# voxel-tracer/cuda-raytracing-optimized

Hardware: AMD Instinct MI355X
Metric: Msamples/s (pixels x spp / s), random-spheres 1200x800x100spp (higher is better)
Workload: dtype f32; 1 GPU; random-spheres (488 spheres, LCG seed 0) 1200x800 100spp maxDepth 50, gradient sky, reference RNG stream, fp parity; spp=100, max_depth=50, spheres=488, partition=single GPU, fp_mode=parity, rng=reference, kernel_variant=0

## Files before the change

cuda-raytracing-optimized_amd/__init__.py:

```python
import ctypes as C
import os

import numpy as np

_HERE = os.path.dirname(os.path.abspath(__file__))
RENDERER_LIB = os.path.join(_HERE, "librt_mi355x.so")
HOST_LIB = os.path.join(_HERE, "librt_host.so")

RT_DIFFUSE, RT_METAL, RT_GLASS = 0, 1, 2
(RT_FLOOR_COAT, RT_FLOOR_DIFFUSE, RT_FLOOR_CHECKER, RT_MODEL_COAT, RT_MODEL_DIFFUSE, RT_MODEL_GLOSSY, RT_MODEL_GLASS,
 RT_MODEL_TINTEDGLASS, RT_MODEL_SSS) = range(3, 12)
RT_SKY_CONST_GREY, RT_SKY_GRADIENT = 0, 1
RT_RNG_REFERENCE_STREAM, RT_RNG_COUNTER = 0, 1
RT_FP_PARITY, RT_FP_FAST = 0, 1
RT_MAX_DEVICES = 8



class vec3(C.Structure):
    _fields_ = [("e", C.c_float * 3)]


class camera(C.Structure):
    _fields_ = [("origin", vec3), ("lower_left_corner", vec3), ("horizontal", vec3), ("vertical", vec3),
                ("u", vec3), ("v", vec3), ("w", vec3), ("lens_radius", C.c_float)]


class sphere(C.Structure):
    _fields_ = [("center", vec3), ("radius", C.c_float)]


class plane(C.Structure):
    _fields_ = [("norm", vec3), ("point", vec3)]


class bbox(C.Structure):
    _fields_ = [("min", vec3), ("max", vec3)]


class triangle(C.Structure):
    _fields_ = [("v", vec3 * 3), ("texCoords", C.c_float * 6), ("meshID", C.c_ubyte), ("_pad", C.c_ubyte * 3)]


class bvh_node(C.Structure):
    _fields_ = [("a", vec3), ("b", vec3)]


class material(C.Structure):
    _fields_ = [("type", C.c_int32), ("color", vec3), ("param", C.c_float), ("texId", C.c_int32)]


class stexture(C.Structure):
    _fields_ = [("data", C.POINTER(C.c_float)), ("width", C.c_int32), ("height", C.c_int32)]


class mesh(C.Structure):
    _fields_ = [("tris", C.POINTER(triangle)), ("numTris", C.c_uint32), ("bvh", C.POINTER(bvh_node)),
                ("numBvhNodes", C.c_int32), ("bounds", bbox)]


class kernel_scene(C.Structure):
    _fields_ = [("m", C.POINTER(mesh)), ("floor", plane), ("materials", C.POINTER(material)),
                ("numMaterials", C.c_int32), ("textures", C.POINTER(stexture)), ("numTextures", C.c_int32),
                ("numPrimitivesPerLeaf", C.c_int32)]


class render_options(C.Structure):
    _fields_ = [("sky", C.c_int32), ("nee", C.c_int32), ("rr", C.c_int32), ("t_min", C.c_float),
                ("rng", C.c_int32), ("fp", C.c_int32), ("light", sphere), ("lightColor", vec3),
                ("stripe_rows", C.c_int32), ("num_devices", C.c_int32), ("devices", C.c_int32 * RT_MAX_DEVICES),
                ("part_rank", C.c_int32), ("part_world", C.c_int32), ("variant", C.c_int32), ("counters", C.c_int32),
                ("samples_per_item", C.c_int32), ("floor", C.c_int32)]


class render_stats(C.Structure):
    _fields_ = [("kernel_ms", C.c_double), ("total_ms", C.c_double), ("samples", C.c_int64),
                ("num_launches", C.c_int32), ("vgprs", C.c_int32), ("rays", C.c_uint64),
                ("prim_tests", C.c_uint64), ("node_visits", C.c_uint64), ("exec_tests", C.c_uint64),
                ("shadow_rays", C.c_uint64), ("box_tests", C.c_uint64), ("ref_stats", C.c_uint64 * 18)]


(RT_STAT_PRIMARY, RT_STAT_PRIMARY_HIT_MESH, RT_STAT_PRIMARY_NOHITS, RT_STAT_PRIMARY_BBOX_NOHITS, RT_STAT_SECONDARY,
 RT_STAT_SECONDARY_MESH, RT_STAT_SECONDARY_NOHIT, RT_STAT_SECONDARY_MESH_NOHIT, RT_STAT_SECONDARY_BBOX_NOHIT, RT_STAT_SHADOWS,
 RT_STAT_SHADOWS_BBOX_NOHITS, RT_STAT_SHADOWS_NOHITS, RT_STAT_LOW_POWER, RT_STAT_EXCEED_MAX_BOUNCE, RT_STAT_RUSSIAN_KILL,
 RT_STAT_NAN, RT_STAT_NODES_BOTH, RT_STAT_NODES_SINGLE) = range(18)
RT_STAT_NAMES = ["primary", "primary hit mesh", "primary nohit", "primary bb nohit", "secondary", "secondary mesh", "secondary no hit",
                 "secondary mesh nohit", "secondary bb nohit", "shadows", "shadows bb nohit", "shadows nohit", "power < 0.01",
                 "exceeded max bounce", "russian roulette", "NaNs", "both nodes hit", "single node hit"]


_SIZES = {vec3: 12, camera: 88, sphere: 16, plane: 24, bbox: 24, triangle: 64, bvh_node: 24, material: 24,
          stexture: 16, mesh: 56, kernel_scene: 64}
for _t, _s in _SIZES.items():
    assert C.sizeof(_t) == _s, (_t, C.sizeof(_t), _s)

sphere_dtype = np.dtype([("center", np.float32, 3), ("radius", np.float32)])
material_dtype = np.dtype([("type", np.int32), ("color", np.float32, 3), ("param", np.float32), ("texId", np.int32)])
triangle_dtype = np.dtype([("v", np.float32, (3, 3)), ("texCoords", np.float32, 6), ("meshID", np.uint8), ("_pad", np.uint8, 3)])
bvh_node_dtype = np.dtype([("a", np.float32, 3), ("b", np.float32, 3)])
assert sphere_dtype.itemsize == 16 and material_dtype.itemsize == 24
assert triangle_dtype.itemsize == 64 and bvh_node_dtype.itemsize == 24

RENDERER_SYMBOLS = ["initRenderer", "runRenderer", "cleanupRenderer", "initRendererSpheres",
                    "getDefaultRenderOptions", "setRenderOptions", "setExternalFramebuffer", "getRenderStats",
                    "rtDeviceCount", "rtApiVersion", "rtStructSizes", "rtLastLaunches",
                    "runRendererProgressive", "rtProgressiveSamples", "rtResetProgressive", "setCamera",
                    "renderGuides", "rtLastGuidesMs",
                    "rtDefaultDenoiseFlags", "denoiseFrame", "rtLastDenoiseMs",
                    "accumulateFrame", "rtResetHistory", "rtHistoryFrames", "rtLastAccumulateMs",
                    "previewFrame", "rtResetPreview", "rtPreviewFrames", "rtLastPreviewMs",
                    "displayFrame", "rtLastExposure", "rtDisplayHistogram", "rtResetDisplay", "rtLastDisplayMs",
                    "traceRays", "occludedRays", "rtLastRaysMs",
                    "updateTriangles", "updateMaterials", "updateSpheres", "getMeshBvh", "rtLastUpdateMs",
                    "rebuildBvh", "rtLastRebuildMs",
                    "rtLastSphereForm"]
RT_API_VERSION = 1002
ABI_STRUCTS = [render_options, render_stats, camera, sphere, material, triangle, bvh_node, mesh, kernel_scene, stexture, plane, bbox, vec3]
HOST_SYMBOLS = ["rtMakeCamera", "rtRandomFloat", "rtSceneThreeSpheres", "rtSceneRandomSpheres", "rtStaircaseCamera",
                "rtBuildBvh", "rtBuildBvhLevels", "rtLoadBvhFile", "rtSaveBvhFile", "rtFreeMesh", "rtMeshView",
                "rtSceneStaircaseProcedural", "rtLinearToSRGB", "rtWritePPM", "rtSaveReference", "rtLoadReference", "rtRmse",
                "rtDisplayFrameHost", "rtCentreRays", "rtRefitBvhArrays", "rtRefitBvh", "rtRebuildBvhArrays", "rtRebuildBvh"]

_renderer = None
_host = None


def load_host():
    global _host
    if _host is None:
        if not os.path.exists(HOST_LIB):
            raise ImportError(f"{HOST_LIB} is not built: run `make` (or __graft_entry__.build())")
        h = C.CDLL(HOST_LIB)
        fp = C.POINTER(C.c_float)
        h.rtMakeCamera.argtypes = [fp, fp, fp, C.c_float, C.c_float, C.c_float, C.c_float, C.POINTER(camera)]
        h.rtMakeCamera.restype = None
        h.rtRandomFloat.argtypes = [C.POINTER(C.c_uint32)]
        h.rtRandomFloat.restype = C.c_float
        h.rtSceneThreeSpheres.argtypes = [C.c_void_p, C.c_void_p, C.c_int, C.c_int, C.c_int, C.POINTER(camera)]
        h.rtSceneThreeSpheres.restype = C.c_int
        h.rtSceneRandomSpheres.argtypes = [C.c_uint32, C.c_void_p, C.c_void_p, C.c_int, C.c_int, C.c_int, C.POINTER(camera)]
        h.rtSceneRandomSpheres.restype = C.c_int
        h.rtStaircaseCamera.argtypes = [C.c_int, C.c_int, C.POINTER(camera)]
        h.rtStaircaseCamera.restype = None
        h.rtBuildBvh.argtypes = [C.c_void_p, C.c_int, C.c_int]
        h.rtBuildBvh.restype = C.c_void_p
        h.rtBuildBvhLevels.argtypes = [C.c_void_p, C.c_int, C.c_int, C.c_int]
        h.rtBuildBvhLevels.restype = C.c_void_p
        h.rtLoadBvhFile.argtypes = [C.c_char_p]
        h.rtLoadBvhFile.restype = C.c_void_p
        h.rtSaveBvhFile.argtypes = [C.c_void_p, C.c_char_p]
        h.rtSaveBvhFile.restype = C.c_int
        h.rtFreeMesh.argtypes = [C.c_void_p]
        h.rtFreeMesh.restype = None
        h.rtMeshView.argtypes = [C.c_void_p, C.POINTER(mesh)]
        h.rtMeshView.restype = C.c_int
        h.rtSceneStaircaseProcedural.argtypes = [C.c_int, C.c_void_p, C.c_int, C.c_void_p]
        h.rtSceneStaircaseProcedural.restype = C.c_int
        h.rtLinearToSRGB.argtypes = [C.c_float]
        h.rtLinearToSRGB.restype = C.c_uint32
        h.rtWritePPM.argtypes = [C.c_char_p, C.c_int, C.c_int, C.c_void_p]
        h.rtWritePPM.restype = C.c_int
        h.rtSaveReference.argtypes = [C.c_char_p, C.c_int, C.c_int, C.c_void_p]
        h.rtSaveReference.restype = C.c_int
        h.rtLoadReference.argtypes = [C.c_char_p, C.c_void_p, C.c_int, C.c_int]
        h.rtLoadReference.restype = C.c_int
        h.rtRmse.argtypes = [C.c_void_p, C.c_void_p, C.c_int, C.c_int]
        h.rtRmse.restype = C.c_double
        h.rtDisplayFrameHost.argtypes = [C.c_void_p, C.c_void_p, C.c_int, C.c_int, C.c_int, C.c_int, C.c_float, C.c_float, C.POINTER(C.c_float),
                                         C.POINTER(C.c_uint32)]
        h.rtDisplayFrameHost.restype = C.c_int
        h.rtCentreRays.argtypes = [C.POINTER(camera), C.c_int, C.c_int, C.POINTER(C.c_int32), C.c_int, fp, fp]
        h.rtCentreRays.restype = None
        h.rtRefitBvhArrays.argtypes = [C.c_void_p, C.c_uint32, C.c_void_p, C.c_int, C.c_int, C.POINTER(bbox)]
        h.rtRefitBvhArrays.restype = C.c_int
        h.rtRefitBvh.argtypes = [C.c_void_p]
        h.rtRefitBvh.restype = C.c_int
        h.rtRebuildBvhArrays.argtypes = [C.c_void_p, C.c_uint32, C.c_void_p, C.c_int, C.c_int, C.POINTER(bbox), C.c_void_p]
        h.rtRebuildBvhArrays.restype = C.c_int
        h.rtRebuildBvh.argtypes = [C.c_void_p, C.c_void_p]
        h.rtRebuildBvh.restype = C.c_int
        _host = h
    return _host


def check_abi(lib, path=RENDERER_LIB, structs=None):
    structs = ABI_STRUCTS if structs is None else structs
    if not hasattr(lib, "rtStructSizes"):
        raise ImportError(f"{path} predates the ABI handshake (no rtStructSizes): rebuild it with `make`")
    lib.rtApiVersion.argtypes = []
    lib.rtApiVersion.restype = C.c_int
    lib.rtStructSizes.argtypes = [C.POINTER(C.c_int32), C.c_int]
    lib.rtStructSizes.restype = C.c_int
    ver = lib.rtApiVersion()
    if ver != RT_API_VERSION:
        raise ImportError(f"{path} has API version {ver}, this binding was written against {RT_API_VERSION}: rebuild the library or update the mirror")
    out = (C.c_int32 * len(structs))()
    n = lib.rtStructSizes(out, len(structs))
    if n != len(structs):
        raise ImportError(f"{path} reports {n} ABI structs, the mirror has {len(structs)}")
    for t, sz in zip(structs, out):
        if C.sizeof(t) != sz:
            raise ImportError(f"{path}: sizeof({t.__name__}) is {sz} in the library and {C.sizeof(t)} in the Python mirror - "
                              "library and mirror are of different generations; refusing to call into it")


def load_renderer():
    global _renderer
    if _renderer is None:
        if not os.path.exists(RENDERER_LIB):
            raise ImportError(f"{RENDERER_LIB} is not built: run `make` (or __graft_entry__.build()); "
                              "there is no CPU fallback for the render path")
        r = C.CDLL(RENDERER_LIB)
        check_abi(r)
        r.initRenderer.argtypes = [kernel_scene, camera, C.POINTER(C.POINTER(vec3)), C.c_int, C.c_int, C.c_int]
        r.initRenderer.restype = None
        r.runRenderer.argtypes = [C.c_int, C.c_int, C.c_int]
        r.runRenderer.restype = None
        r.cleanupRenderer.argtypes = []
        r.cleanupRenderer.restype = None
        r.initRendererSpheres.argtypes = [C.c_void_p, C.c_void_p, C.c_int, camera, C.POINTER(C.POINTER(vec3)),
                                          C.c_int, C.c_int, C.c_int]
        r.initRendererSpheres.restype = None
        r.getDefaultRenderOptions.argtypes = [C.POINTER(render_options), C.c_int]
        r.getDefaultRenderOptions.restype = None
        r.setRenderOptions.argtypes = [C.POINTER(render_options)]
        r.setRenderOptions.restype = None
        r.setExternalFramebuffer.argtypes = [C.c_void_p]
        r.setExternalFramebuffer.restype = None
        r.getRenderStats.argtypes = [C.POINTER(render_stats)]
        r.getRenderStats.restype = None
        r.rtDeviceCount.argtypes = []
        r.rtDeviceCount.restype = C.c_int
        r.rtApiVersion.argtypes = []
        r.rtApiVersion.restype = C.c_int
        r.rtLastLaunches.argtypes = [C.POINTER(C.c_int32), C.c_int]
        r.rtLastLaunches.restype = C.c_int
        r.runRendererProgressive.argtypes = [C.c_int, C.c_int, C.c_int]
        r.runRendererProgressive.restype = None
        r.rtProgressiveSamples.argtypes = []
        r.rtProgressiveSamples.restype = C.c_int
        r.rtResetProgressive.argtypes = []
        r.rtResetProgressive.restype = None
        r.setCamera.argtypes = [C.POINTER(camera)]
        r.setCamera.restype = None
        r.renderGuides.argtypes = [C.c_int, C.POINTER(C.c_float), C.POINTER(C.c_float), C.POINTER(C.c_float),
                                   C.POINTER(C.c_int32), C.POINTER(C.c_int32)]
        r.renderGuides.restype = None
        r.rtLastGuidesMs.argtypes = []
        r.rtLastGuidesMs.restype = C.c_double
        r.rtDefaultDenoiseFlags.argtypes = []
        r.rtDefaultDenoiseFlags.restype = C.c_int
        r.denoiseFrame.argtypes = [C.c_void_p, C.c_void_p, C.c_int, C.c_int, C.c_int, C.c_float, C.c_float]
        r.denoiseFrame.restype = None
        r.rtLastDenoiseMs.argtypes = []
        r.rtLastDenoiseMs.restype = C.c_double
        r.accumulateFrame.argtypes = [C.c_void_p, C.c_void_p, C.c_void_p, C.c_int, C.c_int, C.c_float, C.c_float]
        r.accumulateFrame.restype = None
        r.rtResetHistory.argtypes = []
        r.rtResetHistory.restype = None
        r.rtHistoryFrames.argtypes = []
        r.rtHistoryFrames.restype = C.c_int
        r.rtLastAccumulateMs.argtypes = []
        r.rtLastAccumulateMs.restype = C.c_double
        r.previewFrame.argtypes = [C.c_void_p, C.c_void_p, C.c_void_p, C.c_void_p, C.c_int, C.c_int, C.c_int, C.c_int, C.c_float, C.c_float, C.c_float]
        r.previewFrame.restype = None
        r.rtResetPreview.argtypes = []
        r.rtResetPreview.restype = None
        r.rtPreviewFrames.argtypes = []
        r.rtPreviewFrames.restype = C.c_int
        r.rtLastPreviewMs.argtypes = []
        r.rtLastPreviewMs.restype = C.c_double
        r.displayFrame.argtypes = [C.c_void_p, C.c_void_p, C.c_int, C.c_int, C.c_float, C.c_float]
        r.displayFrame.restype = None
        r.rtLastExposure.argtypes = []
        r.rtLastExposure.restype = C.c_float
        r.rtDisplayHistogram.argtypes = [C.POINTER(C.c_uint32), C.c_int]
        r.rtDisplayHistogram.restype = C.c_int
        r.rtResetDisplay.argtypes = []
        r.rtResetDisplay.restype = None
        r.rtLastDisplayMs.argtypes = []
        r.rtLastDisplayMs.restype = C.c_double
        fp, ip = C.POINTER(C.c_float), C.POINTER(C.c_int32)
        r.traceRays.argtypes = [C.c_int, fp, fp, fp, fp, C.c_int, fp, ip, fp, fp, ip]
        r.traceRays.restype = None
        r.occludedRays.argtypes = [C.c_int, fp, fp, fp, fp, C.POINTER(C.c_uint8)]
        r.occludedRays.restype = None
        r.rtLastRaysMs.argtypes = []
        r.rtLastRaysMs.restype = C.c_double
        r.updateTriangles.argtypes = [C.c_int, C.c_int, C.c_void_p]
        r.updateTriangles.restype = None
        r.updateMaterials.argtypes = [C.c_void_p, C.c_int]
        r.updateMaterials.restype = None
        r.updateSpheres.argtypes = [C.c_void_p, C.c_void_p, C.c_int]
        r.updateSpheres.restype = None
        r.getMeshBvh.argtypes = [C.c_void_p, C.c_int, C.POINTER(bbox)]
        r.getMeshBvh.restype = C.c_int
        r.rtLastUpdateMs.argtypes = []
        r.rtLastUpdateMs.restype = C.c_double
        r.rebuildBvh.argtypes = [C.c_void_p]
        r.rebuildBvh.restype = None
        r.rtLastRebuildMs.argtypes = []
        r.rtLastRebuildMs.restype = C.c_double
        _renderer = r
    return _renderer



def _f3(v):
    return (C.c_float * 3)(*[float(x) for x in v])


def make_camera(lookfrom, lookat, vup, vfov, aspect, aperture, focus_dist):
    cam = camera()
    load_host().rtMakeCamera(_f3(lookfrom), _f3(lookat), _f3(vup), vfov, aspect, aperture, focus_dist, C.byref(cam))
    return cam


def scene_three_spheres(nx, ny):
    sp = np.zeros(3, sphere_dtype)
    mt = np.zeros(3, material_dtype)
    cam = camera()
    n = load_host().rtSceneThreeSpheres(sp.ctypes.data, mt.ctypes.data, 3, nx, ny, C.byref(cam))
    assert n == 3
    return sp, mt, cam


def scene_random_spheres(nx, ny, seed=0):
    cap = 488
    sp = np.zeros(cap, sphere_dtype)
    mt = np.zeros(cap, material_dtype)
    cam = camera()
    n = load_host().rtSceneRandomSpheres(seed, sp.ctypes.data, mt.ctypes.data, cap, nx, ny, C.byref(cam))
    assert n == cap, n
    return sp, mt, cam


def staircase_camera(nx, ny):
    cam = camera()
    load_host().rtStaircaseCamera(nx, ny, C.byref(cam))
    return cam


class HostMesh:

    def __init__(self, handle):
        if not handle:
            raise ValueError("mesh build/load failed")
        self._h = C.c_void_p(handle)
        self.view = mesh()
        self.nppl = load_host().rtMeshView(self._h, C.byref(self.view))

    @classmethod
    def build(cls, tris, nppl=5, extra_levels=None):
        tris = np.ascontiguousarray(tris, dtype=triangle_dtype)
        if extra_levels is None:
            return cls(load_host().rtBuildBvh(tris.ctypes.data, len(tris), nppl))
        return cls(load_host().rtBuildBvhLevels(tris.ctypes.data, len(tris), nppl, extra_levels))

    @classmethod
    def load(cls, path):
        return cls(load_host().rtLoadBvhFile(os.fsencode(path)))

    def save(self, path):
        return load_host().rtSaveBvhFile(self._h, os.fsencode(path))

    @property
    def tris(self):
        return np.ctypeslib.as_array(C.cast(self.view.tris, C.POINTER(C.c_ubyte)), (self.view.numTris * 64,)).view(triangle_dtype)

    @property
    def bvh(self):
        return np.ctypeslib.as_array(C.cast(self.view.bvh, C.POINTER(C.c_ubyte)), (self.view.numBvhNodes * 24,)).view(bvh_node_dtype)

    def refit(self):
        if load_host().rtRefitBvh(self._h) != 0:
            raise ValueError("rtRefitBvh refused the mesh")
        self.nppl = load_host().rtMeshView(self._h, C.byref(self.view))

    def rebuild(self):
        old_slot = np.zeros(self.view.numTris, np.int32)
        if load_host().rtRebuildBvh(self._h, old_slot.ctypes.data) != 0:
            raise ValueError("rtRebuildBvh refused the mesh")
        self.nppl = load_host().rtMeshView(self._h, C.byref(self.view))
        return old_slot

    def close(self):
        if self._h:
            load_host().rtFreeMesh(self._h)
            self._h = None

    def __del__(self):
        try:
            self.close()
        except Exception:
            pass


def scene_staircase_procedural(detail=1):
    h = load_host()
    mats = np.zeros(20, material_dtype)
    need = h.rtSceneStaircaseProcedural(detail, None, 0, mats.ctypes.data)
    n = -need if need < 0 else need
    tris = np.zeros(n, triangle_dtype)
    got = h.rtSceneStaircaseProcedural(detail, tris.ctypes.data, n, mats.ctypes.data)
    assert got == n, (got, n)
    return tris, mats


def make_kernel_scene(host_mesh, materials, textures=(), floor=None):
    materials = np.ascontiguousarray(materials, dtype=material_dtype)
    ks = kernel_scene()
    ks.m = C.pointer(host_mesh.view)
    ks.materials = C.cast(materials.ctypes.data, C.POINTER(material))
    ks.numMaterials = len(materials)
    tex_arr = (stexture * max(1, len(textures)))()
    keep = [materials, tex_arr, host_mesh]
    for k, t in enumerate(textures):
        t = np.ascontiguousarray(t, dtype=np.float32)
# ... 167 lines not shown
def update_materials(mats):
    mats = _records("update_materials", "material", mats, material_dtype)
    load_renderer().updateMaterials(mats.ctypes.data, len(mats))


def update_spheres(spheres, mats):
    spheres = _records("update_spheres", "sphere", spheres, sphere_dtype)
    mats = _records("update_spheres", "material", mats, material_dtype)
    if len(spheres) != len(mats):
        raise ValueError("update_spheres: one material per sphere")
    load_renderer().updateSpheres(spheres.ctypes.data, mats.ctypes.data, len(spheres))


def mesh_bvh():
    r = load_renderer()
    n = r.getMeshBvh(None, 0, None)
    nodes = np.zeros(n, bvh_node_dtype)
    b = bbox()
    r.getMeshBvh(nodes.ctypes.data, n, C.byref(b))
    return nodes, np.array([list(b.min.e), list(b.max.e)], np.float32)


def last_update_ms():
    return load_renderer().rtLastUpdateMs()


def _header_constant(name):
    import re
    text = open(os.path.join(os.path.dirname(_HERE), "include", "rt_api.h")).read()
    m = re.search(r"^#define\s+%s\s+\(?\s*(\d+)\s*(?:<<\s*(\d+))?\s*\)?\s*$" % name, text, re.M)
    if not m:
        raise ImportError(f"include/rt_api.h does not define {name}")
    return int(m.group(1)) << int(m.group(2) or 0)


RT_REBUILD_TILE = _header_constant("RT_REBUILD_TILE")
RT_REBUILD_MAX_TRIS = _header_constant("RT_REBUILD_MAX_TRIS")


def rebuild_bvh():
    r = load_renderer()
    old_slot = np.zeros(int(_state.get("num_tris") or 0) if not _state.get("spheres") else 0, np.int32)
    r.rebuildBvh(old_slot.ctypes.data if len(old_slot) else None)
    return old_slot


def last_rebuild_ms():
    return load_renderer().rtLastRebuildMs()


def rebuild_bvh_arrays(tris, bvh, nppl):
    for name, a, dt in (("tris", tris, triangle_dtype), ("bvh", bvh, bvh_node_dtype)):
        if not (isinstance(a, np.ndarray) and a.dtype == dt and a.ndim == 1 and a.flags["C_CONTIGUOUS"] and a.flags["WRITEABLE"]):
            raise ValueError(f"rebuild_bvh_arrays: {name} must be a writable C-contiguous one-dimensional array of its record dtype")
    if isinstance(nppl, bool) or not isinstance(nppl, (int, np.integer)):
        raise ValueError("rebuild_bvh_arrays: nppl must be an integer")
    b = bbox()
    old_slot = np.zeros(len(tris), np.int32)
    if load_host().rtRebuildBvhArrays(tris.ctypes.data, len(tris), bvh.ctypes.data, len(bvh), int(nppl), C.byref(b), old_slot.ctypes.data) != 0:
        return None
    return np.array([list(b.min.e), list(b.max.e)], np.float32), old_slot


def refit_bvh_arrays(tris, bvh, nppl):
    tris = _records("refit_bvh_arrays", "triangle", tris, triangle_dtype)
    if not (isinstance(bvh, np.ndarray) and bvh.dtype == bvh_node_dtype and bvh.ndim == 1 and bvh.flags["C_CONTIGUOUS"] and bvh.flags["WRITEABLE"]):
        raise ValueError("refit_bvh_arrays: bvh must be a writable C-contiguous one-dimensional array of bvh_node_dtype records")
    b = bbox()
    if load_host().rtRefitBvhArrays(tris.ctypes.data, len(tris), bvh.ctypes.data, len(bvh), int(nppl), C.byref(b)) != 0:
        return None
    return np.array([list(b.min.e), list(b.max.e)], np.float32)


def centre_rays(cam, nx, ny, ij):
    ij = np.ascontiguousarray(ij, dtype=np.int32)
    if ij.ndim != 2 or ij.shape[1] != 2:
        raise ValueError(f"centre_rays: ij must have shape (n, 2), got {ij.shape}")
    n = ij.shape[0]
    org, d = np.zeros((n, 3), np.float32), np.zeros((n, 3), np.float32)
    fp = C.POINTER(C.c_float)
    load_host().rtCentreRays(C.byref(cam), nx, ny, ij.ctypes.data_as(C.POINTER(C.c_int32)), n, org.ctypes.data_as(fp), d.ctypes.data_as(fp))
    return org, d


RT_DENOISE_DEMODULATE, RT_DENOISE_SAME_PRIM = 1, 2
RT_DENOISE_MAX_ITERATIONS, RT_DENOISE_MAX_SQUARINGS, RT_DENOISE_ALBEDO_FLOOR = 8, 7, 0.01


def default_denoise_flags():
    return load_renderer().rtDefaultDenoiseFlags()


def _frame_in_out(who, fb, out):
    shape = (_state["ny"], _state["nx"], 3)
    ok = lambda a: isinstance(a, np.ndarray) and a.dtype == np.float32 and a.flags["C_CONTIGUOUS"] and a.shape == shape
    if fb is not None and not ok(fb):
        raise ValueError(f"{who}: fb must be a C-contiguous float32 array of shape {shape}")
    if out is None:
        out = np.empty(shape, np.float32)
    elif not (ok(out) and out.flags["WRITEABLE"]):
        raise ValueError(f"{who}: out must be a writable C-contiguous float32 array of shape {shape}")
    return None if fb is None else fb.ctypes.data, out


def denoiseFrame(fb=None, iterations=5, flags=None, normal_squarings=5, sigma_z=0.01, sigma_c=1.0, out=None):
    r = load_renderer()
    if flags is None:
        flags = r.rtDefaultDenoiseFlags()
    src, out = _frame_in_out("denoiseFrame", fb, out)
    r.denoiseFrame(src, out.ctypes.data, iterations, flags, normal_squarings, sigma_z, sigma_c)
    return out


def last_denoise_ms():
    return load_renderer().rtLastDenoiseMs()


RT_ACCUM_MAX_HISTORY = 1024


def accumulateFrame(fb=None, out=None, history=False, flags=None, max_history=32, sigma_z=0.01, normal_min=0.9):
    nx, ny = _state["nx"], _state["ny"]
    r = load_renderer()
    if flags is None:
        flags = r.rtDefaultDenoiseFlags()
    src, out = _frame_in_out("accumulateFrame", fb, out)
    hist = None
    if history is True:
        hist = np.empty((ny, nx), np.float32)
    elif history is not False and history is not None:
        hist = history
        if not (isinstance(hist, np.ndarray) and hist.dtype == np.float32 and hist.flags["C_CONTIGUOUS"] and hist.flags["WRITEABLE"] and hist.shape == (ny, nx)):
            raise ValueError(f"accumulateFrame: history must be True, False or a writable C-contiguous float32 array of shape {(ny, nx)}")
    r.accumulateFrame(src, out.ctypes.data, None if hist is None else hist.ctypes.data, flags, max_history, sigma_z, normal_min)
    return out if hist is None else (out, hist)


def reset_history():
    load_renderer().rtResetHistory()


def history_frames():
    return load_renderer().rtHistoryFrames()


def last_accumulate_ms():
    return load_renderer().rtLastAccumulateMs()


RT_PREVIEW_MIN_HISTORY, RT_PREVIEW_LUM_EPS = 4.0, 1e-4


def _pixel_plane(who, what, plane):
    shape = (_state["ny"], _state["nx"])
    if plane is True:
        return np.empty(shape, np.float32)
    if plane is False or plane is None:
        return None
    if not (isinstance(plane, np.ndarray) and plane.dtype == np.float32 and plane.flags["C_CONTIGUOUS"] and plane.flags["WRITEABLE"] and plane.shape == shape):
        raise ValueError(f"{who}: {what} must be True, False or a writable C-contiguous float32 array of shape {shape}")
    return plane


def previewFrame(fb=None, out=None, history=False, variance=False, flags=None, max_history=32, iterations=5, normal_squarings=5, sigma_z=0.01, normal_min=0.9,
                 sigma_l=4.0):
    r = load_renderer()
    if flags is None:
        flags = r.rtDefaultDenoiseFlags()
    src, out = _frame_in_out("previewFrame", fb, out)
    hist = _pixel_plane("previewFrame", "history", history)
    var = _pixel_plane("previewFrame", "variance", variance)
    r.previewFrame(src, out.ctypes.data, None if hist is None else hist.ctypes.data, None if var is None else var.ctypes.data, flags, max_history, iterations,
                   normal_squarings, sigma_z, normal_min, sigma_l)
    planes = tuple(a for a in (hist, var) if a is not None)
    return (out,) + planes if planes else out


def reset_preview():
    load_renderer().rtResetPreview()


def preview_frames():
    return load_renderer().rtPreviewFrames()


def last_preview_ms():
    return load_renderer().rtLastPreviewMs()


RT_DISPLAY_TOP_DOWN, RT_DISPLAY_DITHER, RT_DISPLAY_AUTO_EXPOSURE, RT_DISPLAY_FROM_PREVIEW = 1, 2, 4, 8
RT_TONEMAP_NONE, RT_TONEMAP_REINHARD, RT_TONEMAP_ACES = 0, 1, 2
RT_DISPLAY_BINS, RT_DISPLAY_KEY = 256, 0.18
RT_DISPLAY_BAYER8 = ((0, 32, 8, 40, 2, 34, 10, 42), (48, 16, 56, 24, 50, 18, 58, 26), (12, 44, 4, 36, 14, 46, 6, 38), (60, 28, 52, 20, 62, 30, 54, 22),
                     (3, 35, 11, 43, 1, 33, 9, 41), (51, 19, 59, 27, 49, 17, 57, 25), (15, 47, 7, 39, 13, 45, 5, 37), (63, 31, 55, 23, 61, 29, 53, 21))


def _display_in_out(who, src, out, shape):
    if src is not None and not (isinstance(src, np.ndarray) and src.dtype == np.float32 and src.flags["C_CONTIGUOUS"] and src.shape == shape + (3,)):
        raise ValueError(f"{who}: src must be a C-contiguous float32 array of shape {shape + (3,)}")
    if out is None:
        out = np.empty(shape + (4,), np.uint8)
    elif not (isinstance(out, np.ndarray) and out.dtype == np.uint8 and out.flags["C_CONTIGUOUS"] and out.flags["WRITEABLE"] and out.shape == shape + (4,)):
        raise ValueError(f"{who}: out must be a writable C-contiguous uint8 array of shape {shape + (4,)}")
    return None if src is None else src.ctypes.data, out


def display_frame(src=None, out=None, flags=0, tonemap=0, exposure=1.0, adapt=1.0):
    src, out = _display_in_out("display_frame", src, out, (_state["ny"], _state["nx"]))
    load_renderer().displayFrame(src, out.ctypes.data, flags, tonemap, exposure, adapt)
    return out


def last_exposure():
    return load_renderer().rtLastExposure()


def display_histogram():
    out = np.zeros(RT_DISPLAY_BINS, np.uint32)
    n = load_renderer().rtDisplayHistogram(out.ctypes.data_as(C.POINTER(C.c_uint32)), RT_DISPLAY_BINS)
    assert n == RT_DISPLAY_BINS
    return out


def reset_display():
    load_renderer().rtResetDisplay()


def last_display_ms():
    return load_renderer().rtLastDisplayMs()


def display_frame_host(src, out=None, flags=0, tonemap=0, exposure=1.0, adapt=1.0, state=None, histogram=False):
    if not (isinstance(src, np.ndarray) and src.ndim == 3):
        raise ValueError("display_frame_host: src must be a (ny, nx, 3) float32 array")
    addr, out = _display_in_out("display_frame_host", src, out, src.shape[:2])
    if state is not None and not (isinstance(state, np.ndarray) and state.dtype == np.float32 and state.size == 1 and state.flags["WRITEABLE"]):
        raise ValueError("display_frame_host: state must be None or a writable float32 array of one element")
    hist = np.zeros(RT_DISPLAY_BINS, np.uint32) if histogram else None
    rc = load_host().rtDisplayFrameHost(addr, out.ctypes.data, src.shape[1], src.shape[0], flags, tonemap, exposure, adapt,
                                        None if state is None else state.ctypes.data_as(C.POINTER(C.c_float)),
                                        None if hist is None else hist.ctypes.data_as(C.POINTER(C.c_uint32)))
    if rc != 0:
        raise ValueError("display_frame_host: arguments displayFrame would refuse (flags, tonemap, exposure or adapt)")
    return (out, hist) if histogram else out


def cleanupRenderer():
    load_renderer().cleanupRenderer()
    _state.update(fb=None, keep=None)


def getDefaultRenderOptions(is_sphere_scene):
    o = render_options()
    load_renderer().getDefaultRenderOptions(C.byref(o), 1 if is_sphere_scene else 0)
    return o


def setRenderOptions(opt=None, **kw):
    if opt is None:
        raise ValueError("pass the options struct from getDefaultRenderOptions()")
    for k, v in kw.items():
        if k == "devices":
            opt.num_devices = len(v)
            for idx, d in enumerate(v):
                opt.devices[idx] = d
        else:
            setattr(opt, k, v)
    load_renderer().setRenderOptions(C.byref(opt))
    return opt


def setExternalFramebuffer(array):
    if array is None:
        load_renderer().setExternalFramebuffer(None)
        _state["ext"] = None
        return
    assert array.dtype == np.float32 and array.flags["C_CONTIGUOUS"] and array.shape == (_state["ny"], _state["nx"], 3)
    load_renderer().setExternalFramebuffer(array.ctypes.data)
    _state["ext"] = array


def getRenderStats():
    s = render_stats()
    load_renderer().getRenderStats(C.byref(s))
    return s


def device_count():
    return load_renderer().rtDeviceCount()


RT_KERNEL_SPHERE_QUEUE, RT_KERNEL_SPHERE_TILES, RT_KERNEL_MESH_QUEUE, RT_KERNEL_MESH_TILES = 1, 2, 3, 4
LAUNCH_FIELDS = ("family", "phase", "cls", "chunked", "dbg", "scene", "lean", "threads", "blocks", "device", "fp")


def last_launches():
    lib = load_renderer()
    n = lib.rtLastLaunches(None, 0)
    buf = (C.c_int32 * (n * len(LAUNCH_FIELDS)))()
    n = min(n, lib.rtLastLaunches(buf, n))
    return [dict(zip(LAUNCH_FIELDS, buf[k * len(LAUNCH_FIELDS):(k + 1) * len(LAUNCH_FIELDS)])) for k in range(n)]


RT_SPHERE_FORM_NONE, RT_SPHERE_FORM_GENERAL, RT_SPHERE_FORM_DEFAULT = -1, 0, 1


def last_sphere_form():
    lib = load_renderer()
    lib.rtLastSphereForm.argtypes = []
    lib.rtLastSphereForm.restype = C.c_int
    return lib.rtLastSphereForm()



def write_ppm(path, fb):
    fb = np.ascontiguousarray(fb, dtype=np.float32)
    return load_host().rtWritePPM(os.fsencode(path), fb.shape[1], fb.shape[0], fb.ctypes.data)


def save_reference(path, fb):
    fb = np.ascontiguousarray(fb, dtype=np.float32)
    return load_host().rtSaveReference(os.fsencode(path), fb.shape[1], fb.shape[0], fb.ctypes.data)


def load_reference(path, nx, ny):
    out = np.zeros((ny, nx, 3), np.float32)
    rc = load_host().rtLoadReference(os.fsencode(path), out.ctypes.data, nx, ny)
    return rc, out


def rmse(f, g):
    f = np.ascontiguousarray(f, dtype=np.float32)
    g = np.ascontiguousarray(g, dtype=np.float32)
    assert f.shape == g.shape
    return load_host().rtRmse(f.ctypes.data, g.ctypes.data, f.shape[1], f.shape[0])



PROBE_SYMBOLS = [f"rtProbe{n}_{m}" for n in ("Rng", "DiskSphere", "GetRay", "SphereHit", "TriangleHit", "Bbox", "Scatter", "Math", "ShadowRay", "PlaneHit", "SinCos", "Schlick")
                 for m in ("parity", "fast")]


def _f32(a):
    return np.ascontiguousarray(a, dtype=np.float32)


def _u32(a):
    return np.ascontiguousarray(a, dtype=np.uint32)


def _p(a):
    return a.ctypes.data_as(C.c_void_p)


class Probe:

    def __init__(self, mode="parity"):
        assert mode in ("parity", "fast")
        self.lib = load_renderer()
        self.sfx = "_" + mode

    def _fn(self, name):
        f = getattr(self.lib, "rtProbe" + name + self.sfx)
        f.restype = None
        return f

    def rng(self, pixel_ids):
        ids = _u32(pixel_ids); n = len(ids)
        seed = np.zeros(n, np.uint32); draws = np.zeros((n, 4), np.float32); state = np.zeros(n, np.uint32)
        self._fn("Rng")(_p(ids), C.c_int(n), _p(seed), _p(draws), _p(state))
        return seed, draws, state

    def disk_sphere(self, states):
        st = _u32(states); n = len(st)
        disk = np.zeros((n, 3), np.float32); sd = np.zeros(n, np.uint32)
        sph = np.zeros((n, 3), np.float32); ss = np.zeros(n, np.uint32)
        self._fn("DiskSphere")(_p(st), C.c_int(n), _p(disk), _p(sd), _p(sph), _p(ss))
        return disk, sd, sph, ss

    def get_ray(self, cam, s, t, states):
        s = _f32(s); t = _f32(t); st = _u32(states); n = len(s)
        org = np.zeros((n, 3), np.float32); d = np.zeros((n, 3), np.float32); sa = np.zeros(n, np.uint32)
        self._fn("GetRay")(C.byref(cam), _p(s), _p(t), _p(st), C.c_int(n), _p(org), _p(d), _p(sa))
        return org, d, sa

    def sphere_hit(self, spheres, org, dirs, tmin, tmax):
        sp = np.ascontiguousarray(spheres, dtype=sphere_dtype); n = len(sp)
        org = _f32(org); dirs = _f32(dirs); tmin = _f32(tmin); tmax = _f32(tmax)
        out = np.zeros(n, np.float32)
        self._fn("SphereHit")(_p(sp), _p(org), _p(dirs), _p(tmin), _p(tmax), C.c_int(n), _p(out))
        return out

    def triangle_hit(self, tris, org, dirs, tmin, tmax):
        tr = np.ascontiguousarray(tris, dtype=triangle_dtype); n = len(tr)
        org = _f32(org); dirs = _f32(dirs); tmin = _f32(tmin); tmax = _f32(tmax)
        t = np.zeros(n, np.float32); u = np.zeros(n, np.float32); v = np.zeros(n, np.float32)
        self._fn("TriangleHit")(_p(tr), _p(org), _p(dirs), _p(tmin), _p(tmax), C.c_int(n), _p(t), _p(u), _p(v))
        return t, u, v

    def bbox(self, bmin, bmax, org, dirs, tmax):
        bmin = _f32(bmin); bmax = _f32(bmax); org = _f32(org); dirs = _f32(dirs); tmax = _f32(tmax); n = len(tmax)
        dist = np.zeros(n, np.float32); hit = np.zeros(n, np.int32)
        self._fn("Bbox")(_p(bmin), _p(bmax), _p(org), _p(dirs), _p(tmax), C.c_int(n), _p(dist), _p(hit))
        return dist, hit

    def scatter(self, t, normal, inside, wo, mats, color, states, hit_point=None):
        t = _f32(t); normal = _f32(normal); inside = np.ascontiguousarray(inside, dtype=np.int32); wo = _f32(wo)
        hp = _f32(hit_point if hit_point is not None else np.zeros((len(t), 3), np.float32))
        mats = np.ascontiguousarray(mats, dtype=material_dtype); color = _f32(color); st = _u32(states); n = len(t)
        wi = np.zeros((n, 3), np.float32); thr = np.zeros((n, 3), np.float32); flags = np.zeros(n, np.int32)
        tout = np.zeros(n, np.float32); sa = np.zeros(n, np.uint32)
        self._fn("Scatter")(_p(t), _p(hp), _p(normal), _p(inside), _p(wo), _p(mats), _p(color), _p(st), C.c_int(n),
                            _p(wi), _p(thr), _p(flags), _p(tout), _p(sa))
        return wi, thr, flags, tout, sa

    def shadow_ray(self, light, light_color, org, atten, normal, states):
        org = _f32(org); atten = _f32(atten); normal = _f32(normal); st = _u32(states); n = len(st)
        out = np.zeros((n, 9), np.float32); ok = np.zeros(n, np.int32); sa = np.zeros(n, np.uint32)
        self._fn("ShadowRay")(C.byref(light), C.byref(light_color), _p(org), _p(atten), _p(normal), _p(st), C.c_int(n), _p(out), _p(ok), _p(sa))
        return ok, out[:, 0:3], out[:, 3:6], out[:, 6], out[:, 7], out[:, 8].astype(np.int32), sa

    def plane_hit(self, planes, org, dirs, tmin, tmax):
        pl = np.ascontiguousarray(planes, dtype=np.float32).reshape(-1, 6); n = len(pl)
        org = _f32(org); dirs = _f32(dirs); tmin = _f32(tmin); tmax = _f32(tmax)
        out = np.zeros(n, np.float32)
        self._fn("PlaneHit")(_p(pl), _p(org), _p(dirs), _p(tmin), _p(tmax), C.c_int(n), _p(out))
        return out

    def sincos(self, y):
        y = _f32(y); n = len(y)
        s = np.zeros(n, np.float32); c = np.zeros(n, np.float32)
        self._fn("SinCos")(_p(y), C.c_int(n), _p(s), _p(c))
        return s, c

    def schlick(self, cosine, ref_idx, u):
        c = _f32(cosine); r = _f32(ref_idx); u = _f32(u); n = len(c)
        out = np.zeros(n, np.float32); above = np.zeros(n, np.int32)
        self._fn("Schlick")(_p(c), _p(r), _p(u), C.c_int(n), _p(out), _p(above))
        return out, above

    def math(self, a, b):
        a = _f32(a); b = _f32(b); n = len(a)
        q = np.zeros(n, np.float32); r = np.zeros(n, np.float32); p5 = np.zeros(n, np.float32); u3 = np.zeros((n, 3), np.float32)
        self._fn("Math")(_p(a), _p(b), C.c_int(n), _p(q), _p(r), _p(p5), _p(u3))
        return q, r, p5, u3
```

cuda-raytracing-optimized_amd/csrc/rt_kernels_spheres.hip:

```cpp
#include "rt_device.h"
#include "rt_params.h"
#include "rt_sphere_form.h"

#include <float.h>
#include <cstdio>
#include <cstdlib>
#include <algorithm>
#include <utility>

using namespace rtd;

#if defined(RT_MODE_PARITY)
#define RT_LAUNCH_NAME rt_launch_spheres_parity
#elif defined(RT_MODE_FAST)
#define RT_LAUNCH_NAME rt_launch_spheres_fast
#else
#error "define RT_MODE_PARITY or RT_MODE_FAST"
#endif

namespace {

#ifndef RT_BOX_CUT
#define RT_BOX_CUT 12
#endif
// ... 873 lines not shown
        if (px < P.nx && r < P.part.local_rows)
            fbf[((size_t)r * P.nx + i0) * 3 + off] = wfb[q];
    }

    if (P.counters) {
        atomicAdd(&P.counters->rays, (unsigned long long)nrays);
        atomicAdd(&P.counters->prim_tests, (unsigned long long)nrays * (unsigned long long)P.n);
        atomicAdd(&P.counters->exec_tests, (unsigned long long)groups_done * 4ull);
        atomicAdd(&P.counters->box_tests, (unsigned long long)boxes_done);
    }
}

template <int SCENE>
__global__ void __launch_bounds__(kThreads) k_classify_spheres(const RtSphereParams P) {
    extern __shared__ __align__(16) unsigned char smem[];
    float* unused;
    const SceneLds S = stage_scene<false, SCENE>(P, smem, &unused);
    const int tiles_x = (P.nx + 7) >> 3;
    const int tiles_y = (P.part.local_rows + 7) >> 3;
    const uint32_t total = (uint32_t)tiles_x * (uint32_t)tiles_y * 64u;
    const uint32_t p = blockIdx.x * kThreads + threadIdx.x;
    const uint32_t tile = p >> 6, within = p & 63u;
    const int ty = (int)(tile / (uint32_t)tiles_x), tx = (int)(tile - (uint32_t)ty * (uint32_t)tiles_x);
    const int i = tx * 8 + (int)(within & 7u);
    const int lr = ty * 8 + (int)(within >> 3);
    const bool valid = p < total && i < P.nx && lr < P.part.local_rows;
    bool hits = false, glass = false;
    if (valid) {
        const int j = global_row(P.part, lr);
        const float u = ((float)i + 0.5f) / (float)P.nx, v = ((float)j + 0.5f) / (float)P.ny;
        const f3 org = ld3(P.cam.origin);
        const f3 dn = unit(ld3(P.cam.lower_left_corner) + u * ld3(P.cam.horizontal) + v * ld3(P.cam.vertical) - org);
        for (int k = 0; k < P.n_padded; k++) {
            const float4 sph = S.sph[sidx(k)];
            const f3 oc = org - F3(sph.x, sph.y, sph.z);
            const float b = dot(oc, dn);
            const float c = dot(oc, oc) - sph.w;
            const bool h = (S.orig[k] != 0x7fffffff) && (b * b - c > 0.0f) && (b < 0.0f || c < 0.0f);
            hits = hits || h;
            glass = glass || (h && S.typ[k] == RT_GLASS);
        }
    }
    const int cls = glass ? 0 : (hits ? 1 : 2);
    const unsigned long long m0 = __ballot(valid && cls == 0), m1 = __ballot(valid && cls == 1), m2 = __ballot(valid && cls == 2);
    uint32_t b0 = 0, b1 = 0, b2 = 0;
    if ((threadIdx.x & 63) == 0) {
        if (m0) b0 = atomicAdd(P.queue + 4, (uint32_t)__popcll(m0));
        if (m1) b1 = atomicAdd(P.queue + 5, (uint32_t)__popcll(m1));
        if (m2) b2 = atomicAdd(P.queue + 6, (uint32_t)__popcll(m2));
    }
    b0 = __builtin_amdgcn_readfirstlane(b0);
    b1 = __builtin_amdgcn_readfirstlane(b1);
    b2 = __builtin_amdgcn_readfirstlane(b2);
    if (valid) {
        const unsigned long long m = cls == 0 ? m0 : (cls == 1 ? m1 : m2);
        const uint32_t base = cls == 0 ? b0 : (cls == 1 ? b1 : b2);
        const uint32_t rank = __builtin_amdgcn_mbcnt_hi((uint32_t)(m >> 32), __builtin_amdgcn_mbcnt_lo((uint32_t)m, 0u));
        P.order[(uint32_t)cls * total + base + rank] = p;
    }
}

#if defined(RT_MODE_PARITY)
__device__ __forceinline__ Hit first_hit_spheres(const RtSphereParams& P, const SceneLds& S, f3 org, f3 dn, float t_min, float t_max, f3& normal) {
    const float a = dot(dn, dn);
    Hit h = { t_max, -1, 0x7fffffff };
    for (int k = 0; k < P.n_padded; k++) {
        const int orig = S.orig[k];
        if (orig == 0x7fffffff) continue;
        const float t = sphere_hit_exact(S.sph[sidx(k)], org, dn, a, t_min, h.closest);
        if (t < t_max) accept(h, t, k, orig);
    }
    normal = F3(0, 0, 0);
    if (h.sid >= 0) {
        const float4 sc4 = S.sph[sidx(h.sid)];
        const f3 hp = org + h.closest * dn;
        normal = (hp - F3(sc4.x, sc4.y, sc4.z)) / S.rad[h.sid];
        if (dot(dn, normal) > 0.0f) normal = -normal;
    } else {
        h.closest = FLT_MAX;
    }
    return h;
}

template <int SCENE>
__global__ void __launch_bounds__(kThreads) k_guides_spheres(const RtSphereParams P, const RtGuidePlanes G) {
    extern __shared__ __align__(16) unsigned char smem[];
    float* unused;
    const SceneLds S = stage_scene<false, SCENE>(P, smem, &unused);
    const int tiles_x = (P.nx + 7) >> 3;
    const int tiles_y = (P.part.local_rows + 7) >> 3;
    const uint32_t total = (uint32_t)tiles_x * (uint32_t)tiles_y * 64u;
    const uint32_t p = blockIdx.x * kThreads + threadIdx.x;
    const uint32_t tile = p >> 6, within = p & 63u;
    const int ty = (int)(tile / (uint32_t)tiles_x), tx = (int)(tile - (uint32_t)ty * (uint32_t)tiles_x);
    const int i = tx * 8 + (int)(within & 7u);
    const int lr = ty * 8 + (int)(within >> 3);
    if (!(p < total && i < P.nx && lr < P.part.local_rows)) return;
    const int j = global_row(P.part, lr);
    const float u = ((float)i + 0.5f) / (float)P.nx, v = ((float)j + 0.5f) / (float)P.ny;
    const f3 org = ld3(P.cam.origin);
    const f3 dir = unit(ld3(P.cam.lower_left_corner) + u * ld3(P.cam.horizontal) + v * ld3(P.cam.vertical) - org);
    const f3 dn = unit(dir);
    f3 normal;
    const Hit h = first_hit_spheres(P, S, org, dn, P.t_min, FLT_MAX, normal);
    const size_t px = (size_t)lr * P.nx + i;
    f3 albedo;
    if (h.sid >= 0) {
        const float4 m = S.mat[h.sid];
        albedo = F3(m.x, m.y, m.z);
    } else {
        albedo = sky_color(P.sky, dir);
    }
    if (G.albedo) { float* o = G.albedo + px * 3; o[0] = albedo.x; o[1] = albedo.y; o[2] = albedo.z; }
    if (G.normal) { float* o = G.normal + px * 3; o[0] = normal.x; o[1] = normal.y; o[2] = normal.z; }
    if (G.depth) G.depth[px] = h.closest;
    if (G.prim) G.prim[px] = h.sid >= 0 ? h.orig : RT_GUIDE_PRIM_NONE;
}

template <int SCENE, bool ANY>
__global__ void __launch_bounds__(kThreads) k_rays_spheres(const RtSphereParams P, const RtRayBatch B) {
    extern __shared__ __align__(16) unsigned char smem[];
    float* unused;
    const SceneLds S = stage_scene<false, SCENE>(P, smem, &unused);
    const uint32_t n = (uint32_t)B.n;
    const uint32_t tiles = (n + kThreads - 1) / kThreads;
    for (uint32_t tile = blockIdx.x; tile < tiles; tile += gridDim.x) {
        const uint32_t r = tile * kThreads + threadIdx.x;
        const bool live = r < n;
        f3 org = F3(0, 0, 0), dn = F3(0, 0, 1);
        float t_min = B.t_min_default, t_max = FLT_MAX;
        if (live) {
            const float* o = B.org + (size_t)r * 3;
            const float* d = B.dir + (size_t)r * 3;
            org = F3(o[0], o[1], o[2]);
            dn = unit(F3(d[0], d[1], d[2]));
            if (B.t_min) t_min = B.t_min[r];
            if (B.t_max) t_max = fminf(B.t_max[r], FLT_MAX);
        }
        if (ANY) {
            const float a = dot(dn, dn);
            bool occ = false;
            for (int base = 0; base < P.n_padded; base += kSphereGroup) {
#pragma unroll
                for (int kk = 0; kk < kSphereGroup; kk++) {
                    const int k = base + kk;
                    const int orig = S.orig[k];
                    if (live && !occ && orig != 0x7fffffff)
                        occ = sphere_hit_exact(S.sph[sidx(k)], org, dn, a, t_min, t_max) < t_max;
                }
                if (__ballot(live && !occ) == 0ull) break;
            }
            if (live) B.occluded[r] = occ ? 1 : 0;
        } else if (live) {
            f3 normal;
            const Hit h = first_hit_spheres(P, S, org, dn, t_min, t_max, normal);
            if (B.t) B.t[r] = h.closest;
            if (B.prim) B.prim[r] = h.sid >= 0 ? h.orig : RT_GUIDE_PRIM_NONE;
            if (B.normal) { float* o = B.normal + (size_t)r * 3; o[0] = normal.x; o[1] = normal.y; o[2] = normal.z; }
            if (B.uv) { float* o = B.uv + (size_t)r * 2; o[0] = 0.0f; o[1] = 0.0f; }
        }
    }
}
#endif

constexpr int kCostClasses = 18;
constexpr int kChainClasses = 4;
constexpr int kExactCostSamples = 8;
constexpr int kHeavyClasses = 3;

static_assert(9ull * 16ull * 255ull * RT_PROGRESSIVE_MAX_SAMPLES <= 0xFFFFFFFFull, "cost_class: window sum of a progressive total overflows 32 bits");
__device__ __forceinline__ int cost_class(const RtSphereParams& P, const uint32_t* __restrict__ rays, uint32_t samples, bool exact, int i, int lr) {
    uint32_t sum = 0, cnt = 0;
    for (int dy = -1; dy <= 1; dy++) {
        const int y = lr + dy;
        if (y < 0 || y >= P.part.local_rows) continue;
        for (int dx = -1; dx <= 1; dx++) {
            const int x = i + dx;
            if (x < 0 || x >= P.nx) continue;
            sum += rays[(size_t)y * P.nx + x];
            cnt++;
        }
    }
    const uint32_t own = (rays[(size_t)lr * P.nx + i] * (exact ? 16u : 12u)) / samples;
    const uint32_t e = max((sum * 16u) / (cnt * samples), own);
    const uint32_t lim[kCostClasses - 1] = { (uint32_t)P.chain_top_thr, 320u, 240u, 192u, 160u, 128u, 96u, 72u, 56u, 44u, 36u, 30u, 26u, 22u, 19u, 18u, 17u };
    int cls = kCostClasses - 1;
#pragma unroll
    for (int c = kCostClasses - 2; c >= 0; c--) if (e >= lim[c]) cls = c;
    return cls;
}

__device__ __forceinline__ uint32_t coprime_stride_of(uint32_t n) {
    if (n <= 64u) return 1u;
    uint32_t c = ((uint32_t)((unsigned long long)n * 2654435769ull >> 32)) | 1u;
    for (;;) {
        uint32_t a = c, b = n;
        while (b) { const uint32_t t = a % b; a = b; b = t; }
        if (a == 1u) break;
        c += 2u;
    }
    return c % n;
}

constexpr int kOrderBlocks = 1024;

template <int PASS>
__global__ void __launch_bounds__(kThreads) k_order_by_cost(const RtSphereParams P) {
    constexpr int kLists = kCostClasses * kXcdQueues;
    __shared__ uint32_t s_cnt[kLists], s_base[kLists], s_start[kLists], s_n[kLists], s_stride[kLists];
    const int xq = P.xcd_queues == kXcdQueues ? kXcdQueues : 1;
    const int tiles_x = (P.nx + 7) >> 3;
    const int tiles_y = (P.part.local_rows + 7) >> 3;
    const uint32_t total = (uint32_t)tiles_x * (uint32_t)tiles_y * 64u;
    const uint32_t per = ((total + gridDim.x - 1u) / gridDim.x + (uint32_t)kThreads - 1u) / (uint32_t)kThreads * (uint32_t)kThreads;
    const uint32_t first = blockIdx.x * per, last = min(first + per, total);
    const bool fresh = P.s_split == 0;
    const bool exact = fresh && P.cost_samples >= kExactCostSamples;
    const uint32_t* const rays = fresh ? P.cost_rays : P.px_rays;
    const uint32_t samples = (uint32_t)(fresh ? P.cost_samples : P.s_split);
    uint32_t packed = 0;
    auto class_of = [&](uint32_t p) {
        const uint32_t tile = p >> 6, within = p & 63u;
        const int ty = (int)(tile / (uint32_t)tiles_x), tx = (int)(tile - (uint32_t)ty * (uint32_t)tiles_x);
        const int i = tx * 8 + (int)(within & 7u);
        const int lr = ty * 8 + (int)(within >> 3);
        packed = ((uint32_t)lr << 16) | (uint32_t)i;
        if (!(p < last && i < P.nx && lr < P.part.local_rows)) return -1;
        const int x = xq > 1 ? (int)rt_xcd_of_pixel((uint32_t)lr, (uint32_t)P.nx, (uint32_t)i) : 0;
        return x * kCostClasses + cost_class(P, rays, samples, exact, i, lr);
    };
    if (threadIdx.x < kLists) s_cnt[threadIdx.x] = 0u;
    __syncthreads();
    for (uint32_t p = first + threadIdx.x; p < last; p += kThreads) {
        const int cls = class_of(p);
        if (cls >= 0) atomicAdd(&s_cnt[cls], 1u);
    }
    __syncthreads();
    const int lx = (int)threadIdx.x / kCostClasses, lc = (int)threadIdx.x - lx * kCostClasses;
    uint32_t* const Q = P.queue + (size_t)lx * kXcdQueueWords;
    if (PASS == 0) {
        if ((int)threadIdx.x < xq * kCostClasses && s_cnt[threadIdx.x]) atomicAdd(Q + 4 + lc, s_cnt[threadIdx.x]);
        return;
    }
    if ((int)threadIdx.x < xq * kCostClasses) {
        uint32_t start = 0;
        for (int x = 0; x < lx; x++)
            for (int c = 0; c < kCostClasses; c++) start += P.queue[(size_t)x * kXcdQueueWords + 4 + c];
        if (lc == 0) Q[3] = start;
        for (int c = 0; c < lc; c++) start += Q[4 + c];
        const uint32_t n = Q[4 + lc];
        s_start[threadIdx.x] = start;
        s_n[threadIdx.x] = n;
        s_stride[threadIdx.x] = (lc == kCostClasses - 1) ? 1u : coprime_stride_of(n);
        s_base[threadIdx.x] = s_cnt[threadIdx.x] ? atomicAdd(Q + 4 + kCostClasses + lc, s_cnt[threadIdx.x]) : 0u;
        s_cnt[threadIdx.x] = 0u;
    }
    __syncthreads();
    for (uint32_t p = first + threadIdx.x; p < last; p += kThreads) {
        const int cls = class_of(p);
        if (cls >= 0) {
            const uint32_t rank = s_base[cls] + atomicAdd(&s_cnt[cls], 1u);
            const uint32_t at = s_start[cls] + (uint32_t)(((unsigned long long)rank * s_stride[cls]) % s_n[cls]);
            const size_t px = (size_t)(packed >> 16) * P.nx + (packed & 0xFFFFu);
            const float4 state = fresh ? make_float4(0.0f, 0.0f, 0.0f, __uint_as_float(pixel_seed((uint32_t)(global_row(P.part, (int)(packed >> 16)) * P.nx + (int)(packed & 0xFFFFu)))))
                                       : P.px_state[px];
            const uint32_t parked_rays = fresh ? 0u : P.px_rays[px];
            if (P.ord_rec) {
                P.ord_rec[2 * (size_t)at] = state;
                P.ord_rec[2 * (size_t)at + 1] = make_float4(__uint_as_float(packed), __uint_as_float(parked_rays), 0.0f, 0.0f);
            } else {
                P.order[at] = packed;
                P.ord_state[at] = state;
                P.ord_rays[at] = parked_rays;
            }
        }
    }
}


constexpr int kCfgCull = 1 << 0;
constexpr int kCfgChainSingle = 1 << 1;
constexpr int kCfgSingleRay = 1 << 2;
constexpr BitField kCfgPool = { 3, 0x1F };
constexpr BitField kCfgBoost = { 8, 0xFF };
constexpr BitField kCfgSparseMax = { 16, 0xFF };
constexpr int kCfgDbgLight = 1 << 29;
constexpr int kCfgP1Segments = 1 << 30;
constexpr BitField kChainEvery = { 0, 0xFF };
constexpr BitField kChainWaves = { 8, 0xF };
constexpr BitField kChainPixels = { 12, 0xF };
constexpr BitField kChainHeavyThr = { 16, 0xFF };
constexpr BitField kChainLists = { 24, 0xF };
constexpr BitField caps_list(int c) { return { 4 * c, 0xF }; }
constexpr BitField kCapsMidWaves = { 16, 0xF };
constexpr BitField kCapsMidCap = { 20, 0xFF };

template <int FORM> struct FormTag {};
constexpr int kDefaultCfg = kCfgCull | kCfgChainSingle | kCfgSingleRay | kCfgPool.put(1) | kCfgBoost.put(1) | kCfgSparseMax.put(4);
constexpr int default_chain_cfg(bool six_waves) { return kChainEvery.put(1) | kChainWaves.put(six_waves ? 2 : 3) | kChainPixels.put(4) | kChainHeavyThr.put(8) | kChainLists.put(4); }
constexpr int kDefaultCaps = caps_list(0).put(1) | caps_list(1).put(4) | caps_list(2).put(4) | caps_list(3).put(4) | kCapsMidWaves.put(0) | kCapsMidCap.put(16);
template <int PHASE, int CLS, bool CHUNKED, bool DBG, int SCENE = 0, int LEAN = 0, int FORM = 0>
__global__ void __launch_bounds__(kThreads, (LEAN & 4) ? 6 : 4) k_render_spheres_queue(const RtSphereParams P, uint32_t stride, int cfg, int chain_cfg, int caps, FormTag<FORM>) {
    static_assert(FORM == kSphereFormGeneral || (PHASE == 2 && CLS == 2 && !CHUNKED && !DBG && SCENE == 0), "the folded form is the cost-ordered dispatch of whole pixels, LDS scene, no diagnostics");
    constexpr bool FOLDED = FORM == kSphereFormDefault;
    constexpr bool MID = CLS == 2 && !FOLDED;
    if (FOLDED) { cfg = kDefaultCfg; chain_cfg = default_chain_cfg((LEAN & 4) != 0); caps = kDefaultCaps; }
    extern __shared__ __align__(16) unsigned char smem[];
    float* unused;
    const SceneLds S = stage_scene<false, SCENE>(P, smem, &unused);

    const bool cull = (cfg & kCfgCull) != 0;
    const int boost = (cfg >> kCfgBoost.shift) & kCfgBoost.mask;
    const int sparse_max = (cfg >> kCfgSparseMax.shift) & kCfgSparseMax.mask;
    const int tiles_x = (P.nx + 7) >> 3;
    const int tiles_y = (P.part.local_rows + 7) >> 3;
    const uint32_t padded = (uint32_t)tiles_x * (uint32_t)tiles_y * 64u;
    constexpr int n_cls = CLS == 2 ? kCostClasses : (CLS == 1 ? 3 : 0);
    __shared__ uint32_t s_cls_base[kCostClasses], s_cls_pos[kCostClasses + 1], s_cls_stride[kCostClasses];
    __shared__ uint32_t s_q[8 * kXcdQueues];
    const uint32_t xq = (FOLDED || (CLS == 2 && P.xcd_queues == kXcdQueues)) ? (uint32_t)kXcdQueues : 1u;
    const uint32_t myx = xq > 1u ? ((uint32_t)__builtin_amdgcn_s_getreg((31 << 11) | 20) & (uint32_t)(kXcdQueues - 1)) : 0u;
    if (threadIdx.x < xq) {
        const uint32_t x = threadIdx.x;
        const uint32_t* const Q = P.queue + (size_t)x * kXcdQueueWords;
        const uint32_t seg = CLS == 2 ? Q[3] : 0u;
        const int n_chain = CLS == 2 ? ((chain_cfg >> kChainLists.shift) & kChainLists.mask) : 0;
        const int n_heavy_end = CLS == 2 ? kChainClasses + kHeavyClasses : 1;
        uint32_t pos = 0, nA = 0, n0 = 0;
        for (int c = 0; c < n_cls; c++) {
            const uint32_t n = Q[4 + c];
            if (x == myx) {
                s_cls_base[c] = CLS == 2 ? seg + pos : (uint32_t)c * padded;
                s_cls_pos[c] = pos;
                s_cls_stride[c] = (CLS != 1 || c == n_cls - 1) ? 1u : coprime_stride_of(n);
            }
            if (c < n_chain) nA += n; else if (c < n_heavy_end) n0 += n;
            pos += n;
        }
        if (x == myx) for (int c = n_cls; c <= kCostClasses; c++) s_cls_pos[c] = pos;
        const uint32_t total_px = n_cls ? pos - nA : padded;
        const uint32_t n_rest = total_px - n0;
        const uint32_t wgs = xq > 1u ? max(gridDim.x / xq, 1u) : gridDim.x;
        uint32_t spread = wgs * blockDim.x;
        if (nA > 0u) spread -= min(spread - 64u, ((wgs + (uint32_t)(chain_cfg & kChainEvery.mask) - 1u) / (uint32_t)(chain_cfg & kChainEvery.mask)) * (uint32_t)((chain_cfg >> kChainWaves.shift) & kChainWaves.mask) * 64u);
        uint32_t* const sq = s_q + 8 * x;
        sq[0] = nA; sq[1] = n0; sq[2] = total_px * (CHUNKED ? (uint32_t)P.chunks : 1u); sq[3] = spread;
        sq[4] = (n0 > 0u && n0 <= spread && (spread - n0) <= n_rest) ? 1u : 0u;
        sq[5] = 0u;
        if (MID && ((caps >> kCapsMidWaves.shift) & kCapsMidWaves.mask) != 0 && n0 > 0u) { sq[5] = 1u; sq[2] = n_rest; sq[4] = 0u; }
        sq[6] = seg;
    }
    __syncthreads();
    int role = 2;
    if (CLS == 2 && s_q[8 * myx] > 0u && (int)(threadIdx.x >> 6) < ((chain_cfg >> kChainWaves.shift) & kChainWaves.mask) && (blockIdx.x % (uint32_t)(chain_cfg & kChainEvery.mask)) == 0u) role = 0;
    else if (MID && s_q[8 * myx + 5] != 0u && (int)(threadIdx.x >> 6) < ((chain_cfg >> kChainWaves.shift) & kChainWaves.mask) + ((caps >> kCapsMidWaves.shift) & kCapsMidWaves.mask)) role = 1;
    const int mid_cap = (caps >> kCapsMidCap.shift) & kCapsMidCap.mask;
    uint32_t stolen = 0;
    int ccls = 7;

    Lane L;
    L.col = F3(0, 0, 0);
    L.org = F3(0, 0, 0); L.dir = F3(0, 0, 1);
    int lr = 0;
    int chunk = 0, s_end_lane = 0;
    auto s_end_of = [&]() -> int { return CHUNKED ? s_end_lane : (PHASE == 1 ? P.s_split : (PHASE == 2 ? P.ns : min(P.ns, P.spw))); };
    uint32_t nrays = 0, groups_done = 0, boxes_done = 0;
    bool have_pixel = false;
    uint32_t pix_rays = 0;
    bool exhausted = false;
    uint32_t pool_next = 0, pool_end = 0;
    float* fbf = reinterpret_cast<float*>(P.fb);
    auto sample_params = [&]() {
        typedef const __attribute__((address_space(4))) float* ColdF;
        typedef const __attribute__((address_space(4))) int32_t* ColdI;
        unsigned long long base = (unsigned long long)P.self;
        asm volatile("" : "+s"(base));
        SampleParams sp;
        ColdF cf = (ColdF)(base + offsetof(RtSphereParams, cam));
        float* dst = reinterpret_cast<float*>(&sp.cam);
#pragma unroll
        for (int k = 0; k < (int)(sizeof(rt_camera) / 4); k++) dst[k] = cf[k];
        sp.nx = *(ColdI)(base + offsetof(RtSphereParams, nx)); sp.ny = *(ColdI)(base + offsetof(RtSphereParams, ny));
        sp.rng_mode = *(ColdI)(base + offsetof(RtSphereParams, rng_mode));
        return sp;
    };
    unsigned long long* const wdbg = DBG ? P.wave_dbg : nullptr;
    const unsigned long long dbg_t0 = wdbg ? __builtin_amdgcn_s_memrealtime() : 0ull;
    const unsigned long long dbg_t0c = wdbg ? __builtin_amdgcn_s_memtime() : 0ull;
    unsigned long long dbg_tex = 0ull;
    uint32_t dbg_iters = 0, dbg_coop_iters = 0, dbg_coop_rays = 0, dbg_maxpix = 0;
    unsigned long long dbg_tm[16] = { 0, 0, 0, 0, 0, 0, 0, 0, 0, 0, 0, 0, 0, 0, 0, 0 };
    float dbg_grab = 0.0f, dbg_p1 = 0.0f;

    bool need_sample = false;
    auto finish = [&](bool fin, bool now, f3 sample) {
        if (fin) {
            if (DBG && P.counters && (isnan(sample.x) || isnan(sample.y) || isnan(sample.z))) ray_stat<DBG>(P, RT_STAT_NAN);
            L.col = L.col + sample;
            L.s++;
            if (L.s < s_end_of()) {
                if (now) start_sample<PHASE == 0>(sample_params(), L); else need_sample = true;
            } else {
                if (PHASE == 1) {
                    const size_t px = (size_t)lr * P.nx + L.i;
                    P.px_state[px] = make_float4(L.col.x, L.col.y, L.col.z, __uint_as_float(L.rng));
                    P.px_rays[px] = pix_rays;
                } else if (!CHUNKED) {
                    const f3 out = L.col / (float)P.ns;
                    *reinterpret_cast<float3*>(fbf + ((size_t)((!FOLDED && P.fb_global_rows) ? L.j : lr) * P.nx + L.i) * 3) = make_float3(out.x, out.y, out.z);
                    uint32_t* const rays_out = rt_cold_arg<uint32_t*>(offsetof(RtSphereParams, acc_rays));
                    if (rays_out) {
                        const size_t px = (size_t)lr * P.nx + L.i;
                        rays_out[px] = pix_rays;
                        float4* const acc = rt_cold_arg<float4*>(offsetof(RtSphereParams, acc_state));
                        if (acc) acc[px] = make_float4(L.col.x, L.col.y, L.col.z, __uint_as_float(L.rng));
                    }
                } else {
                    float* dst = reinterpret_cast<float*>(P.partial) + (((size_t)lr * P.nx + L.i) * (uint32_t)P.chunks + (uint32_t)chunk) * 3;
                    dst[0] = L.col.x; dst[1] = L.col.y; dst[2] = L.col.z;
                }
                if (wdbg) {
                    dbg_maxpix = max(dbg_maxpix, pix_rays);
                    if (PHASE == 2)
                        P.px_state[(size_t)lr * P.nx + L.i] = make_float4(dbg_grab, (float)(__builtin_amdgcn_s_memrealtime() - dbg_t0) * 1e-5f, (float)pix_rays, dbg_p1);
                }
                have_pixel = false;
            }
        }
    };

    uint32_t poison_at = (PHASE == 1 && P.poison_fb) ? 2u + 2u * ((blockIdx.x * (blockDim.x >> 6) + (threadIdx.x >> 6)) % 24u) : ~0u;
    uint32_t iter_no = 0;
    while (true) {
        if (PHASE == 1 && iter_no++ == poison_at) poison_rows(P, (size_t)blockIdx.x * blockDim.x + threadIdx.x, (size_t)gridDim.x * blockDim.x);
        const bool dbg_timers = DBG && wdbg && (cfg & kCfgDbgLight) == 0;
        const unsigned long long t_refill = dbg_timers ? __builtin_amdgcn_s_memtime() : 0ull;
        while (!exhausted) {
            const unsigned long long live_m = __ballot(have_pixel);
            int cap = 64;
            if (MID && (role == 1 || __ballot(have_pixel && ccls == 6) != 0ull)) cap = mid_cap;
            if (CLS == 2 && (role == 0 || __ballot(have_pixel && ccls < 6) != 0ull)) {
                cap = (chain_cfg >> kChainPixels.shift) & kChainPixels.mask;
                if (__ballot(have_pixel && ccls == 2) != 0ull) cap = min(cap, (caps >> caps_list(2).shift) & caps_list(2).mask);
                if (__ballot(have_pixel && ccls == 1) != 0ull) cap = min(cap, (caps >> caps_list(1).shift) & caps_list(1).mask);
                if (__ballot(have_pixel && ccls == 0) != 0ull) cap = min(cap, caps & caps_list(0).mask);
            }
            const int allowed = cap - (int)__popcll(live_m);
            if (allowed <= 0) break;
            const unsigned long long idle_m = ~live_m;
            const uint32_t idle_rank = __builtin_amdgcn_mbcnt_hi((uint32_t)(idle_m >> 32), __builtin_amdgcn_mbcnt_lo((uint32_t)idle_m, 0u));
            const unsigned long long need = __ballot(!have_pixel && idle_rank < (uint32_t)allowed);
            if (need == 0ull) break;
            const uint32_t cnt = (role == 0 && (cfg & kCfgChainSingle)) ? 1u : (uint32_t)__popcll(need);
            const uint32_t qx = xq > 1u ? ((myx + (stolen >> 1)) & (uint32_t)(kXcdQueues - 1)) : 0u;
            const uint32_t* const sq = s_q + 8 * qx;
            const uint32_t total = sq[2];
            if (pool_next >= pool_end) {
                const bool leftovers = (stolen & 1u) != 0u;
                const uint32_t grab = leftovers ? 1u : ((CHUNKED || PHASE == 1) ? max(cnt, 128u) : ((PHASE == 2 && role == 2) ? max(cnt, (uint32_t)((cfg >> kCfgPool.shift) & kCfgPool.mask) * 4u) : cnt));
                const uint32_t limit = (role == 0 || leftovers) ? sq[0] : ((MID && role == 1) ? sq[1] : total);
                uint32_t b = 0;
                if ((threadIdx.x & 63) == 0) b = atomicAdd(P.queue + (size_t)qx * kXcdQueueWords + ((role == 0 || leftovers) ? 1 : ((MID && role == 1) ? 2 : 0)), grab);
                b = __builtin_amdgcn_readfirstlane(b);
                if (b >= limit) {
                    if (role < 2) { role = 2; continue; }
                    if (xq > 1u && stolen + 1u < 2u * xq) { stolen++; continue; }
                    exhausted = true;
                    break;
                }
                pool_next = b;
                pool_end = min(b + grab, limit);
            }
            const uint32_t base = pool_next;
            const uint32_t take = min(cnt, pool_end - pool_next);
            pool_next += take;
            const uint32_t rank = __builtin_amdgcn_mbcnt_hi((uint32_t)(need >> 32), __builtin_amdgcn_mbcnt_lo((uint32_t)need, 0u));
            if (role == 2 && pool_next >= total && xq == 1u) exhausted = true;
            if (!have_pixel && rank < take) {
                const uint32_t item = base + rank;
                uint32_t pos = item;
                if (CHUNKED) { pos = item / (uint32_t)P.chunks; chunk = (int)(item - pos * (uint32_t)P.chunks); }
                uint32_t p, opos = 0;
                float4 rec0 = make_float4(0.0f, 0.0f, 0.0f, 0.0f);
                uint32_t rec_rays = 0;
                if (CLS == 0) {
                    if (PHASE == 1 && (cfg & kCfgP1Segments) != 0) p = ((uint32_t)(((unsigned long long)(pos >> 3) * stride) % (padded >> 3)) << 3) | (pos & 7u);
                    else p = (uint32_t)(((unsigned long long)pos * stride) % padded);
                } else {
                    uint32_t q;
                    if (role == 0 || (stolen & 1u) != 0u) q = pos;
                    else if (MID && role == 1) q = sq[0] + pos;
                    else if (MID && sq[5] != 0u) q = sq[0] + sq[1] + pos;
                    else {
                        const uint32_t nA = sq[0], n0 = sq[1], spread = sq[3];
                        const bool spread_ok = sq[4] != 0u;
                        uint32_t i0, i1;
                        bool is0;
                        if (spread_ok && pos < spread) {
                            const uint32_t before = (uint32_t)(((unsigned long long)pos * n0) / spread);
                            const uint32_t after = (uint32_t)(((unsigned long long)(pos + 1u) * n0) / spread);
                            is0 = after > before; i0 = before; i1 = pos - before;
                        } else if (spread_ok) {
                            is0 = false; i0 = 0; i1 = pos - n0;
                        } else {
                            is0 = pos < n0; i0 = pos; i1 = pos - n0;
                        }
                        q = nA + (is0 ? i0 : n0 + i1);
                    }
                    if (CLS == 2) {
                        opos = sq[6] + q;
                        if (FOLDED || P.ord_rec) {
                            rec0 = P.ord_rec[2 * (size_t)opos];
                            const float4 rec1 = P.ord_rec[2 * (size_t)opos + 1];
                            p = __float_as_uint(rec1.x);
                            rec_rays = __float_as_uint(rec1.y);
                        } else {
                            p = P.order[opos];
                        }
                    } else {
                        int c = 0;
                        for (int k = 1; k < n_cls; k++) if (q >= s_cls_pos[k]) c = k;
                        const uint32_t j = q - s_cls_pos[c];
                        const uint32_t nc = s_cls_pos[c + 1] - s_cls_pos[c];
                        p = P.order[s_cls_base[c] + (uint32_t)(((unsigned long long)j * s_cls_stride[c]) % nc)];
                    }
                }
                int i;
                if (CLS == 2) {
                    i = (int)(p & 0xFFFFu);
                    lr = (int)(p >> 16);
                } else {
                    const uint32_t tile = p >> 6, within = p & 63u;
                    const int ty = (int)(tile / (uint32_t)tiles_x), tx = (int)(tile - (uint32_t)ty * (uint32_t)tiles_x);
                    i = tx * 8 + (int)(within & 7u);
                    lr = ty * 8 + (int)(within >> 3);
                }
                if (i < P.nx && lr < P.part.local_rows) {
                    const int acc_first = (PHASE == 0 && !CHUNKED) ? rt_cold_arg<int32_t>(offsetof(RtSphereParams, acc_first)) : 0;
                    if (acc_first > 0) {
                        const size_t px = (size_t)lr * P.nx + i;
                        const float4 st4 = rt_cold_arg<const float4*>(offsetof(RtSphereParams, acc_state))[px];
                        L.i = i; L.j = global_row(P.part, lr);
                        L.pixelId = (uint32_t)(L.j * P.nx + i);
                        L.rng = __float_as_uint(st4.w);
                        L.col = F3(st4.x, st4.y, st4.z);
                        L.s = acc_first;
                        pix_rays = rt_cold_arg<const uint32_t*>(offsetof(RtSphereParams, acc_rays))[px];
                    } else if (PHASE == 0) {
                        s_end_lane = min(P.ns, (chunk + 1) * P.spw);
                        init_pixel(P, L, i, global_row(P.part, lr), chunk * P.spw);
                        pix_rays = 0;
                    } else if (PHASE == 1) {
                        init_pixel(P, L, i, global_row(P.part, lr), 0);
                        pix_rays = 0;
                    } else {
                        const float4 st4 = (CLS == 2 && (FOLDED || P.ord_rec)) ? rec0 : P.ord_state[opos];
                        L.i = i; L.j = global_row(P.part, lr);
                        L.pixelId = (uint32_t)(L.j * P.nx + i);
                        L.rng = __float_as_uint(st4.w);
                        L.col = F3(st4.x, st4.y, st4.z);
                        L.s = P.s_split;
                        pix_rays = (CLS == 2 && (FOLDED || P.ord_rec)) ? rec_rays : P.ord_rays[opos];
                        if (wdbg) { dbg_grab = (float)(__builtin_amdgcn_s_memrealtime() - dbg_t0) * 1e-5f; dbg_p1 = (float)pix_rays; }
                    }
                    need_sample = true;
                    have_pixel = true;
                    ccls = 7;
                    if (CLS == 2 && role == 0) { ccls = 0; for (int k = 1; k < kChainClasses; k++) if (pos >= s_cls_pos[k]) ccls = k; }
                    if (MID && role == 1) ccls = 6;
                    if (CLS == 2 && role == 2 && (stolen & 1u) != 0u) ccls = kChainClasses - 1;
                }
            }
        }
        if (need_sample) { start_sample<PHASE == 0>(sample_params(), L); need_sample = false; }
        const unsigned long long live_now = __ballot(have_pixel);
        if (dbg_timers) dbg_tm[7] += __builtin_amdgcn_s_memtime() - t_refill;
        if (live_now == 0ull) break;
        if (wdbg) {
            if (exhausted && dbg_tex == 0ull) dbg_tex = __builtin_amdgcn_s_memrealtime();
            dbg_iters++;
            if (__popcll(live_now) <= sparse_max) { dbg_coop_iters++; dbg_coop_rays += (uint32_t)__popcll(live_now); }
        }

        const int steps = (boost > 0 && __popcll(live_now) > sparse_max && !(MID && s_q[8 * myx + 5] != 0u && __ballot(have_pixel && ccls == 6) != 0ull)) ? 1 + boost : 1;
        for (int x = 0; x < steps; x++) {
            bool sel = have_pixel;
            if (x > 0) {
                const uint32_t heavy_thr = (uint32_t)((chain_cfg >> kChainHeavyThr.shift) & kChainHeavyThr.mask);
                const bool heavy = have_pixel && pix_rays > heavy_thr * (uint32_t)(L.s - chunk * P.spw + 2);
                const unsigned long long hm = __ballot(heavy);
                if (hm == 0ull) break;
                const int h = (int)__popcll(hm);
                const int hr = (int)__builtin_amdgcn_mbcnt_hi((uint32_t)(hm >> 32), __builtin_amdgcn_mbcnt_lo((uint32_t)hm, 0u));
                const int start = h > kSparseRays ? ((x - 1) * kSparseRays) % h : 0;
                int d = hr - start;
                if (d < 0) d += h;
                sel = heavy && d < kSparseRays;
            }
            if (sel) { nrays++; pix_rays++; }
            if (x > 0 || steps == 1) __builtin_amdgcn_s_setprio(3); else __builtin_amdgcn_s_setprio(0);
            f3 sample;
            const bool done = trace_rays<false, DBG, (LEAN & 1) != 0, (LEAN & 2) ? ((LEAN & 32) ? 4 : ((LEAN & 16) ? 2 : 1)) : 0, (LEAN & 8) != 0>(P, S, L, sel, -1, cull, groups_done, boxes_done, sample, sparse_max, dbg_timers ? dbg_tm : nullptr, (cfg & kCfgSingleRay) != 0);
            if (dbg_timers) { dbg_tm[x > 0 ? 9 : 8] += 1ull; }
            finish(done && sel, steps > 1, sample);
        }
    }

    if (PHASE == 1 && poison_at != ~0u && iter_no <= poison_at) poison_rows(P, (size_t)blockIdx.x * blockDim.x + threadIdx.x, (size_t)gridDim.x * blockDim.x);
    if (DBG && P.counters) {
        atomicAdd(&P.counters->rays, (unsigned long long)nrays);
        atomicAdd(&P.counters->prim_tests, (unsigned long long)nrays * (unsigned long long)P.n);
        atomicAdd(&P.counters->exec_tests, (unsigned long long)groups_done * 4ull);
        atomicAdd(&P.counters->box_tests, (unsigned long long)boxes_done);
    }
    if (wdbg) atomicMax(wdbg + 65536ull * 8 - 1, (unsigned long long)dbg_maxpix);
    if (wdbg && (threadIdx.x & 63) == 0) {
        unsigned long long* w = wdbg + ((size_t)blockIdx.x * (blockDim.x >> 6) + (threadIdx.x >> 6)) * 8;
        w[0] = dbg_t0; w[1] = dbg_tex; w[2] = __builtin_amdgcn_s_memrealtime();
        w[3] = dbg_iters; w[4] = dbg_coop_iters; w[5] = dbg_coop_rays;
        w[6] = ((unsigned long long)__builtin_amdgcn_s_getreg((31 << 11) | 20) << 32) | (unsigned)__builtin_amdgcn_s_getreg((31 << 11) | 4);
        w[7] = 1;
        for (int k = 0; k < 8; k++) atomicAdd(wdbg + 65534ull * 8 + k, dbg_tm[k]);
        if (dbg_coop_iters >= 2000ull) {
            for (int k = 0; k < 8; k++) atomicAdd(wdbg + 65532ull * 8 + k, dbg_tm[k]);
            for (int k = 0; k < 4; k++) atomicAdd(wdbg + 65531ull * 8 + k, dbg_tm[10 + k]);
            atomicAdd(wdbg + 65531ull * 8 + 4, dbg_coop_iters); atomicAdd(wdbg + 65531ull * 8 + 5, 1ull);
            atomicAdd(wdbg + 65531ull * 8 + 6, __builtin_amdgcn_s_memtime() - dbg_t0c);
        }
        atomicAdd(wdbg + 65533ull * 8 + 0, dbg_tm[8]); atomicAdd(wdbg + 65533ull * 8 + 1, dbg_tm[9]);
    }
}

}

namespace {
__global__ void __launch_bounds__(256) k_sum_chunks(const RtSphereParams P) {
    const size_t px = (size_t)blockIdx.x * 256 + threadIdx.x;
    if (px >= (size_t)P.part.local_rows * P.nx) return;
    const float* src = reinterpret_cast<const float*>(P.partial) + px * P.chunks * 3;
    f3 col = F3(src[0], src[1], src[2]);
    for (int c = 1; c < P.chunks; c++) col = col + F3(src[3 * c], src[3 * c + 1], src[3 * c + 2]);
    const f3 out = col / (float)P.ns;
    float* dst = reinterpret_cast<float*>(P.fb) + px * 3;
    dst[0] = out.x; dst[1] = out.y; dst[2] = out.z;
}
}

constexpr size_t kStaticLds = 1024;
constexpr size_t kLdsPerCu = 160 * 1024 - kStaticLds;
static size_t lds_bytes(int n_padded, int n, bool with_fb, int scene = 0, int waves = kWavesPerWg, bool onepass = false) {
    const size_t test_data = (size_t)(n_padded + n_padded / kSphereGroup) * 16 + (size_t)(n_padded / kSphereGroup) * 48 + (size_t)rt_cell_f4(n_padded / kSphereGroup) * 16;
    const size_t scratch = (size_t)waves * ws_total(onepass);
    if (scene == 1) return scratch;
    if (scene == 2) return test_data + (size_t)n_padded * 4 + scratch;
    return test_data + (size_t)n_padded * 16 + (size_t)n_padded * 12 +
           (size_t)((n + 3) & ~3) * 4 + (with_fb ? (size_t)kThreads * 3 * 4 : 0) + scratch;
}

static int scene_form(const RtSphereParams& p, bool onepass) {
    if (p.global_scene) return 1;
    return lds_bytes(p.n_padded, p.n, false, 0, kWavesPerWg, onepass) <= kLdsPerCu ? 0 : 2;
}

template <typename... Params, typename... Args>
static hipError_t launch_with_lds(void (*kern)(Params...), dim3 grid, dim3 block, size_t lds, hipStream_t stream, const Args&... args) {
    if (lds > 64 * 1024) {
        const hipError_t e = hipFuncSetAttribute(reinterpret_cast<const void*>(kern), hipFuncAttributeMaxDynamicSharedMemorySize, (int)lds);
        if (e != hipSuccess) return e;
    }
    hipLaunchKernelGGL(kern, grid, block, lds, stream, args...);
    return hipGetLastError();
}

static hipError_t order_pixels_by_cost(const RtSphereParams& q, hipStream_t stream) {
    hipLaunchKernelGGL(k_order_by_cost<0>, dim3(kOrderBlocks), dim3(kThreads), 0, stream, q);
    hipLaunchKernelGGL(k_order_by_cost<1>, dim3(kOrderBlocks), dim3(kThreads), 0, stream, q);
    return hipGetLastError();
}

#if defined(RT_MODE_PARITY)
hipError_t rt_order_pixels_by_cost(const RtSphereParams& q, hipStream_t stream) { return order_pixels_by_cost(q, stream); }
size_t rt_sphere_kernel_lds_bytes(int n_padded, int n) {
    return lds_bytes(n_padded, n, false, 2, 8) + kStaticLds;
}
hipError_t rt_launch_guides_spheres(const RtSphereParams& p, const RtGuidePlanes& g, hipStream_t stream) {
    const int scene = scene_form(p, false);
    const auto kern = scene == 0 ? k_guides_spheres<0> : (scene == 1 ? k_guides_spheres<1> : k_guides_spheres<2>);
    const unsigned long long total = (unsigned long long)((p.nx + 7) / 8) * ((p.part.local_rows + 7) / 8) * 64ull;
    const dim3 grid((unsigned)((total + kThreads - 1) / kThreads));
    return launch_with_lds(kern, grid, dim3(kThreads), lds_bytes(p.n_padded, p.n, false, scene, 0), stream, p, g);
}
hipError_t rt_launch_rays_spheres(const RtSphereParams& p, const RtRayBatch& b, bool any, hipStream_t stream) {
    if (b.n <= 0) return hipSuccess;
    const int scene = scene_form(p, false);
    using Kern = void (*)(const RtSphereParams, const RtRayBatch);
    const Kern kerns[2][3] = { { k_rays_spheres<0, false>, k_rays_spheres<1, false>, k_rays_spheres<2, false> },
                               { k_rays_spheres<0, true>, k_rays_spheres<1, true>, k_rays_spheres<2, true> } };
    const size_t lds = lds_bytes(p.n_padded, p.n, false, scene, 0);
    int dev = 0, cus = 256;
    if (hipGetDevice(&dev) == hipSuccess) (void)hipDeviceGetAttribute(&cus, hipDeviceAttributeMultiprocessorCount, dev);
    const unsigned per_cu = lds * 2 <= kLdsPerCu ? 2u : 1u;
    const unsigned tiles = ((unsigned)b.n + kThreads - 1) / kThreads;
    const dim3 grid(std::min(tiles, (unsigned)cus * per_cu));
    return launch_with_lds(kerns[any ? 1 : 0][scene], grid, dim3(kThreads), lds, stream, p, b);
}
#endif

constexpr int kLeanBasic = 1 << 0, kLeanOneList = 1 << 1, kLeanSixWaves = 1 << 2, kLeanAxes3 = 1 << 3, kLeanWords2 = 1 << 4, kLeanWords4 = 1 << 5;
using KindsFull = std::integer_sequence<int, 1, 3, 7, 11, 15, 19, 27, 35, 43>;
using KindsChunked = std::integer_sequence<int, 1, 3, 7>;
using KindsHybrid = std::integer_sequence<int, 1, 35, 43>;
using KindsStamped = std::integer_sequence<int, 3>;

template <int... LEANS>
constexpr bool in_kinds(std::integer_sequence<int, LEANS...>, int lean) { return ((lean == LEANS) || ...); }
constexpr bool built(int scene, bool chunked, int lean) {
    if (lean == 0) return true;
    if (scene == 0) return chunked ? in_kinds(KindsChunked{}, lean) : in_kinds(KindsFull{}, lean);
    return scene == 2 && !chunked && in_kinds(KindsHybrid{}, lean);
}
constexpr bool folded_built(int phase, int cls, bool chunked, bool dbg, int scene, int lean) {
    return phase == 2 && cls == 2 && !chunked && !dbg && scene == 0 && in_kinds(KindsFull{}, lean);
}
constexpr int clip_lean(int scene, bool chunked, int lean) {
    return built(scene, chunked, lean) ? lean : (built(scene, chunked, lean & kLeanBasic) ? (lean & kLeanBasic) : 0);
}

enum class SpherePlanError { None, Mid, Tune };
constexpr int kFirstSamples = 2;

struct SpherePlan {
    SpherePlanError error = SpherePlanError::None;
    SphereFrame frame = SphereFrame::PlainSingle;
    bool legacy = false;
    int coop_below = -1;
    int cull = 1;
    int scene = 0;
    bool chunked = false;
    int lean = 0;
    int lean_dbg = 0;
    int form = kSphereFormGeneral;
    int threads = kThreads;
    size_t lds = 0;
    unsigned blocks = 1, blocks_y = 1;
    unsigned cls_blocks = 1;
    uint32_t stride = 1;
    uint32_t stride1 = 1;
    int cfg = 0, cfg1 = 0, chain_cfg = 0, caps = 0;
    bool sum_chunks = false;
};

enum { kTuneChainEvery, kTuneChainWaves, kTuneHeavyThr, kTuneChainLists, kTuneBoost, kTuneChainPixels, kTuneList0, kTuneList1, kTuneList2, kTuneFields };
constexpr int kCapsNoTiers = caps_list(0).put(4) | caps_list(1).put(4) | caps_list(2).put(4) | caps_list(3).put(4);

static SpherePlan plan_spheres(const RtSphereParams& p, int variant, const RtSwitches& sw, int cus) {
    SpherePlan pl;
    const int cb_bits = (variant >> 16) & 0xFF;
    pl.legacy = cb_bits != 0 && cb_bits != 255;
    pl.cull = ((variant >> 26) & 1) ? 0 : 1;
    const size_t tile_lds = lds_bytes(p.n_padded, p.n, true, 0, kWavesPerWg);
    if (((variant & 0xFF) == 1 || pl.legacy) && !p.global_scene && tile_lds <= kLdsPerCu) {
        pl.frame = SphereFrame::Tiles;
        pl.coop_below = cb_bits == 0 ? -1 : (cb_bits == 255 ? -2 : cb_bits);
        pl.lds = tile_lds;
        pl.blocks = (p.nx + 8 * kWavesPerWg - 1) / (8 * kWavesPerWg);
        pl.blocks_y = (p.part.local_rows + 7) / 8;
        return pl;
    }
    pl.chunked = p.chunks > 1;
    int lean = 0;
    if (!p.global_scene && p.basic_materials && sw.basic) {
        const int n_small_groups = p.n_groups - p.n_big_groups;
        lean = kLeanBasic;
        if (pl.cull && p.cell_on != 0 && n_small_groups >= 1 && n_small_groups <= 128 && sw.onepass) {
            lean |= kLeanOneList;
            if (n_small_groups > 64) lean |= kLeanWords4;
            else if (n_small_groups > 32) lean |= kLeanWords2;
            if (p.box_shared_axis != 2) lean |= kLeanAxes3;
        }
    }
    lean = clip_lean(0, pl.chunked, lean);
    auto two_dispatch = [&](int order, bool enough_samples) {
        return order == 0 && p.order && p.px_state && p.px_rays && p.chunks == 1 && p.rng_mode == RT_RNG_REFERENCE_STREAM && enough_samples &&
               p.nx <= 65535 && p.part.local_rows <= 65535;
    };
    int order_mode = (variant >> 24) & 3;
    if (p.wave_dbg != nullptr || p.counters != nullptr) {
        pl.lean_dbg = (in_kinds(KindsStamped{}, lean) && p.counters == nullptr && sw.wave_debug_light && two_dispatch(order_mode, p.ns >= 8)) ? lean : 0;
        lean = pl.lean_dbg;
    }
    int waves = kWavesPerWg;
    pl.scene = scene_form(p, (lean & kLeanOneList) != 0);
    if (pl.scene == 2) {
        lean = clip_lean(2, pl.chunked, lean);
        if (lds_bytes(p.n_padded, p.n, false, 2, 16, (lean & kLeanOneList) != 0) > kLdsPerCu) waves = 8;
    }
    int default_wgs = 1;
    if ((lean & (kLeanOneList | kLeanWords2 | kLeanWords4)) == kLeanOneList && sw.lean6_pixels > 0 && (long long)p.nx * p.part.local_rows >= sw.lean6_pixels &&
        2 * (lds_bytes(p.n_padded, p.n, false, 0, 12, true) + kStaticLds) <= (size_t)160 * 1024) { lean |= kLeanSixWaves; waves = 12; default_wgs = 2; }
    pl.lean = lean;
    pl.threads = 64 * waves;
    pl.lds = lds_bytes(p.n_padded, p.n, false, pl.scene, waves, (lean & kLeanOneList) != 0);
    int wg_per_cu = (variant >> 8) & 0xFF;
    if (wg_per_cu == 0) wg_per_cu = default_wgs;
    const long long total_px = (long long)((p.nx + 7) / 8) * ((p.part.local_rows + 7) / 8) * 64;
    const long long useful = (total_px + pl.threads - 1) / pl.threads;
    pl.blocks = (unsigned)std::max(1ll, std::min((long long)cus * wg_per_cu, useful));
    pl.cls_blocks = (unsigned)((total_px + kThreads - 1) / kThreads);
    if (order_mode == 0 && ((pl.scene == 2 && !sw.hybrid_two) || pl.scene == 1)) order_mode = 2;
    if (order_mode != 1 && total_px > 64) pl.stride = rt_coprime_stride((unsigned long long)total_px);
    const bool resume = p.acc_first > 0 && p.acc_state && p.acc_rays;
    const bool reuse = !resume && p.cost_rays != nullptr && p.cost_samples >= kFirstSamples && p.wave_dbg == nullptr;
    if (pl.scene == 1) pl.frame = SphereFrame::GlobalSingle;
    else if (two_dispatch(order_mode, p.ns >= 8 || resume)) pl.frame = resume ? SphereFrame::TwoDispatchResume : (reuse ? SphereFrame::OrderedSingle : SphereFrame::TwoDispatch);
    else if ((order_mode == 0 || order_mode == 3) && p.order != nullptr) pl.frame = SphereFrame::ClassifiedSingle;
    else pl.frame = SphereFrame::PlainSingle;
    pl.sum_chunks = pl.chunked;

    if (sw.mid_waves < 0 || sw.mid_waves > 12 || sw.mid_cap < 1 || sw.mid_cap > 64) { pl.error = SpherePlanError::Mid; return pl; }
    const int pb = (variant >> 27) & 7;
    int sparse_max = 4 + 4 * ((variant >> 30) & 3);
    if (cb_bits == 255) sparse_max = 0;
    const int boost = (pb == 7 || cb_bits == 255) ? 0 : (pb == 0 ? 1 : pb);
    int t[kTuneFields] = { 1, waves == 16 ? 3 : (waves >= 10 ? 2 : 1), 8, kChainClasses, boost, kSparseRays, 1, 4, 4 };
    if (sw.tune) {
        t[kTuneChainWaves] = waves == 16 ? 3 : 1;
        for (int i = 0; i < sw.tune->n; i++) t[i] = sw.tune->v[i];
        const int lo[kTuneFields] = { 1, 0, 1, 0, 0, 1, 1, 1, 1 }, hi[kTuneFields] = { 255, waves, 255, 15, 255, 15, 15, 15, 15 };
        for (int i = 0; i < kTuneFields; i++)
            if (t[i] < lo[i] || t[i] > hi[i]) { pl.error = SpherePlanError::Tune; return pl; }
    }
    pl.chain_cfg = kChainEvery.put(t[kTuneChainEvery]) | kChainWaves.put(t[kTuneChainWaves]) | kChainPixels.put(t[kTuneChainPixels]) | kChainHeavyThr.put(t[kTuneHeavyThr]) |
                   kChainLists.put(t[kTuneChainLists]);
    const int mid_waves = (p.xcd_queues == kXcdQueues && pl.blocks < (unsigned)kXcdQueues) ? 0 : sw.mid_waves;
    pl.caps = caps_list(0).put(t[kTuneList0]) | caps_list(1).put(t[kTuneList1]) | caps_list(2).put(t[kTuneList2]) | caps_list(3).put(t[kTuneChainPixels]) |
              kCapsMidWaves.put(mid_waves) | kCapsMidCap.put(sw.mid_cap);
    pl.cfg = (pl.cull ? kCfgCull : 0) | (sw.chain_single ? kCfgChainSingle : 0) | (sw.single_ray ? kCfgSingleRay : 0) | kCfgPool.put((sw.pool / 4) & kCfgPool.mask) |
             kCfgBoost.put(t[kTuneBoost]) | kCfgSparseMax.put(sparse_max) | (sw.wave_debug_light ? kCfgDbgLight : 0);
    pl.stride1 = p.p1_tile_major == 1 ? 1u : pl.stride;
    pl.cfg1 = pl.cfg;
    const bool default_constants = pl.cfg == kDefaultCfg && pl.chain_cfg == default_chain_cfg((pl.lean & kLeanSixWaves) != 0) && pl.caps == kDefaultCaps;
    pl.form = sphere_frame_form(pl.frame, p, sw, folded_built(2, 2, pl.chunked, false, pl.scene, pl.lean), default_constants);
    if (p.p1_tile_major == 2 && total_px > 512) {
        pl.stride1 = rt_coprime_stride((unsigned long long)total_px >> 3);
        pl.cfg1 |= kCfgP1Segments;
    }
    return pl;
}

template <int PHASE, int CLS, bool CHUNKED, bool DBG, int SCENE, int LEAN = 0> struct SphereQueueForm {};

template <int PHASE, int CLS, bool CHUNKED, bool DBG, int SCENE, int LEAN>
static hipError_t launch_sphere_queue(SphereQueueForm<PHASE, CLS, CHUNKED, DBG, SCENE, LEAN>, const RtSphereParams& q, const SpherePlan& pl, hipStream_t stream,
                                      uint32_t stride, int cfg, int caps) {
    const int form = (PHASE == 2 && CLS == 2) ? pl.form : kSphereFormGeneral;
    auto launch_form = [&](auto tag) -> hipError_t {
        void (*kern)(const RtSphereParams, uint32_t, int, int, int, decltype(tag)) = k_render_spheres_queue<PHASE, CLS, CHUNKED, DBG, SCENE, LEAN>;
        return launch_with_lds(kern, dim3(pl.blocks), dim3(pl.threads), pl.lds, stream, q, stride, cfg, pl.chain_cfg, caps, tag);
    };
    hipError_t e;
    if constexpr (folded_built(PHASE, CLS, CHUNKED, DBG, SCENE, LEAN)) {
        e = form == kSphereFormDefault ? launch_form(FormTag<kSphereFormDefault>{}) : launch_form(FormTag<kSphereFormGeneral>{});
    } else {
        if (form != kSphereFormGeneral) return hipErrorInvalidValue;
        e = launch_form(FormTag<kSphereFormGeneral>{});
    }
    rt_note_launch(RT_KERNEL_SPHERE_QUEUE, PHASE, CLS, CHUNKED, DBG, SCENE, LEAN, pl.threads, pl.blocks);
    if (PHASE == 2 && CLS == 2) rt_note_sphere_form(form);
    return e;
}

template <int PHASE, int CLS, bool CHUNKED, bool DBG, int SCENE, int... LEANS, typename Go>
static bool launch_kind_of(std::integer_sequence<int, LEANS...>, int lean, Go&& go, hipError_t& e) {
    return ((lean == LEANS && ((e = go(SphereQueueForm<PHASE, CLS, CHUNKED, DBG, SCENE, LEANS>{})), true)) || ...);
}

template <int PHASE, int CLS, bool CHUNKED>
static hipError_t launch_queue_form(const SpherePlan& pl, const RtSphereParams& q, hipStream_t stream, uint32_t stride, int cfg, int caps = kCapsNoTiers) {
    const bool counting = q.wave_dbg != nullptr || q.counters != nullptr;
    auto go = [&](auto form) -> hipError_t { return launch_sphere_queue(form, q, pl, stream, stride, cfg, caps); };
    hipError_t e = hipErrorInvalidValue;
    if (pl.scene == 1) {
        if constexpr (PHASE == 0 && CLS == 0) e = counting ? go(SphereQueueForm<0, 0, CHUNKED, true, 1>{}) : go(SphereQueueForm<0, 0, CHUNKED, false, 1>{});
        return e;
    }
    if (counting && q.counters == nullptr && pl.scene == 0 && !CHUNKED && PHASE != 0 && launch_kind_of<PHASE, CLS, false, true, 0>(KindsStamped{}, pl.lean_dbg, go, e)) return e;
    if (counting) return pl.scene == 2 ? go(SphereQueueForm<PHASE, CLS, CHUNKED, true, 2>{}) : go(SphereQueueForm<PHASE, CLS, CHUNKED, true, 0>{});
    if (pl.lean == 0) return pl.scene == 2 ? go(SphereQueueForm<PHASE, CLS, CHUNKED, false, 2>{}) : go(SphereQueueForm<PHASE, CLS, CHUNKED, false, 0>{});
    if (pl.scene == 0 && !CHUNKED) launch_kind_of<PHASE, CLS, false, false, 0>(KindsFull{}, pl.lean, go, e);
    if (pl.scene == 0 && CHUNKED) launch_kind_of<PHASE, CLS, true, false, 0>(KindsChunked{}, pl.lean, go, e);
    if (pl.scene == 2 && !CHUNKED) launch_kind_of<PHASE, CLS, false, false, 2>(KindsHybrid{}, pl.lean, go, e);
    return e;
}

hipError_t RT_LAUNCH_NAME(const RtSphereParams& p, int variant, const RtSwitches& sw, hipStream_t stream) {
    if (!p.self) return hipErrorInvalidValue;
    int dev = 0, cus = 256;
    if (hipGetDevice(&dev) == hipSuccess) (void)hipDeviceGetAttribute(&cus, hipDeviceAttributeMultiprocessorCount, dev);
    const SpherePlan pl = plan_spheres(p, variant, sw, cus);
    auto wait_fb = [&]() -> hipError_t {
        if (!p.poison_fb) return hipSuccess;
        hipLaunchKernelGGL(k_poison_fb, dim3(512), dim3(256), 0, stream, p);
        return hipGetLastError();
    };
    hipError_t e;
    if (pl.frame == SphereFrame::Tiles) {
        if ((e = wait_fb()) != hipSuccess) return e;
        e = launch_with_lds(pl.legacy ? k_render_spheres_tiles<true> : k_render_spheres_tiles<false>, dim3(pl.blocks, pl.blocks_y), dim3(kThreads), pl.lds, stream, p, pl.coop_below, pl.cull);
        rt_note_launch(RT_KERNEL_SPHERE_TILES, 0, pl.legacy ? 1 : 0, 0, 0, 0, 0, kThreads, pl.blocks * pl.blocks_y);
        return e;
    }
    if (!p.queue) return hipErrorInvalidValue;
    if ((e = hipMemsetAsync(p.queue, 0, 256, stream)) != hipSuccess) return e;
    if (pl.error == SpherePlanError::Tune)
        fprintf(stderr, "rt error: RT_TUNE=%s out of range (chain_every 1..255, chain_waves 0..%d, heavy_thr 1..255, n_chain 0..15, boost 0..255, "
                        "chain_pixels 1..15, chain_pixels of list 0 / 1 / 2 1..15)\n", sw.tune->text.c_str(), kWavesPerWg);
    if (pl.error != SpherePlanError::None) return hipErrorInvalidValue;
    if (pl.frame == SphereFrame::TwoDispatch || pl.frame == SphereFrame::TwoDispatchResume || pl.frame == SphereFrame::OrderedSingle) {
        RtSphereParams q = p;
        if (pl.frame == SphereFrame::TwoDispatchResume) {
            q.px_state = p.acc_state; q.px_rays = p.acc_rays; q.s_split = p.acc_first;
            e = wait_fb();
        } else if (pl.frame == SphereFrame::OrderedSingle) {
            q.s_split = 0;
            e = wait_fb();
        } else {
            q.phase = 1; q.s_split = kFirstSamples;
            e = launch_queue_form<1, 0, false>(pl, q, stream, pl.stride1, pl.cfg1);
        }
        if (e != hipSuccess) return e;
        if ((e = hipMemsetAsync(p.queue, 0, sizeof(uint32_t) * kXcdQueues * kXcdQueueWords, stream)) != hipSuccess) return e;
        if ((e = order_pixels_by_cost(q, stream)) != hipSuccess) return e;
        q.phase = 2;
        if (sw.wave_debug_phase) q.wave_dbg = nullptr;
        return launch_queue_form<2, 2, false>(pl, q, stream, pl.stride, pl.cfg, pl.caps);
    }
    const bool classified = pl.frame == SphereFrame::ClassifiedSingle;
    if (classified) {
        e = launch_with_lds(pl.scene == 2 ? k_classify_spheres<2> : k_classify_spheres<0>, dim3(pl.cls_blocks), dim3(kThreads), pl.lds, stream, p);
        if (e != hipSuccess) return e;
    }
    if ((e = wait_fb()) != hipSuccess) return e;
    if (classified) e = pl.chunked ? launch_queue_form<0, 1, true>(pl, p, stream, pl.stride, pl.cfg) : launch_queue_form<0, 1, false>(pl, p, stream, pl.stride, pl.cfg);
    else e = pl.chunked ? launch_queue_form<0, 0, true>(pl, p, stream, pl.stride, pl.cfg) : launch_queue_form<0, 0, false>(pl, p, stream, pl.stride, pl.cfg);
    if (e != hipSuccess) return e;
    if (pl.sum_chunks) {
        const size_t npx = (size_t)p.part.local_rows * p.nx;
        hipLaunchKernelGGL(k_sum_chunks, dim3((unsigned)((npx + 255) / 256)), dim3(256), 0, stream, p);
    }
    return hipGetLastError();
}
```

cuda-raytracing-optimized_amd/csrc/rt_params.h:

```cpp
#pragma once

#include <hip/hip_runtime.h>
#include <stdint.h>

#include <optional>
#include <string>

#include "../../include/rt_types.h"
#include "../../include/rt_api.h"

constexpr int kSphereGroupShift = 4;
constexpr int kSphereGroup = 1 << kSphereGroupShift;
constexpr int kCellCount = 64;
constexpr int kCellWordsMax = 8;
__host__ __device__ inline int rt_cell_words(int n_groups) { const int w = (n_groups + 31) / 32; return w <= kCellWordsMax ? w : 0; }
__host__ __device__ inline int rt_cell_f4(int n_groups) { return (6 * kCellCount * rt_cell_words(n_groups)) / 4; }

struct RtPartition {
    int32_t stripe_rows;
    int32_t rank;
    int32_t world;
    int32_t local_rows;
};

struct RtCounters {
    unsigned long long rays;
    unsigned long long prim_tests;
    unsigned long long node_visits;
    unsigned long long shadow_rays;
    unsigned long long exec_tests;
    unsigned long long box_tests;
    unsigned long long ref_stats[RT_STAT_COUNT];
};

struct RtSphereParams {
    rt_camera cam;
    int32_t nx, ny, ns, max_depth;
    int32_t n;
    int32_t n_padded;
    int32_t n_groups;
    int32_t n_big_groups;
    int32_t n_big;
    const float4* spheres;
    const float*  rad;
    int32_t fb_global_rows;
    const struct RtSphereParams* self;
    int32_t basic_materials;
    int32_t global_scene;
    const float4* groups;
    float cull_cx, cull_cy, cull_cz, cull_radius, cull_k1, cull_k2, cull_k3, cull_coord_max;
    float box_shared_lo, box_shared_hi;
    int32_t box_shared_axis;
    float pair_k0;
    int32_t cell_on;
    int32_t cell_axes;
    float cell_scale[3], cell_off[3];
    float ubox[6];
    const float4* mat_color;
    const int32_t* mat_type;
    const int32_t* orig;
    const int32_t* slot_of;
    rt_vec3* fb;
    RtPartition part;
    int32_t sky;
    int32_t rr;
    int32_t rng_mode;
    float   t_min;
    RtCounters* counters;
    uint32_t* queue;
    unsigned long long* wave_dbg;
    uint32_t* order;
    int32_t spw;
    int32_t chunks;
    rt_vec3* partial;
    int32_t phase;
    int32_t s_split;
    int32_t chain_top_thr;
    int32_t poison_fb;
    float4* px_state;
    uint32_t* px_rays;
    float4* ord_state;
    uint32_t* ord_rays;
    float4* ord_rec;
    int32_t xcd_queues;
    int32_t p1_tile_major;
    float4* acc_state;
    uint32_t* acc_rays;
    int32_t acc_first;
    uint32_t* cost_rays;
    int32_t cost_samples;
};
constexpr int kXcdQueueWords = 64;
constexpr int kXcdQueues = 8;
__host__ __device__ inline uint32_t rt_xcd_of_pixel(uint32_t local_row, uint32_t nx, uint32_t column) {
#ifdef RT_XCD_PLAIN
    return ((local_row * nx + column) >> 5) & 7u;
#else
    return ((((local_row * nx + column) >> 5) * 2654435761u) >> 29) & 7u;
#endif
}

struct RtMeshParams {
    rt_camera cam;
    int32_t nx, ny, ns, max_depth;
    const rt_triangle* tris;
    const float4* bvh4;
    const float* bvh_axis;
    const float4* leaf_tri;
    const uint32_t* leaf_ofs;
    uint32_t first_leaf;
    uint32_t nppl;
    int32_t leaf_sentinels_trailing;
    int32_t lean_ok;
    rt_bbox bounds;
    const rt_material* materials;
    const float* const* tex_data;
    const int32_t* tex_width;
    const int32_t* tex_height;
    rt_vec3* fb;
    RtPartition part;
    int32_t sky;
    int32_t nee;
    int32_t rr;
    int32_t rng_mode;
    float   t_min;
    rt_sphere light;
    rt_vec3 lightColor;
    int32_t floor_on;
    rt_plane floor;
    RtCounters* counters;
    uint32_t* queue;
    unsigned long long* dbg;
    int32_t s_split;
    float4* px_state;
    uint32_t* px_rays;
    uint32_t* order;
    float4* ord_state;
    uint32_t* ord_rays;
    float4* ord_rec;
    int32_t xcd_queues;
    int32_t p1_segments;
    float4* acc_state;
    int32_t acc_first;
};

struct BitField {
    int shift, mask;
    constexpr int put(int value) const { return value << shift; }
    constexpr int get(int word) const { return (word >> shift) & mask; }
};

template <typename T>
__device__ __forceinline__ T rt_cold_arg(size_t offset) {
    unsigned long long base = (unsigned long long)__builtin_amdgcn_kernarg_segment_ptr();
    asm volatile("" : "+s"(base));
    return *reinterpret_cast<const __attribute__((address_space(4))) T*>(base + offset);
}

size_t rt_sphere_kernel_lds_bytes(int n_padded, int n);
hipError_t rt_order_pixels_by_cost(const RtSphereParams& q, hipStream_t stream);

struct RtTune {
    std::string text;
    int n = 0;
    int v[9] = {};
};

struct RtSwitches {
    bool xcd_queues = true;
    bool ord_packed = true;
    int p1_tile = 2;
    std::optional<std::string> wave_debug;
    bool fb_direct = false;
    bool fb_poison = true;
    bool box_cells = true;
    bool compact_leaves = true;
    bool ext_fb_no_register = false;
    bool cleanup_device_reset = false;
    int cost_reuse = 1;
    int top_thr = 384;
    bool basic = true;
    bool onepass = true;
    long long lean6_pixels = 2600000;
    bool hybrid_two = false;
    int mid_waves = 0, mid_cap = 16;
    bool chain_single = true;
    bool single_ray = true;
    int pool = 4;
    bool wave_debug_light = false;
    bool wave_debug_phase = false;
    std::optional<RtTune> tune;
    bool mesh_lean = true;
    bool mesh_tile_order = false;
    bool mesh_two = true;
    int mesh_split = 2;
    int mesh_heavy = 5;
    int mesh_rounds = 2;
    bool mesh_rev = false;
    int mesh_chain_thr = 448;
    int mesh_chain_lanes = 6;
    int mesh_chain_frac = 8;
    std::optional<std::string> mesh_diag_file;
};
RtSwitches rt_read_switches();

inline uint32_t rt_coprime_stride(unsigned long long n) {
    auto gcd = [](unsigned long long a, unsigned long long b) { while (b) { const unsigned long long t = a % b; a = b; b = t; } return a; };
    unsigned long long cand = (unsigned long long)((double)n * 0.6180339887) | 1ull;
    while (gcd(cand, n) != 1ull) cand += 2;
    return (uint32_t)(cand % n);
}

hipError_t rt_launch_spheres_parity(const RtSphereParams& p, int variant, const RtSwitches& sw, hipStream_t stream);
hipError_t rt_launch_spheres_fast(const RtSphereParams& p, int variant, const RtSwitches& sw, hipStream_t stream);
hipError_t rt_launch_mesh_parity(const RtMeshParams& p, int variant, const RtSwitches& sw, hipStream_t stream);
hipError_t rt_launch_mesh_fast(const RtMeshParams& p, int variant, const RtSwitches& sw, hipStream_t stream);
void rt_note_launch(int family, int phase, int cls, int chunked, int dbg, int scene, int lean, int threads, unsigned blocks);
void rt_note_sphere_form(int form);

struct RtGuidePlanes {
    float* albedo;
    float* normal;
    float* depth;
    int32_t* prim;
    int32_t* nodes;
};
hipError_t rt_launch_guides_spheres(const RtSphereParams& p, const RtGuidePlanes& g, hipStream_t stream);
hipError_t rt_launch_guides_mesh(const RtMeshParams& p, const RtGuidePlanes& g, hipStream_t stream);

struct RtRayBatch {
    const float* org;
    const float* dir;
    const float* t_min;
    const float* t_max;
    float* t;
    int32_t* prim;
    float* normal;
    float* uv;
    int32_t* nodes;
    uint8_t* occluded;
    int32_t n;
    float t_min_default;
};
hipError_t rt_launch_rays_spheres(const RtSphereParams& p, const RtRayBatch& b, bool any, hipStream_t stream);
hipError_t rt_launch_rays_mesh(const RtMeshParams& p, const RtRayBatch& b, bool any, hipStream_t stream);
```

cuda-raytracing-optimized_amd/csrc/rt_renderer.hip:

```cpp
#include <hip/hip_runtime.h>

#include <algorithm>
#include <array>
#include <chrono>
#include <climits>
#include <cmath>
#include <cstdio>
#include <cstdlib>
#include <cstring>
#include <functional>
#include <string>
#include <vector>

#include "../../include/rt_api.h"
#include "rt_params.h"
#include "rt_scene_layout.h"
#include "rt_denoise.h"
#include "rt_accumulate.h"
#include "rt_preview.h"
#include "rt_display.h"
#include "rt_update.h"
#include "rt_build.h"

namespace {

#define HIP_CHECK(expr) hip_check((expr), #expr, __FILE__, __LINE__)

void hip_check(hipError_t result, const char* func, const char* file, int line) {
    if (result != hipSuccess) {
        fprintf(stderr, "HIP error = %s at %s:%d '%s' \n", hipGetErrorString(result), file, line, func);
        (void)hipDeviceReset();
        exit(99);
    }
}

[[noreturn]] void rt_fail(const char* msg, const char* who = "") {
    fprintf(stderr, "rt error: %s%s\n", who, msg);
    exit(99);
}

template <typename T>
T* dev_alloc(std::vector<void*>& owned, size_t count) {
    void* p = nullptr;
    HIP_CHECK(hipMalloc(&p, count * sizeof(T)));
    owned.push_back(p);
    return static_cast<T*>(p);
}

template <typename T>
void dev_release(std::vector<void*>& owned, T*& p) {
    if (!p) return;
    owned.erase(std::find(owned.begin(), owned.end(), static_cast<void*>(p)));
    HIP_CHECK(hipFree(p));
    p = nullptr;
}

void dev_release_all(std::vector<void*>& owned) {
    for (void* p : owned) HIP_CHECK(hipFree(p));
    owned.clear();
}

template <typename T>
T* upload(std::vector<void*>& owned, const std::vector<T>& v) {
    if (v.empty()) return nullptr;
    T* p = dev_alloc<T>(owned, v.size());
    HIP_CHECK(hipMemcpy(p, v.data(), v.size() * sizeof(T), hipMemcpyHostToDevice));
    return p;
}

struct DeviceState {
    int device = 0;
    std::vector<void*> owned;
    hipStream_t stream = nullptr;
    hipEvent_t ev_start = nullptr, ev_stop = nullptr;
    hipEvent_t ev_upd_start = nullptr, ev_upd_stop = nullptr;
    hipEvent_t ev_reb_start = nullptr, ev_reb_stop = nullptr;
    RtSphereParams* d_params = nullptr;
    RtSphereParams* h_params = nullptr;
    float4* d_spheres = nullptr;
    float* d_rad = nullptr;
    float4* d_mat_color = nullptr;
    int32_t* d_mat_type = nullptr;
    float4* d_groups = nullptr;
    int32_t* d_orig = nullptr;
    int32_t* d_slot_of = nullptr;
    rt_triangle* d_tris = nullptr;
    float4* d_bvh = nullptr;
    float* d_bvh_axis = nullptr;
    float4* d_leaf_tri = nullptr;
    uint32_t* d_leaf_ofs = nullptr;
    rt_material* d_materials = nullptr;
    rt_triangle* d_tris_alt = nullptr;
    int32_t* d_old_slot = nullptr;
    uint32_t* d_build_work = nullptr;
    size_t build_words = 0;
    float** d_tex_data = nullptr;
    int32_t* d_tex_width = nullptr;
    int32_t* d_tex_height = nullptr;
    rt_vec3* d_fb = nullptr;
    size_t fb_rows = 0;
    RtCounters* d_counters = nullptr;
    uint32_t* d_queue = nullptr;
    unsigned long long* d_wave_dbg = nullptr;
    uint32_t* d_order = nullptr;
    rt_vec3* d_partial = nullptr;
    size_t partial_bytes = 0;
    float4* d_px_state = nullptr;
    uint32_t* d_px_rays = nullptr;
    float4* d_ord_state = nullptr;
    uint32_t* d_ord_rays = nullptr;
    float4* d_ord_rec = nullptr;
    uint32_t* d_cost_rays = nullptr;
    int cost_samples = 0;
    std::array<int, 11> cost_key = {};
    float4* d_acc_state = nullptr;
    uint32_t* d_acc_rays = nullptr;
    void* d_guide[5] = { nullptr, nullptr, nullptr, nullptr, nullptr };
};

constexpr size_t kGuideBytes[5] = { 12, 12, 4, 4, 4 };

struct RenderContext {
    bool initialised = false;
    bool is_spheres = false;
    int nx = 0, ny = 0, max_depth = 0;
    rt_camera cam;
    rt_render_options opt;
    rt_vec3* h_fb = nullptr;
    rt_vec3* h_ext = nullptr;
    bool ext_registered = false;
    SphereLayout sphere;
    MeshLayout mesh;
    std::vector<DeviceState> devs;
    rt_render_stats stats;
    int prog_samples = 0;
    int camera_moves = 0;
    int scene_edits = 0;
    bool refit_stale = false;
    double update_ms = 0.0;
    double rebuild_ms = 0.0;
    double guides_ms = 0.0;
    double denoise_ms = 0.0;
    double accumulate_ms = 0.0;
    double preview_ms = 0.0;
    double display_ms = 0.0;
    double rays_ms = 0.0;
};

struct PassState {
    int device = -1;
    size_t npix = 0;
    std::vector<void*> owned;
    float* d_guide[4] = { nullptr, nullptr, nullptr, nullptr };
    rt_vec3* d_in = nullptr;
    rt_vec3* d_out = nullptr;
    hipEvent_t ev_start = nullptr, ev_stop = nullptr;
};

struct DenoiseState : PassState {
    float4* d_rec = nullptr;
    float4* d_col[2] = { nullptr, nullptr };
};

struct AccumulateState : PassState {
    float* d_history = nullptr;
    float4* d_rec[2] = { nullptr, nullptr };
    int newest = 0;
    int frames = 0;
    rt_camera prev_cam;
};

RenderContext g_ctx;
struct PreviewState : PassState {
    float* d_history = nullptr;
    float* d_variance = nullptr;
    float4* d_rec[2] = { nullptr, nullptr };
    float2* d_mom[2] = { nullptr, nullptr };
    float4* d_col[2] = { nullptr, nullptr };
    int newest = 0;
    int frames = 0;
    rt_camera prev_cam;
};

struct DisplayState : PassState {
    uint32_t* d_rgba = nullptr;
    uint32_t* d_words = nullptr;
    uint32_t h_words[RT_DISPLAY_BINS + 2] = {};
    bool adapted = false;
    float last_exposure = 1.0f;
};

enum { kRayOrg = 0, kRayDir, kRayTMin, kRayTMax, kRayT, kRayPrim, kRayNormal, kRayUv, kRayNodes, kRayOccluded, kRayBuffers };
constexpr size_t kRayBytes[kRayBuffers] = { 12, 12, 4, 4, 4, 4, 12, 8, 4, 1 };
constexpr int kRayChunk = RT_RAY_CHUNK;
struct RayState {
    int device = -1;
    std::vector<void*> owned;
    char* d_buf[kRayBuffers] = {};
    size_t cap[kRayBuffers] = {};
    hipEvent_t ev_start = nullptr, ev_stop = nullptr;
};

DenoiseState g_denoise;
AccumulateState g_accumulate;
PreviewState g_preview;
DisplayState g_display;
RayState g_rays;

void reset_display() {
    g_display.adapted = false;
    memset(g_display.h_words, 0, RT_DISPLAY_BINS * sizeof(uint32_t));
}

std::vector<int32_t> g_launches;
int g_launch_device = 0, g_launch_fp = 0;
int g_sphere_form = RT_SPHERE_FORM_NONE;

void default_options(rt_render_options* o, int spheres) {
    memset(o, 0, sizeof *o);
    o->sky = spheres ? RT_SKY_GRADIENT : RT_SKY_CONST_GREY;
    o->nee = spheres ? 0 : 1;
    o->rr = spheres ? 0 : 1;
    o->t_min = spheres ? 0.001f : 0.01f;
    o->rng = RT_RNG_REFERENCE_STREAM;
    o->fp = RT_FP_PARITY;
    o->light.center.e[0] = (float)52.514355;
    o->light.center.e[1] = (float)715.686951;
    o->light.center.e[2] = (float)-272.620972;
    o->light.radius = 50.0f;
    o->lightColor.e[0] = o->lightColor.e[1] = o->lightColor.e[2] = 20.0f;
    o->stripe_rows = 8;
    o->num_devices = 0;
    o->part_rank = 0;
    o->part_world = 1;
}

void free_device(DeviceState& d) {
    HIP_CHECK(hipSetDevice(d.device));
    if (d.stream) HIP_CHECK(hipStreamSynchronize(d.stream));
    dev_release_all(d.owned);
    if (d.h_params) HIP_CHECK(hipHostFree(d.h_params));
    if (d.ev_start) HIP_CHECK(hipEventDestroy(d.ev_start));
    if (d.ev_stop) HIP_CHECK(hipEventDestroy(d.ev_stop));
    if (d.ev_upd_start) HIP_CHECK(hipEventDestroy(d.ev_upd_start));
    if (d.ev_upd_stop) HIP_CHECK(hipEventDestroy(d.ev_upd_stop));
    if (d.ev_reb_start) HIP_CHECK(hipEventDestroy(d.ev_reb_start));
    if (d.ev_reb_stop) HIP_CHECK(hipEventDestroy(d.ev_reb_stop));
    if (d.stream) HIP_CHECK(hipStreamDestroy(d.stream));
    d = DeviceState();
}

template <typename State>
void free_pass(State& n) {
    if (n.device >= 0) {
        int current = 0;
        HIP_CHECK(hipGetDevice(&current));
        HIP_CHECK(hipSetDevice(n.device));
        HIP_CHECK(hipDeviceSynchronize());
        dev_release_all(n.owned);
        if (n.ev_start) HIP_CHECK(hipEventDestroy(n.ev_start));
        if (n.ev_stop) HIP_CHECK(hipEventDestroy(n.ev_stop));
        HIP_CHECK(hipSetDevice(current));
    }
    n = State();
}

int local_rows_of(int ny, int sr, int rank, int world) {
    int rows = 0;
    const int nstripes = (ny + sr - 1) / sr;
    for (int k = rank; k < nstripes; k += world) rows += std::min(sr, ny - k * sr);
    return rows;
}

void fetch_refit() {
    RenderContext& c = g_ctx;
    if (!c.refit_stale) return;
    const DeviceState& d = c.devs[0];
    int current = 0;
    HIP_CHECK(hipGetDevice(&current));
    HIP_CHECK(hipSetDevice(d.device));
    HIP_CHECK(hipMemcpy(c.mesh.bvh.data(), d.d_bvh, c.mesh.bvh.size() * sizeof(float4), hipMemcpyDeviceToHost));
    HIP_CHECK(hipMemcpy(c.mesh.bvh_axis.data(), d.d_bvh_axis, c.mesh.bvh_axis.size() * sizeof(float), hipMemcpyDeviceToHost));
    if (!c.mesh.leaf_tri.empty()) HIP_CHECK(hipMemcpy(c.mesh.leaf_tri.data(), d.d_leaf_tri, c.mesh.leaf_tri.size() * sizeof(float4), hipMemcpyDeviceToHost));
    HIP_CHECK(hipSetDevice(current));
    c.refit_stale = false;
}

void upload_sphere_arrays(DeviceState& d) {
    const RenderContext& c = g_ctx;
    dev_release(d.owned, d.d_spheres); dev_release(d.owned, d.d_rad); dev_release(d.owned, d.d_mat_color); dev_release(d.owned, d.d_mat_type);
    dev_release(d.owned, d.d_groups); dev_release(d.owned, d.d_orig); dev_release(d.owned, d.d_slot_of);
    d.d_spheres = upload(d.owned, c.sphere.spheres);
    d.d_rad = upload(d.owned, c.sphere.rad);
    d.d_mat_color = upload(d.owned, c.sphere.mat_color);
    d.d_mat_type = upload(d.owned, c.sphere.mat_type);
    d.d_groups = upload(d.owned, c.sphere.groups);
    d.d_orig = upload(d.owned, c.sphere.orig);
    d.d_slot_of = upload(d.owned, c.sphere.slot_of);
}

void setup_devices() {
    RenderContext& c = g_ctx;
    fetch_refit();
    free_pass(g_denoise);
    free_pass(g_accumulate);
    free_pass(g_preview);
    free_pass(g_display);
    free_pass(g_rays);
    for (DeviceState& d : c.devs) free_device(d);
    c.devs.clear();
    int count = 0;
    HIP_CHECK(hipGetDeviceCount(&count));
    int nd = c.opt.num_devices <= 0 ? 1 : c.opt.num_devices;
    if (nd > RT_MAX_DEVICES) rt_fail("too many devices");
    int current = 0;
    HIP_CHECK(hipGetDevice(&current));
    for (int k = 0; k < nd; k++) {
        DeviceState d;
        d.device = (c.opt.num_devices <= 0) ? current : c.opt.devices[k];
        if (d.device < 0 || d.device >= count) rt_fail("device index out of range");
        HIP_CHECK(hipSetDevice(d.device));
        HIP_CHECK(hipStreamCreateWithFlags(&d.stream, hipStreamNonBlocking));
        HIP_CHECK(hipEventCreate(&d.ev_start));
        HIP_CHECK(hipEventCreate(&d.ev_stop));
        HIP_CHECK(hipEventCreate(&d.ev_upd_start));
        HIP_CHECK(hipEventCreate(&d.ev_upd_stop));
        HIP_CHECK(hipEventCreate(&d.ev_reb_start));
        HIP_CHECK(hipEventCreate(&d.ev_reb_stop));
        if (c.is_spheres) {
            d.d_params = dev_alloc<RtSphereParams>(d.owned, 1);
            HIP_CHECK(hipHostMalloc((void**)&d.h_params, sizeof(RtSphereParams), hipHostMallocDefault));
            upload_sphere_arrays(d);
        } else {
            d.d_tris = upload(d.owned, c.mesh.tris);
            d.d_bvh = upload(d.owned, c.mesh.bvh);
            d.d_bvh_axis = upload(d.owned, c.mesh.bvh_axis);
            d.d_leaf_tri = upload(d.owned, c.mesh.leaf_tri);
            d.d_leaf_ofs = upload(d.owned, c.mesh.leaf_ofs);
            d.d_materials = upload(d.owned, c.mesh.materials);
            if (!c.mesh.tex.empty()) {
                std::vector<float*> ptrs;
                for (const std::vector<float>& t : c.mesh.tex) ptrs.push_back(upload(d.owned, t));
                d.d_tex_data = upload(d.owned, ptrs);
                d.d_tex_width = upload(d.owned, c.mesh.tex_w);
                d.d_tex_height = upload(d.owned, c.mesh.tex_h);
            }
        }
        const int world = c.opt.part_world * nd, rank = c.opt.part_rank * nd + k;
        d.fb_rows = (size_t)local_rows_of(c.ny, c.opt.stripe_rows, rank, world);
        if (d.fb_rows > 0) {
            const size_t pixels = d.fb_rows * c.nx;
            const size_t padded = (size_t)((c.nx + 7) / 8) * ((d.fb_rows + 7) / 8) * 64;
            d.d_fb = dev_alloc<rt_vec3>(d.owned, pixels);
            d.d_order = dev_alloc<uint32_t>(d.owned, 3 * padded);
        }
        d.d_counters = dev_alloc<RtCounters>(d.owned, 1);
        HIP_CHECK(hipMemset(d.d_counters, 0, sizeof(RtCounters)));
        d.d_queue = dev_alloc<uint32_t>(d.owned, (size_t)kXcdQueues * kXcdQueueWords);
        HIP_CHECK(hipMemset(d.d_queue, 0, sizeof(uint32_t) * kXcdQueues * kXcdQueueWords));
        c.devs.push_back(d);
    }
    HIP_CHECK(hipSetDevice(c.devs[0].device));
    g_rays.device = c.devs[0].device;
    HIP_CHECK(hipEventCreate(&g_rays.ev_start));
    HIP_CHECK(hipEventCreate(&g_rays.ev_stop));
    HIP_CHECK(hipSetDevice(current));
}

void validate_options(const rt_render_options& o) {
    if (o.stripe_rows <= 0 || (o.stripe_rows % 8) != 0) rt_fail("stripe_rows must be a positive multiple of 8");
    if (o.part_world < 1 || o.part_rank < 0 || o.part_rank >= o.part_world) rt_fail("bad part_rank/part_world");
    if (o.num_devices < 0 || o.num_devices > RT_MAX_DEVICES) rt_fail("bad num_devices");
    if (!(o.t_min >= 0.0f)) rt_fail("t_min must be >= 0");
    if (o.sky != RT_SKY_CONST_GREY && o.sky != RT_SKY_GRADIENT) rt_fail("bad sky mode");
    if (o.rng != RT_RNG_REFERENCE_STREAM && o.rng != RT_RNG_COUNTER) rt_fail("bad rng mode");
    if (o.fp != RT_FP_PARITY && o.fp != RT_FP_FAST) rt_fail("bad fp mode");
}

void common_init(const rt_camera& cam, rt_vec3** fb, int nx, int ny, int maxDepth) {
    RenderContext& c = g_ctx;
    if (nx <= 0 || ny <= 0 || (long long)nx * ny > (1ll << 30)) rt_fail("bad image size");
    if (!fb) rt_fail("fb out-parameter is null");
    c.nx = nx; c.ny = ny;
    c.max_depth = maxDepth > 255 ? 255 : maxDepth;
    c.cam = cam;
    HIP_CHECK(hipHostMalloc((void**)&c.h_fb, (size_t)nx * ny * sizeof(rt_vec3), hipHostMallocDefault));
    memset(c.h_fb, 0, (size_t)nx * ny * sizeof(rt_vec3));
    *fb = c.h_fb;
    memset(&c.stats, 0, sizeof c.stats);
    c.prog_samples = 0;
    setup_devices();
    c.initialised = true;
}

void build_sphere_scene(const char* fn, const rt_sphere* spheres, const rt_material* materials, int n) {
    RenderContext& c = g_ctx;
    for (int k = 0; k < n; k++)
        if (materials[k].type < RT_DIFFUSE || materials[k].type >= RT_MATERIAL_TYPE_COUNT) rt_fail(": bad material type", fn);
    c.sphere = layout_spheres(spheres, materials, n, rt_read_switches().box_cells);
    c.sphere.scene.global_scene = rt_sphere_kernel_lds_bytes(c.sphere.scene.n_padded, n) > 160 * 1024 ? 1 : 0;
    if (c.sphere.scene.n_padded > (1 << 24)) rt_fail(": more than 16 M sphere slots", fn);
}

void cleanup_impl() {
    RenderContext& c = g_ctx;
    free_pass(g_denoise);
    free_pass(g_accumulate);
    free_pass(g_preview);
    free_pass(g_display);
    free_pass(g_rays);
    for (DeviceState& d : c.devs) free_device(d);
    c.devs.clear();
    if (c.h_ext) { if (c.ext_registered) HIP_CHECK(hipHostUnregister(c.h_ext)); c.h_ext = nullptr; c.ext_registered = false; }
    if (c.h_fb) HIP_CHECK(hipHostFree(c.h_fb));
    c = RenderContext();
}

}

void rt_note_launch(int family, int phase, int cls, int chunked, int dbg, int scene, int lean, int threads, unsigned blocks) {
    const int32_t rec[RT_LAUNCH_WORDS] = { family, phase, cls, chunked, dbg, scene, lean, threads, (int32_t)blocks, g_launch_device, g_launch_fp };
    g_launches.insert(g_launches.end(), rec, rec + RT_LAUNCH_WORDS);
}
void rt_note_sphere_form(int form) { g_sphere_form = g_sphere_form == RT_SPHERE_FORM_NONE ? form : std::min(g_sphere_form, form); }

extern "C" {

int rtApiVersion(void) { return RT_API_VERSION; }

int rtStructSizes(int32_t* out, int n) {
    const int32_t sizes[RT_SIZEOF_COUNT] = {
        (int32_t)sizeof(rt_render_options), (int32_t)sizeof(rt_render_stats), (int32_t)sizeof(rt_camera), (int32_t)sizeof(rt_sphere),
        (int32_t)sizeof(rt_material), (int32_t)sizeof(rt_triangle), (int32_t)sizeof(rt_bvh_node), (int32_t)sizeof(rt_mesh),
        (int32_t)sizeof(rt_kernel_scene), (int32_t)sizeof(rt_stexture), (int32_t)sizeof(rt_plane), (int32_t)sizeof(rt_bbox), (int32_t)sizeof(rt_vec3) };
    for (int k = 0; k < n && k < RT_SIZEOF_COUNT; k++) out[k] = sizes[k];
    return RT_SIZEOF_COUNT;
}

int rtLastSphereForm(void) { return g_sphere_form; }

int rtLastLaunches(int32_t* out, int cap) {
    const int count = (int)(g_launches.size() / RT_LAUNCH_WORDS);
    const int n = std::min(count, std::max(cap, 0));
    if (out && n > 0) memcpy(out, g_launches.data(), (size_t)n * RT_LAUNCH_WORDS * sizeof(int32_t));
    return count;
}

int rtDeviceCount(void) {
    int count = 0;
    if (hipGetDeviceCount(&count) != hipSuccess) return 0;
    return count;
}

void getDefaultRenderOptions(rt_render_options* opt, int is_sphere_scene) {
    if (!opt) return;
    default_options(opt, is_sphere_scene);
}

void initRenderer(const rt_kernel_scene sc, const rt_camera cam, rt_vec3** fb, int nx, int ny, int maxDepth) {
    if (g_ctx.initialised) cleanup_impl();
    RenderContext& c = g_ctx;
    if (!sc.m || !sc.m->tris || !sc.m->bvh || !sc.materials) rt_fail("initRenderer: null scene pointers");
    if (sc.m->numBvhNodes < 4 || (sc.m->numBvhNodes & 1)) rt_fail("initRenderer: numBvhNodes must be even and >= 4");
    if (sc.numPrimitivesPerLeaf <= 0) rt_fail("initRenderer: numPrimitivesPerLeaf must be positive");
    const uint32_t first_leaf = (uint32_t)sc.m->numBvhNodes / 2;
    if ((unsigned long long)first_leaf * (unsigned)sc.numPrimitivesPerLeaf > sc.m->numTris)
        rt_fail("initRenderer: leaves * numPrimitivesPerLeaf exceeds numTris (traversal would read out of bounds)");
    if (first_leaf > (1u << 30)) rt_fail("initRenderer: BVH deeper than the 32-bit traversal bit-stack");
    c.is_spheres = false;
    default_options(&c.opt, 0);
    for (size_t k = 0; k < sc.m->numTris; k++)
        if (sc.m->tris[k].meshID >= sc.numMaterials && !std::isinf(sc.m->tris[k].v[0].e[0])) rt_fail("initRenderer: triangle meshID out of range");
    for (int t = 0; t < sc.numTextures; t++)
        if (!sc.textures[t].data || sc.textures[t].width <= 0 || sc.textures[t].height <= 0) rt_fail("initRenderer: bad texture");
    for (int k = 0; k < sc.numMaterials; k++)
        if (sc.materials[k].texId != -1 && (sc.materials[k].texId < 0 || sc.materials[k].texId >= sc.numTextures)) rt_fail("initRenderer: material texId out of range");
    c.mesh = layout_mesh(sc);
    common_init(cam, fb, nx, ny, maxDepth);
}

void initRendererSpheres(const rt_sphere* spheres, const rt_material* materials, int n,
                         const rt_camera cam, rt_vec3** fb, int nx, int ny, int maxDepth) {
    if (g_ctx.initialised) cleanup_impl();
    RenderContext& c = g_ctx;
    if (!spheres || !materials || n <= 0) rt_fail("initRendererSpheres: empty scene");
    c.is_spheres = true;
    default_options(&c.opt, 1);
    build_sphere_scene("initRendererSpheres", spheres, materials, n);
    common_init(cam, fb, nx, ny, maxDepth);
}

void setRenderOptions(const rt_render_options* opt) {
    RenderContext& c = g_ctx;
    if (!c.initialised) rt_fail("setRenderOptions before init");
    if (!opt) rt_fail("setRenderOptions: null");
    validate_options(*opt);
    const rt_render_options old = c.opt;
    c.opt = *opt;
    bool relayout = old.stripe_rows != opt->stripe_rows || old.part_rank != opt->part_rank ||
                    old.part_world != opt->part_world || old.num_devices != opt->num_devices;
    for (int k = 0; k < RT_MAX_DEVICES && !relayout; k++) relayout = old.devices[k] != opt->devices[k];
    if (relayout) setup_devices();
    c.prog_samples = 0;
    g_accumulate.frames = 0;
    g_preview.frames = 0;
    reset_display();
}

}

namespace {

RtPartition partition_of(int k) {
    const RenderContext& c = g_ctx;
    const int nd = (int)c.devs.size();
    RtPartition part;
    part.stripe_rows = c.opt.stripe_rows;
    part.rank = c.opt.part_rank * nd + k;
    part.world = c.opt.part_world * nd;
    part.local_rows = (int)c.devs[k].fb_rows;
    return part;
}

RtPartition whole_image_partition() {
    RtPartition part;
    part.stripe_rows = g_ctx.opt.stripe_rows;
    part.rank = 0;
    part.world = 1;
    part.local_rows = g_ctx.ny;
    return part;
}

RtSphereParams sphere_params(const DeviceState& d, const RtPartition& part) {
    const RenderContext& c = g_ctx;
    RtSphereParams p = c.sphere.scene;
    p.cam = c.cam; p.nx = c.nx; p.ny = c.ny;
    p.spheres = d.d_spheres; p.rad = d.d_rad; p.mat_color = d.d_mat_color; p.mat_type = d.d_mat_type;
    p.groups = d.d_groups; p.orig = d.d_orig; p.slot_of = d.d_slot_of;
    p.part = part; p.sky = c.opt.sky; p.t_min = c.opt.t_min;
    return p;
}

RtMeshParams mesh_params(const DeviceState& d, const RtPartition& part) {
    const RenderContext& c = g_ctx;
    RtMeshParams p = c.mesh.scene;
    p.cam = c.cam; p.nx = c.nx; p.ny = c.ny;
    p.tris = d.d_tris; p.bvh4 = d.d_bvh; p.bvh_axis = d.d_bvh_axis;
    p.materials = d.d_materials;
    p.tex_data = d.d_tex_data; p.tex_width = d.d_tex_width; p.tex_height = d.d_tex_height;
    p.part = part; p.sky = c.opt.sky; p.t_min = c.opt.t_min;
    p.floor_on = c.opt.floor ? 1 : 0;
    return p;
}

void launch_guides(const DeviceState& d, const RtPartition& part, const RtGuidePlanes& g) {
    HIP_CHECK(g_ctx.is_spheres ? rt_launch_guides_spheres(sphere_params(d, part), g, d.stream) : rt_launch_guides_mesh(mesh_params(d, part), g, d.stream));
}

constexpr size_t kWaveDbgWords = (size_t)65536 * 8;
unsigned long long* wave_debug_buffer(DeviceState& d) {
    if (!d.d_wave_dbg) d.d_wave_dbg = dev_alloc<unsigned long long>(d.owned, kWaveDbgWords);
    HIP_CHECK(hipMemsetAsync(d.d_wave_dbg, 0, kWaveDbgWords * sizeof(unsigned long long), d.stream));
    return d.d_wave_dbg;
}

void deliver_stripes(const DeviceState& d, const RtPartition& part, char* host, const char* dev, size_t px_bytes) {
    const RenderContext& c = g_ctx;
    const size_t row_bytes = (size_t)c.nx * px_bytes;
    const size_t stripe_bytes = (size_t)part.stripe_rows * row_bytes;
    const size_t full = d.fb_rows / part.stripe_rows, rem = d.fb_rows % part.stripe_rows;
    char* dst0 = host + (size_t)part.rank * stripe_bytes;
    if (part.world == 1) {
        HIP_CHECK(hipMemcpyAsync(dst0, dev, d.fb_rows * row_bytes, hipMemcpyDeviceToHost, d.stream));
        return;
    }
    if (full > 0)
        HIP_CHECK(hipMemcpy2DAsync(dst0, (size_t)part.world * stripe_bytes, dev, stripe_bytes, stripe_bytes, full, hipMemcpyDeviceToHost, d.stream));
    if (rem > 0)
        HIP_CHECK(hipMemcpyAsync(dst0 + full * (size_t)part.world * stripe_bytes, dev + full * stripe_bytes, rem * row_bytes, hipMemcpyDeviceToHost, d.stream));
}


enum { kCheckInit = 1, kCheckOut = 2, kCheckFlags = 4, kCheckSigmaZ = 8, kCheckFloor = 16 };
void check_pass_args(const char* fn, int which, const rt_vec3* out, int flags, float sigma_z) {
    const RenderContext& c = g_ctx;
    if ((which & kCheckInit) && !c.initialised) rt_fail(" before init", fn);
    if ((which & kCheckOut) && !out) rt_fail(": out is null", fn);
    if ((which & kCheckFlags) && (flags & ~(RT_DENOISE_DEMODULATE | RT_DENOISE_SAME_PRIM)) != 0) rt_fail(": unknown flag bits", fn);
    if ((which & kCheckSigmaZ) && (!std::isfinite(sigma_z) || !(sigma_z > 0.0f))) rt_fail(": sigma_z must be finite and positive", fn);
    if ((which & kCheckFloor) && c.is_spheres && c.opt.floor) rt_fail(": the floor plane is only defined for mesh scenes (kernel_scene.floor)", fn);
}

enum { kPassNoGuides = 1, kPassOwnOutput = 2, kPassNoUpload = 4 };
template <typename State, typename AllocOwn>
int begin_pass(State& n, const rt_vec3* in, AllocOwn alloc_own, int without = 0) {
    const RenderContext& c = g_ctx;
    if (!in) in = c.h_ext ? c.h_ext : c.h_fb;
    int current = 0;
    HIP_CHECK(hipGetDevice(&current));
    const DeviceState& d = c.devs[0];
    HIP_CHECK(hipSetDevice(d.device));
    const size_t npix = (size_t)c.nx * c.ny;
    if (n.device != d.device || n.npix != npix) {
        free_pass(n);
        HIP_CHECK(hipSetDevice(d.device));
        n.device = d.device; n.npix = npix;
        if (!(without & kPassNoGuides))
            for (int q = 0; q < 4; q++) n.d_guide[q] = dev_alloc<float>(n.owned, npix * kGuideBytes[q] / sizeof(float));
        n.d_in = dev_alloc<rt_vec3>(n.owned, npix);
        if (!(without & kPassOwnOutput)) n.d_out = dev_alloc<rt_vec3>(n.owned, npix);
        alloc_own();
        HIP_CHECK(hipEventCreate(&n.ev_start));
        HIP_CHECK(hipEventCreate(&n.ev_stop));
    }
    if (!(without & kPassNoUpload)) HIP_CHECK(hipMemcpyAsync(n.d_in, in, npix * sizeof(rt_vec3), hipMemcpyHostToDevice, d.stream));
    if (!(without & kPassNoGuides))
        launch_guides(d, whole_image_partition(), { n.d_guide[0], n.d_guide[1], n.d_guide[2], reinterpret_cast<int32_t*>(n.d_guide[3]), nullptr });
    return current;
}

template <typename Params>
Params pass_params(const PassState& n) {
    Params q;
    memset(&q, 0, sizeof q);
    q.cam = g_ctx.cam; q.nx = g_ctx.nx; q.ny = g_ctx.ny;
    q.albedo = n.d_guide[0]; q.normal = n.d_guide[1]; q.depth = n.d_guide[2]; q.prim = reinterpret_cast<const int32_t*>(n.d_guide[3]);
    q.in = n.d_in; q.out = n.d_out;
    return q;
}

struct PassCopy {
    void* host;
    const void* dev;
    size_t bytes;
};
double end_pass(const PassState& n, int current, rt_vec3* out, float* history = nullptr, const float* d_history = nullptr, float* variance = nullptr,
                const float* d_variance = nullptr, const PassCopy* own = nullptr, int n_own = 0) {
    const DeviceState& d = g_ctx.devs[0];
    HIP_CHECK(hipEventRecord(n.ev_stop, d.stream));
    if (out) HIP_CHECK(hipMemcpyAsync(out, n.d_out, n.npix * sizeof(rt_vec3), hipMemcpyDeviceToHost, d.stream));
    for (int k = 0; k < n_own; k++) HIP_CHECK(hipMemcpyAsync(own[k].host, own[k].dev, own[k].bytes, hipMemcpyDeviceToHost, d.stream));
    if (history) HIP_CHECK(hipMemcpyAsync(history, d_history, n.npix * sizeof(float), hipMemcpyDeviceToHost, d.stream));
    if (variance) HIP_CHECK(hipMemcpyAsync(variance, d_variance, n.npix * sizeof(float), hipMemcpyDeviceToHost, d.stream));
    HIP_CHECK(hipStreamSynchronize(d.stream));
    float ms = 0.0f;
    HIP_CHECK(hipEventElapsedTime(&ms, n.ev_start, n.ev_stop));
    HIP_CHECK(hipSetDevice(current));
    return (double)ms;
}

void parked_buffers(DeviceState& d, bool packed) {
    const size_t nx = (size_t)g_ctx.nx;
    const size_t pixels = d.fb_rows * nx;
    const size_t padded = ((nx + 7) / 8) * ((d.fb_rows + 7) / 8) * 64;
    if (!d.d_px_state) d.d_px_state = dev_alloc<float4>(d.owned, pixels);
    if (!d.d_px_rays) d.d_px_rays = dev_alloc<uint32_t>(d.owned, pixels);
    if (packed) {
        dev_release(d.owned, d.d_ord_state);
        dev_release(d.owned, d.d_ord_rays);
        if (!d.d_ord_rec) d.d_ord_rec = dev_alloc<float4>(d.owned, padded * 2);
    } else {
        dev_release(d.owned, d.d_ord_rec);
        if (!d.d_ord_state) d.d_ord_state = dev_alloc<float4>(d.owned, padded);
        if (!d.d_ord_rays) d.d_ord_rays = dev_alloc<uint32_t>(d.owned, padded);
    }
}

std::array<int, 11> cost_key_of(const RtPartition& part, bool with_camera) {
    const RenderContext& c = g_ctx;
    return { c.nx, c.ny, part.stripe_rows, part.rank, part.world, part.local_rows, c.max_depth, (int)c.opt.rr, (int)c.opt.rng, with_camera ? c.camera_moves : 0,
             c.scene_edits };
}

double finish_devices(hipEvent_t DeviceState::*start, hipEvent_t DeviceState::*stop, bool with_rows) {
    double ms_max = 0.0;
    for (DeviceState& d : g_ctx.devs) {
        if (with_rows && d.fb_rows == 0) continue;
        HIP_CHECK(hipSetDevice(d.device));
        HIP_CHECK(hipStreamSynchronize(d.stream));
        float ms = 0.0f;
        HIP_CHECK(hipEventElapsedTime(&ms, d.*start, d.*stop));
        ms_max = std::max(ms_max, (double)ms);
    }
    return ms_max;
}

void render_frame(int ns, int first, bool progressive) {
    RenderContext& c = g_ctx;
    const auto t0 = std::chrono::steady_clock::now();
    int current = 0;
    HIP_CHECK(hipGetDevice(&current));
    const int nd = (int)c.devs.size();
    const size_t row_bytes = (size_t)c.nx * sizeof(rt_vec3);
    int64_t samples = 0;
    int launches = 0;
    g_launches.clear();
    g_sphere_form = RT_SPHERE_FORM_NONE;
    g_launch_fp = c.opt.fp;
    const RtSwitches sw = rt_read_switches();

    for (int k = 0; k < nd; k++) {
        DeviceState& d = c.devs[k];
        if (d.fb_rows == 0) continue;
        HIP_CHECK(hipSetDevice(d.device));
        g_launch_device = d.device;
        const RtPartition part = partition_of(k);
        if (c.opt.counters) HIP_CHECK(hipMemsetAsync(d.d_counters, 0, sizeof(RtCounters), d.stream));
        int spw = ns, chunks = 1;
        if (c.is_spheres && c.opt.rng == RT_RNG_COUNTER && (c.opt.variant & 0xFF) == 0) {
            int want = c.opt.samples_per_item;
            if (want <= 0) {
                const long long pixels = std::max<long long>(1, (long long)d.fb_rows * c.nx);
                const long long max_chunks = std::max<long long>(1, (32ll << 20) / pixels);
                want = (int)std::max<long long>(4, (ns + max_chunks - 1) / max_chunks);
            }
            if (want < ns) { spw = want; chunks = (ns + want - 1) / want; }
        }
        const int vk = c.opt.variant & 0xFF, vcb = (c.opt.variant >> 16) & 0xFF;
        const bool fb_direct = c.is_spheres && c.max_depth > 0 && sw.fb_direct && vk == 0 && (vcb == 0 || vcb == 255) && chunks == 1 &&
                               (!c.h_ext || c.ext_registered);
        rt_vec3* const h_target = c.h_ext ? c.h_ext : c.h_fb;
        if (!fb_direct && d.fb_rows > 0) HIP_CHECK(hipMemsetAsync(d.d_fb, 0xFF, d.fb_rows * row_bytes, d.stream));
        HIP_CHECK(hipEventRecord(d.ev_start, d.stream));
        if (c.max_depth <= 0) {
            HIP_CHECK(hipMemsetAsync(d.d_fb, 0, d.fb_rows * row_bytes, d.stream));
        } else if (c.is_spheres) {
            RtSphereParams p = sphere_params(d, part);
            p.ns = ns; p.max_depth = c.max_depth;
            p.fb = d.d_fb;
            p.rr = c.opt.rr; p.rng_mode = c.opt.rng;
            p.counters = c.opt.counters ? d.d_counters : nullptr;
            p.queue = d.d_queue;
            p.order = d.d_order;
            p.spw = spw; p.chunks = chunks; p.partial = nullptr;
            const bool whole_pixels = c.opt.rng == RT_RNG_REFERENCE_STREAM && chunks == 1 && vk == 0 && (vcb == 0 || vcb == 255) && !p.global_scene;
            if (whole_pixels && (ns >= 8 || progressive)) parked_buffers(d, sw.ord_packed);
            p.phase = 0; p.s_split = 0; p.px_state = d.d_px_state; p.px_rays = d.d_px_rays; p.ord_state = d.d_ord_state; p.ord_rays = d.d_ord_rays;
            if (progressive) { p.acc_state = d.d_acc_state; p.acc_rays = d.d_acc_rays; p.acc_first = first; }
            if (whole_pixels && !progressive && sw.cost_reuse != 0 && ns <= RT_PROGRESSIVE_MAX_SAMPLES) {
                if (!d.d_cost_rays) {
                    d.d_cost_rays = dev_alloc<uint32_t>(d.owned, d.fb_rows * c.nx);
                    d.cost_samples = 0;
                }
                const std::array<int, 11> key = cost_key_of(part, sw.cost_reuse != 2);
                p.cost_rays = d.d_cost_rays;
                p.acc_rays = d.d_cost_rays;
                p.cost_samples = key == d.cost_key ? d.cost_samples : 0;
                d.cost_key = key;
                d.cost_samples = ns;
            }
            p.chain_top_thr = sw.top_thr;
            p.ord_rec = sw.ord_packed ? d.d_ord_rec : nullptr;
            p.xcd_queues = sw.xcd_queues ? kXcdQueues : 0;
            p.p1_tile_major = sw.p1_tile;
            if (chunks > 1) {
                const size_t sums = d.fb_rows * c.nx * (size_t)p.chunks;
                if (sums * sizeof(rt_vec3) > d.partial_bytes) {
                    dev_release(d.owned, d.d_partial);
                    d.d_partial = dev_alloc<rt_vec3>(d.owned, sums);
                    d.partial_bytes = sums * sizeof(rt_vec3);
                }
                p.partial = d.d_partial;
            }
            if (sw.wave_debug && !progressive) p.wave_dbg = wave_debug_buffer(d);
            if (c.opt.nee) rt_fail("runRenderer: next-event estimation is only defined for mesh scenes");
            if (c.opt.floor) rt_fail("runRenderer: the floor plane is only defined for mesh scenes (kernel_scene.floor)");
            if (fb_direct) {
                void* dp = nullptr;
                HIP_CHECK(hipHostGetDevicePointer(&dp, (void*)h_target, 0));
                p.fb = reinterpret_cast<rt_vec3*>(dp);
                p.fb_global_rows = 1;
                p.poison_fb = sw.fb_poison ? 1 : 0;
            }
            p.self = d.d_params;
            *d.h_params = p;
            HIP_CHECK(hipMemcpyAsync(d.d_params, d.h_params, sizeof(RtSphereParams), hipMemcpyHostToDevice, d.stream));
            HIP_CHECK(c.opt.fp == RT_FP_FAST ? rt_launch_spheres_fast(p, c.opt.variant, sw, d.stream)
                                             : rt_launch_spheres_parity(p, c.opt.variant, sw, d.stream));
            launches++;
        } else {
            RtMeshParams p = mesh_params(d, part);
            p.ns = ns; p.max_depth = c.max_depth;
            p.leaf_tri = sw.compact_leaves ? d.d_leaf_tri : nullptr; p.leaf_ofs = sw.compact_leaves ? d.d_leaf_ofs : nullptr;
            p.fb = d.d_fb;
            p.nee = c.opt.nee; p.rr = c.opt.rr; p.rng_mode = c.opt.rng;
            p.light = c.opt.light; p.lightColor = c.opt.lightColor;
            if (c.opt.floor && (c.opt.variant & 0xFF) == 1) rt_fail("runRenderer: the floor plane is not built into the tile-per-wave A/B kernel (variant 1)");
            p.counters = c.opt.counters ? d.d_counters : nullptr;
            p.queue = d.d_queue;
            if (c.opt.rng == RT_RNG_REFERENCE_STREAM && sw.mesh_two && !c.opt.counters && first == 0) parked_buffers(d, sw.ord_packed);
            p.s_split = 0; p.px_state = d.d_px_state; p.px_rays = d.d_px_rays; p.order = d.d_order; p.ord_state = d.d_ord_state; p.ord_rays = d.d_ord_rays;
            if (progressive) { p.acc_state = d.d_acc_state; p.acc_first = first; }
            p.ord_rec = sw.ord_packed ? d.d_ord_rec : nullptr;
            p.xcd_queues = sw.xcd_queues ? kXcdQueues : 0;
            p.p1_segments = sw.p1_tile == 2 ? 1 : 0;
            if (sw.wave_debug) p.dbg = wave_debug_buffer(d);
            HIP_CHECK(c.opt.fp == RT_FP_FAST ? rt_launch_mesh_fast(p, c.opt.variant, sw, d.stream)
                                             : rt_launch_mesh_parity(p, c.opt.variant, sw, d.stream));
            launches++;
        }
        HIP_CHECK(hipEventRecord(d.ev_stop, d.stream));

        if (!fb_direct) deliver_stripes(d, part, reinterpret_cast<char*>(h_target), reinterpret_cast<const char*>(d.d_fb), sizeof(rt_vec3));
        samples += (int64_t)d.fb_rows * c.nx * (ns - first);
    }

    const double kernel_ms = finish_devices(&DeviceState::ev_start, &DeviceState::ev_stop, true);
    rt_render_stats st;
    memset(&st, 0, sizeof st);
    for (int k = 0; k < nd; k++) {
        DeviceState& d = c.devs[k];
        if (d.fb_rows == 0) continue;
        HIP_CHECK(hipSetDevice(d.device));
        if (d.d_wave_dbg && sw.wave_debug) {
            std::vector<unsigned long long> h(kWaveDbgWords);
            HIP_CHECK(hipMemcpy(h.data(), d.d_wave_dbg, h.size() * sizeof(unsigned long long), hipMemcpyDeviceToHost));
            if (FILE* f = fopen(sw.wave_debug->c_str(), "wb")) { fwrite(h.data(), sizeof(unsigned long long), h.size(), f); fclose(f); }
            if (d.d_px_state && c.is_spheres) {
                std::vector<float> px((size_t)d.fb_rows * c.nx * 4);
                HIP_CHECK(hipMemcpy(px.data(), d.d_px_state, px.size() * sizeof(float), hipMemcpyDeviceToHost));
                const std::string path = *sw.wave_debug + ".px";
                if (FILE* f = fopen(path.c_str(), "wb")) { fwrite(px.data(), sizeof(float), px.size(), f); fclose(f); }
            }
        }
        if (c.opt.counters) {
            RtCounters h;
            HIP_CHECK(hipMemcpy(&h, d.d_counters, sizeof h, hipMemcpyDeviceToHost));
            st.rays += h.rays; st.prim_tests += h.prim_tests; st.node_visits += h.node_visits;
            st.exec_tests += h.exec_tests; st.shadow_rays += h.shadow_rays; st.box_tests += h.box_tests;
            for (int q = 0; q < RT_STAT_COUNT; q++) st.ref_stats[q] += h.ref_stats[q];
        }
    }
    HIP_CHECK(hipSetDevice(current));
    const auto t1 = std::chrono::steady_clock::now();
    st.kernel_ms = kernel_ms;
    st.total_ms = std::chrono::duration<double, std::milli>(t1 - t0).count();
    st.samples = samples;
    st.num_launches = launches;
    c.stats = st;
}

}

namespace {

bool env_flag(const char* name, bool dflt) {
    const char* v = getenv(name);
    return v ? v[0] != '0' : dflt;
}

bool env_one(const char* name) {
    const char* v = getenv(name);
    return v && v[0] == '1';
}

int env_int(const char* name, int dflt) {
    const char* v = getenv(name);
    return v ? atoi(v) : dflt;
}

std::optional<std::string> env_str(const char* name) {
    const char* v = getenv(name);
    if (!v) return std::nullopt;
    return std::string(v);
}

}

RtSwitches rt_read_switches() {
    RtSwitches s;
    s.xcd_queues = env_flag("RT_XCD_QUEUES", s.xcd_queues);
    s.ord_packed = env_flag("RT_ORD_PACKED", s.ord_packed);
    const int p1_tile = env_int("RT_P1_TILE", s.p1_tile);
    s.p1_tile = (p1_tile >= 0 && p1_tile <= 2) ? p1_tile : 0;
    s.wave_debug = env_str("RT_WAVE_DEBUG");

    s.fb_direct = env_flag("RT_FB_DIRECT", s.fb_direct);
    s.fb_poison = env_flag("RT_FB_POISON", s.fb_poison);
    s.box_cells = env_flag("RT_BOX_CELLS", s.box_cells);
    s.compact_leaves = env_flag("RT_COMPACT_LEAVES", s.compact_leaves);
    s.ext_fb_no_register = env_one("RT_EXT_FB_NO_REGISTER");
    s.cleanup_device_reset = env_one("RT_CLEANUP_DEVICE_RESET");
    const int cost_reuse = env_int("RT_COST_REUSE", s.cost_reuse);
    s.cost_reuse = (cost_reuse >= 0 && cost_reuse <= 2) ? cost_reuse : 1;

    const int top_thr = env_int("RT_TOP_THR", s.top_thr);
    if (top_thr >= 320) s.top_thr = top_thr;
    s.basic = env_flag("RT_BASIC", s.basic);
    s.onepass = env_flag("RT_ONEPASS", s.onepass);
    if (const auto v = env_str("RT_LEAN6_PIXELS")) s.lean6_pixels = atoll(v->c_str());
    s.hybrid_two = env_one("RT_HYBRID_TWO");
    if (const auto v = env_str("RT_MID")) sscanf(v->c_str(), "%d,%d", &s.mid_waves, &s.mid_cap);
    s.chain_single = env_flag("RT_CHAIN_SINGLE", s.chain_single);
    s.single_ray = env_flag("RT_SINGLE_RAY", s.single_ray);
    s.pool = env_int("RT_POOL", s.pool);
    s.wave_debug_light = env_one("RT_WAVE_DEBUG_LIGHT");
    s.wave_debug_phase = env_one("RT_WAVE_DEBUG_PHASE");
    if (const auto v = env_str("RT_TUNE")) {
        RtTune& t = s.tune.emplace();
        t.text = *v;
        t.n = std::max(0, sscanf(v->c_str(), "%d,%d,%d,%d,%d,%d,%d,%d,%d", &t.v[0], &t.v[1], &t.v[2], &t.v[3], &t.v[4], &t.v[5], &t.v[6], &t.v[7], &t.v[8]));
    }

    s.mesh_lean = env_flag("RT_MESH_LEAN", s.mesh_lean);
    const auto order = env_str("RT_MESH_ORDER");
    s.mesh_tile_order = order && (*order)[0] == 't';
    s.mesh_two = env_flag("RT_MESH_TWO", s.mesh_two);
    s.mesh_split = std::max(1, env_int("RT_MESH_SPLIT", s.mesh_split));
    s.mesh_heavy = env_int("RT_MESH_HEAVY", s.mesh_heavy);
    s.mesh_rounds = env_int("RT_MESH_ROUNDS", s.mesh_rounds);
    s.mesh_rev = env_one("RT_MESH_REV");
    s.mesh_chain_thr = std::max(17, env_int("RT_MESH_CHAIN_THR", s.mesh_chain_thr));
    s.mesh_chain_lanes = std::min(64, std::max(0, env_int("RT_MESH_CHAIN_LANES", s.mesh_chain_lanes)));
    s.mesh_chain_frac = env_int("RT_MESH_CHAIN_FRAC", s.mesh_chain_frac) & 0xF;
    s.mesh_diag_file = env_str("RT_MESH_DIAG_FILE");
    return s;
}

extern "C" {

void runRenderer(int ns, int tx, int ty) {
    (void)tx; (void)ty;
    RenderContext& c = g_ctx;
    if (!c.initialised) rt_fail("runRenderer before init");
    if (ns <= 0) rt_fail("runRenderer: ns must be positive");
    render_frame(ns, 0, false);
}

void runRendererProgressive(int ns, int tx, int ty) {
    (void)tx; (void)ty;
    RenderContext& c = g_ctx;
    if (!c.initialised) rt_fail("runRendererProgressive before init");
    if (ns <= 0) rt_fail("runRendererProgressive: ns must be positive");
    if (c.opt.rng != RT_RNG_REFERENCE_STREAM) rt_fail("runRendererProgressive: only the reference RNG stream accumulates (RT_RNG_COUNTER sums sample chunks)");
    if (c.opt.variant != 0) rt_fail("runRendererProgressive: only the default kernels (variant 0) continue a frame");
    if (ns > RT_PROGRESSIVE_MAX_SAMPLES - c.prog_samples) rt_fail("runRendererProgressive: total samples per pixel above RT_PROGRESSIVE_MAX_SAMPLES");
    int current = 0;
    HIP_CHECK(hipGetDevice(&current));
    for (DeviceState& d : c.devs) {
        if (d.fb_rows == 0 || d.d_acc_state) continue;
        HIP_CHECK(hipSetDevice(d.device));
        d.d_acc_state = dev_alloc<float4>(d.owned, d.fb_rows * c.nx);
        if (c.is_spheres) d.d_acc_rays = dev_alloc<uint32_t>(d.owned, d.fb_rows * c.nx);
    }
    HIP_CHECK(hipSetDevice(current));
    const int first = c.prog_samples;
    render_frame(first + ns, first, true);
    c.prog_samples = first + ns;
}

int rtProgressiveSamples(void) { return g_ctx.prog_samples; }

void rtResetProgressive(void) { g_ctx.prog_samples = 0; }

void setCamera(const rt_camera* cam) {
    RenderContext& c = g_ctx;
    if (!c.initialised) rt_fail("setCamera before init");
    if (!cam) rt_fail("setCamera: null");
    if (memcmp(&c.cam, cam, sizeof(rt_camera)) != 0) c.camera_moves++;
    c.cam = *cam;
    c.prog_samples = 0;
}

static void check_update(const char* fn, bool spheres) {
    const RenderContext& c = g_ctx;
    if (!c.initialised) rt_fail(" before init", fn);
    if (c.is_spheres != spheres) rt_fail(spheres ? " needs a sphere scene (initRendererSpheres)" : " needs a mesh scene (initRenderer)", fn);
}

static void launch_refit(const DeviceState& d) {
    RtRefitParams q;
    q.slots = d.d_tris; q.nodes = reinterpret_cast<float*>(d.d_bvh); q.axis = d.d_bvh_axis; q.leaf_rec = d.d_leaf_tri;
    q.first_leaf = g_ctx.mesh.scene.first_leaf; q.nppl = g_ctx.mesh.scene.nppl;
    HIP_CHECK(rt_launch_refit(q, d.stream));
}

static void scene_edited() {
    g_ctx.prog_samples = 0;
    g_ctx.scene_edits++;
}

void updateTriangles(int first, int count, const rt_triangle* tris) {
    RenderContext& c = g_ctx;
    check_update("updateTriangles", false);
    if (first < 0 || count < 0 || (size_t)first + (size_t)count > c.mesh.tris.size()) rt_fail("updateTriangles: [first, first + count) must lie inside the numTris of init");
    if (count == 0) return;
    if (!tris) rt_fail("updateTriangles: tris is null");
    const uint32_t first_leaf = c.mesh.scene.first_leaf;
    if ((first_leaf & (first_leaf - 1)) != 0) rt_fail("updateTriangles: the refit needs a tree whose number of leaves is a power of two");
    for (int k = 0; k < count; k++) {
        const bool sentinel = std::isinf(tris[k].v[0].e[0]);
        if (sentinel != std::isinf(c.mesh.tris[(size_t)first + k].v[0].e[0])) rt_fail("updateTriangles: a slot's sentinel state (isinf(v[0].x)) must not change");
        if (!sentinel && tris[k].meshID >= c.mesh.materials.size()) rt_fail("updateTriangles: triangle meshID out of range");
    }
    std::copy(tris, tris + count, c.mesh.tris.begin() + first);
    int current = 0;
    HIP_CHECK(hipGetDevice(&current));
    for (DeviceState& d : c.devs) {
        HIP_CHECK(hipSetDevice(d.device));
        HIP_CHECK(hipMemcpyAsync(d.d_tris + first, c.mesh.tris.data() + first, (size_t)count * sizeof(rt_triangle), hipMemcpyHostToDevice, d.stream));
        HIP_CHECK(hipEventRecord(d.ev_upd_start, d.stream));
        launch_refit(d);
        HIP_CHECK(hipEventRecord(d.ev_upd_stop, d.stream));
    }
    rt_bvh_node root;
    HIP_CHECK(hipSetDevice(c.devs[0].device));
    HIP_CHECK(hipMemcpyAsync(&root, reinterpret_cast<const char*>(c.devs[0].d_bvh) + sizeof(rt_bvh_node), sizeof root, hipMemcpyDeviceToHost, c.devs[0].stream));
    const double ms_max = finish_devices(&DeviceState::ev_upd_start, &DeviceState::ev_upd_stop, false);
    HIP_CHECK(hipSetDevice(current));
    c.mesh.scene.bounds.min = root.a;
    c.mesh.scene.bounds.max = root.b;
    c.refit_stale = true;
    c.update_ms = ms_max;
    scene_edited();
}

void updateMaterials(const rt_material* materials, int n) {
    RenderContext& c = g_ctx;
    check_update("updateMaterials", false);
    if (!materials) rt_fail("updateMaterials: materials is null");
    if (n != (int)c.mesh.materials.size()) rt_fail("updateMaterials: n must be the numMaterials of init");
    for (int k = 0; k < n; k++)
        if (materials[k].texId != -1 && (materials[k].texId < 0 || materials[k].texId >= (int)c.mesh.tex.size())) rt_fail("updateMaterials: material texId out of range");
    c.mesh.materials.assign(materials, materials + n);
    c.mesh.scene.lean_ok = mesh_lean_ok(c.mesh.materials);
    int current = 0;
    HIP_CHECK(hipGetDevice(&current));
    for (DeviceState& d : c.devs) {
        HIP_CHECK(hipSetDevice(d.device));
        if (n > 0) HIP_CHECK(hipMemcpy(d.d_materials, c.mesh.materials.data(), (size_t)n * sizeof(rt_material), hipMemcpyHostToDevice));
    }
    HIP_CHECK(hipSetDevice(current));
    scene_edited();
}

void updateSpheres(const rt_sphere* spheres, const rt_material* materials, int n) {
    RenderContext& c = g_ctx;
    check_update("updateSpheres", true);
    if (!spheres || !materials) rt_fail("updateSpheres: spheres and materials must not be null");
    if (n != c.sphere.scene.n) rt_fail("updateSpheres: n must be the n of init");
    build_sphere_scene("updateSpheres", spheres, materials, n);
    int current = 0;
    HIP_CHECK(hipGetDevice(&current));
    for (DeviceState& d : c.devs) {
        HIP_CHECK(hipSetDevice(d.device));
        upload_sphere_arrays(d);
    }
    HIP_CHECK(hipSetDevice(current));
    scene_edited();
}

int getMeshBvh(rt_bvh_node* nodes, int cap, rt_bbox* bounds) {
    const RenderContext& c = g_ctx;
    check_update("getMeshBvh", false);
    const int count = (int)(2 * c.mesh.scene.first_leaf);
    const int n = std::min(count, std::max(cap, 0));
    if (n > 0 && !nodes) rt_fail("getMeshBvh: nodes is null");
    if (n > 0) {
        int current = 0;
        HIP_CHECK(hipGetDevice(&current));
        HIP_CHECK(hipSetDevice(c.devs[0].device));
        HIP_CHECK(hipMemcpy(nodes, c.devs[0].d_bvh, (size_t)n * sizeof(rt_bvh_node), hipMemcpyDeviceToHost));
        HIP_CHECK(hipSetDevice(current));
    }
    if (bounds) *bounds = c.mesh.scene.bounds;
    return count;
}

double rtLastUpdateMs(void) {
    if (!g_ctx.initialised) rt_fail("rtLastUpdateMs before init");
    return g_ctx.update_ms;
}

void rebuildBvh(int32_t* old_slot) {
    RenderContext& c = g_ctx;
    check_update("rebuildBvh", false);
    RtMeshParams& mp = c.mesh.scene;
    const uint32_t first_leaf = mp.first_leaf, per_leaf = mp.nppl;
    if ((first_leaf & (first_leaf - 1)) != 0) rt_fail("rebuildBvh: the rebuild needs a tree whose number of leaves is a power of two");
    const size_t slots = (size_t)first_leaf * per_leaf, num_tris = c.mesh.tris.size();
    size_t n = 0;
    for (uint32_t leaf = 0; leaf < first_leaf; leaf++)
        for (uint32_t k = 0; k < per_leaf && !std::isinf(c.mesh.tris[(size_t)leaf * per_leaf + k].v[0].e[0]); k++) n++;
    if (n > (size_t)RT_REBUILD_MAX_TRIS) rt_fail("rebuildBvh: more than RT_REBUILD_MAX_TRIS visible triangles");
    const bool records = per_leaf <= 255;
    const size_t words = rt_build_workspace_words((uint32_t)n, first_leaf);
    std::vector<int32_t> from(num_tris);
    if (records) c.mesh.leaf_ofs.assign(((size_t)first_leaf + 3) / 4, 0u);
    int current = 0;
    HIP_CHECK(hipGetDevice(&current));
    for (DeviceState& d : c.devs) {
        HIP_CHECK(hipSetDevice(d.device));
        if (!d.d_tris_alt) d.d_tris_alt = dev_alloc<rt_triangle>(d.owned, num_tris);
        if (!d.d_old_slot) d.d_old_slot = dev_alloc<int32_t>(d.owned, num_tris);
        if (d.build_words != words) {
            dev_release(d.owned, d.d_build_work);
            d.d_build_work = dev_alloc<uint32_t>(d.owned, words);
            d.build_words = words;
        }
        if (records && !d.d_leaf_tri) d.d_leaf_tri = dev_alloc<float4>(d.owned, slots * 3);
        if (records && !d.d_leaf_ofs) d.d_leaf_ofs = dev_alloc<uint32_t>(d.owned, ((size_t)first_leaf + 3) / 4);
        RtBuildParams b;
        b.slots_in = d.d_tris; b.slots_out = d.d_tris_alt; b.old_slot = d.d_old_slot; b.leaf_ofs = records ? d.d_leaf_ofs : nullptr; b.work = d.d_build_work;
        b.num_tris = (uint32_t)num_tris; b.first_leaf = first_leaf; b.nppl = per_leaf; b.n = (uint32_t)n;
        HIP_CHECK(hipEventRecord(d.ev_reb_start, d.stream));
        HIP_CHECK(rt_launch_rebuild(b, d.stream));
        std::swap(d.d_tris, d.d_tris_alt);
        if (d.d_leaf_tri) HIP_CHECK(hipMemsetAsync(d.d_leaf_tri, 0, slots * 3 * sizeof(float4), d.stream));
        launch_refit(d);
        HIP_CHECK(hipEventRecord(d.ev_reb_stop, d.stream));
    }
    const DeviceState& d0 = c.devs[0];
    rt_bvh_node root;
    HIP_CHECK(hipSetDevice(d0.device));
    HIP_CHECK(hipMemcpyAsync(&root, reinterpret_cast<const char*>(d0.d_bvh) + sizeof(rt_bvh_node), sizeof root, hipMemcpyDeviceToHost, d0.stream));
    HIP_CHECK(hipMemcpyAsync(from.data(), d0.d_old_slot, num_tris * sizeof(int32_t), hipMemcpyDeviceToHost, d0.stream));
    if (records) HIP_CHECK(hipMemcpyAsync(c.mesh.leaf_ofs.data(), d0.d_leaf_ofs, c.mesh.leaf_ofs.size() * sizeof(uint32_t), hipMemcpyDeviceToHost, d0.stream));
    const double ms_max = finish_devices(&DeviceState::ev_reb_start, &DeviceState::ev_reb_stop, false);
    HIP_CHECK(hipSetDevice(current));
    permute_triangles(c.mesh, from);
    if (records) c.mesh.leaf_tri.resize(slots * 3);
    mp.leaf_sentinels_trailing = 1;
    mp.bounds.min = root.a;
    mp.bounds.max = root.b;
    c.refit_stale = true;
    c.rebuild_ms = ms_max;
    if (old_slot) std::copy(from.begin(), from.end(), old_slot);
    scene_edited();
}

double rtLastRebuildMs(void) {
    if (!g_ctx.initialised) rt_fail("rtLastRebuildMs before init");
    return g_ctx.rebuild_ms;
}

void renderGuides(int mask, float* albedo, float* normal, float* depth, int32_t* prim, int32_t* nodes) {
    RenderContext& c = g_ctx;
    if (!c.initialised) rt_fail("renderGuides before init");
    constexpr int kAll = RT_GUIDE_ALBEDO | RT_GUIDE_NORMAL | RT_GUIDE_DEPTH | RT_GUIDE_PRIM | RT_GUIDE_NODES;
    if (mask == 0 || (mask & ~kAll) != 0) rt_fail("renderGuides: mask must name at least one RT_GUIDE_* plane and no unknown bit");
    void* const host[5] = { albedo, normal, depth, prim, nodes };
    for (int k = 0; k < 5; k++)
        if ((mask >> k & 1) && !host[k]) rt_fail("renderGuides: a requested plane has a null pointer");
    if ((mask & RT_GUIDE_NODES) && c.is_spheres) rt_fail("renderGuides: RT_GUIDE_NODES is only defined for mesh scenes");
    if (c.is_spheres && c.opt.floor) rt_fail("renderGuides: the floor plane is only defined for mesh scenes (kernel_scene.floor)");
    int current = 0;
    HIP_CHECK(hipGetDevice(&current));
    const int nd = (int)c.devs.size();
    for (int k = 0; k < nd; k++) {
        DeviceState& d = c.devs[k];
        if (d.fb_rows == 0) continue;
        HIP_CHECK(hipSetDevice(d.device));
        const RtPartition part = partition_of(k);
        void* plane[5] = { nullptr, nullptr, nullptr, nullptr, nullptr };
        for (int q = 0; q < 5; q++) {
            if (!(mask >> q & 1)) continue;
            if (!d.d_guide[q]) d.d_guide[q] = dev_alloc<char>(d.owned, d.fb_rows * c.nx * kGuideBytes[q]);
            plane[q] = d.d_guide[q];
        }
        const RtGuidePlanes g = { static_cast<float*>(plane[0]), static_cast<float*>(plane[1]), static_cast<float*>(plane[2]),
                                  static_cast<int32_t*>(plane[3]), static_cast<int32_t*>(plane[4]) };
        HIP_CHECK(hipEventRecord(d.ev_start, d.stream));
        launch_guides(d, part, g);
        HIP_CHECK(hipEventRecord(d.ev_stop, d.stream));
        for (int q = 0; q < 5; q++)
            if (plane[q]) deliver_stripes(d, part, static_cast<char*>(host[q]), static_cast<const char*>(plane[q]), kGuideBytes[q]);
    }
    c.guides_ms = finish_devices(&DeviceState::ev_start, &DeviceState::ev_stop, true);
    HIP_CHECK(hipSetDevice(current));
}

double rtLastGuidesMs(void) { return g_ctx.guides_ms; }

static void run_rays(int n, const void* const host_in[4], void* const host_out[kRayBuffers], bool any) {
    RenderContext& c = g_ctx;
    RayState& q = g_rays;
    const DeviceState& d = c.devs[0];
    int current = 0;
    HIP_CHECK(hipGetDevice(&current));
    HIP_CHECK(hipSetDevice(d.device));
    const void* host[kRayBuffers];
    for (int k = 0; k < kRayBuffers; k++) host[k] = k < kRayT ? host_in[k] : host_out[k];
    double ms_sum = 0.0;
    for (size_t first = 0; first < (size_t)n; first += kRayChunk) {
        const size_t m = std::min((size_t)kRayChunk, (size_t)n - first);
        for (int k = 0; k < kRayBuffers; k++) {
            if (!host[k] || q.cap[k] >= m) continue;
// ... 284 lines not shown
```

cuda-raytracing-optimized_amd/csrc/rt_sphere_form.h:

```cpp
#pragma once

#include "rt_params.h"

enum class SphereFrame {
    Tiles,
    GlobalSingle,
    TwoDispatch,
    TwoDispatchResume,
    OrderedSingle,
    ClassifiedSingle,
    PlainSingle,
};

constexpr int kSphereFormGeneral = RT_SPHERE_FORM_GENERAL, kSphereFormDefault = RT_SPHERE_FORM_DEFAULT;

inline int sphere_frame_form(SphereFrame frame, const RtSphereParams& p, const RtSwitches& sw, bool kind_folded, bool default_constants) {
    const bool cost_ordered = frame == SphereFrame::TwoDispatch || frame == SphereFrame::OrderedSingle || frame == SphereFrame::TwoDispatchResume;
    const bool direct = p.fb_global_rows != 0 || p.poison_fb != 0;
    const bool diagnostics = p.counters != nullptr || p.wave_dbg != nullptr;
    return (cost_ordered && kind_folded && default_constants && p.xcd_queues == kXcdQueues && p.ord_rec != nullptr && sw.mid_waves == 0 && !sw.tune && !direct && !diagnostics) ? kSphereFormDefault
                                                                                                                                              : kSphereFormGeneral;
}
```

include/rt_api.h:

```cpp
#ifndef RT_API_H
#define RT_API_H

#include "rt_types.h"

#ifdef __cplusplus
extern "C" {
#endif


void initRenderer(const rt_kernel_scene sc, const rt_camera cam, rt_vec3** fb, int nx, int ny, int maxDepth);

void runRenderer(int ns, int tx, int ty);

void cleanupRenderer(void);


void initRendererSpheres(const rt_sphere* spheres, const rt_material* materials, int n,
                         const rt_camera cam, rt_vec3** fb, int nx, int ny, int maxDepth);

void getDefaultRenderOptions(rt_render_options* opt, int is_sphere_scene);

void setRenderOptions(const rt_render_options* opt);

void setExternalFramebuffer(rt_vec3* fb);

void getRenderStats(rt_render_stats* out);

int rtDeviceCount(void);

#define RT_API_VERSION 1002
int rtApiVersion(void);

enum { RT_SIZEOF_RENDER_OPTIONS = 0, RT_SIZEOF_RENDER_STATS, RT_SIZEOF_CAMERA, RT_SIZEOF_SPHERE, RT_SIZEOF_MATERIAL, RT_SIZEOF_TRIANGLE,
       RT_SIZEOF_BVH_NODE, RT_SIZEOF_MESH, RT_SIZEOF_KERNEL_SCENE, RT_SIZEOF_STEXTURE, RT_SIZEOF_PLANE, RT_SIZEOF_BBOX, RT_SIZEOF_VEC3,
       RT_SIZEOF_COUNT };
int rtStructSizes(int32_t* out, int n);


#define RT_PROGRESSIVE_MAX_SAMPLES 65536
void runRendererProgressive(int ns, int tx, int ty);
int rtProgressiveSamples(void);
void rtResetProgressive(void);
void setCamera(const rt_camera* cam);

enum { RT_GUIDE_ALBEDO = 1, RT_GUIDE_NORMAL = 2, RT_GUIDE_DEPTH = 4, RT_GUIDE_PRIM = 8, RT_GUIDE_NODES = 16 };
enum { RT_GUIDE_PRIM_NONE = -1, RT_GUIDE_PRIM_FLOOR = -2 };
void renderGuides(int mask, float* albedo, float* normal, float* depth, int32_t* prim, int32_t* nodes);
double rtLastGuidesMs(void);

enum { RT_DENOISE_DEMODULATE = 1, RT_DENOISE_SAME_PRIM = 2 };
#define RT_DENOISE_MAX_ITERATIONS 8
#define RT_DENOISE_MAX_SQUARINGS  7
#define RT_DENOISE_ALBEDO_FLOOR   0.01f
int rtDefaultDenoiseFlags(void);
void denoiseFrame(const rt_vec3* in, rt_vec3* out, int iterations, int flags, int normal_squarings, float sigma_z, float sigma_c);
double rtLastDenoiseMs(void);

#define RT_ACCUM_MAX_HISTORY 1024
void accumulateFrame(const rt_vec3* in, rt_vec3* out, float* history, int flags, int max_history, float sigma_z, float normal_min);
void rtResetHistory(void);
int rtHistoryFrames(void);
double rtLastAccumulateMs(void);

#define RT_PREVIEW_MIN_HISTORY 4.0f
#define RT_PREVIEW_LUM_EPS     1e-4f
void   previewFrame(const rt_vec3* in, rt_vec3* out, float* history, float* variance, int flags, int max_history,
                    int iterations, int normal_squarings, float sigma_z, float normal_min, float sigma_l);
void   rtResetPreview(void);
int    rtPreviewFrames(void);
double rtLastPreviewMs(void);

enum { RT_DISPLAY_TOP_DOWN = 1, RT_DISPLAY_DITHER = 2, RT_DISPLAY_AUTO_EXPOSURE = 4, RT_DISPLAY_FROM_PREVIEW = 8 };
enum { RT_TONEMAP_NONE = 0, RT_TONEMAP_REINHARD = 1, RT_TONEMAP_ACES = 2 };
#define RT_DISPLAY_BINS 256
#define RT_DISPLAY_KEY  0.18f
#define RT_DISPLAY_BAYER8 { {  0, 32,  8, 40,  2, 34, 10, 42 }, { 48, 16, 56, 24, 50, 18, 58, 26 }, { 12, 44,  4, 36, 14, 46,  6, 38 }, \
                            { 60, 28, 52, 20, 62, 30, 54, 22 }, {  3, 35, 11, 43,  1, 33,  9, 41 }, { 51, 19, 59, 27, 49, 17, 57, 25 }, \
                            { 15, 47,  7, 39, 13, 45,  5, 37 }, { 63, 31, 55, 23, 61, 29, 53, 21 } }
void   displayFrame(const rt_vec3* in, uint8_t* out_rgba, int flags, int tonemap, float exposure, float adapt);
float  rtLastExposure(void);
int    rtDisplayHistogram(uint32_t* out, int cap);
void   rtResetDisplay(void);
double rtLastDisplayMs(void);

enum { RT_RAY_T = 1, RT_RAY_PRIM = 2, RT_RAY_NORMAL = 4, RT_RAY_UV = 8, RT_RAY_NODES = 16 };
#define RT_RAY_CHUNK (1 << 22)
void   traceRays(int n, const float* org, const float* dir, const float* t_min, const float* t_max, int mask,
                 float* t, int32_t* prim, float* normal, float* uv, int32_t* nodes);
void   occludedRays(int n, const float* org, const float* dir, const float* t_min, const float* t_max, uint8_t* occluded);
double rtLastRaysMs(void);

void   updateTriangles(int first, int count, const rt_triangle* tris);
void   updateMaterials(const rt_material* materials, int n);
void   updateSpheres(const rt_sphere* spheres, const rt_material* materials, int n);
int    getMeshBvh(rt_bvh_node* nodes, int cap, rt_bbox* bounds);
double rtLastUpdateMs(void);

#define RT_REBUILD_MAX_TRIS (1 << 24)
#define RT_REBUILD_TILE 256
void   rebuildBvh(int32_t* old_slot);
double rtLastRebuildMs(void);

enum { RT_KERNEL_SPHERE_QUEUE = 1, RT_KERNEL_SPHERE_TILES = 2, RT_KERNEL_MESH_QUEUE = 3, RT_KERNEL_MESH_TILES = 4 };
enum { RT_LAUNCH_FAMILY = 0, RT_LAUNCH_PHASE, RT_LAUNCH_CLS, RT_LAUNCH_CHUNKED, RT_LAUNCH_DBG, RT_LAUNCH_SCENE, RT_LAUNCH_LEAN,
       RT_LAUNCH_THREADS, RT_LAUNCH_BLOCKS, RT_LAUNCH_DEVICE, RT_LAUNCH_FP, RT_LAUNCH_WORDS };
int rtLastLaunches(int32_t* out, int cap);
enum { RT_SPHERE_FORM_NONE = -1, RT_SPHERE_FORM_GENERAL = 0, RT_SPHERE_FORM_DEFAULT = 1 };
int rtLastSphereForm(void);

#ifdef __cplusplus
}
#endif

#endif
```

Measured before the change: 9345 Msamples/s.

## Add tail delivery of late pixels via host-mapped list and reuse pixel cost order

Adds a tail form of the folded sphere kernel, enabled only by RT_TAIL_DELIVERY and off by default. Once the work queue is exhausted and few pixels remain live, the last pixels are written to a pinned host list, and a ready flag lets the host start the framebuffer copy on a separate stream while the kernel finishes. The host then scatters the late records into the frame. This is meant to hide the device-to-host copy behind the kernel tail, at the cost of extra atomics, fences and host spinning. Separately, when the scene and settings key matches an earlier call, the existing cost order is kept: the queue memset and the order_pixels_by_cost pass are replaced by a tiny reset kernel, which removes per-frame sorting work.

```diff
diff --git a/cuda-raytracing-optimized_amd/__init__.py b/cuda-raytracing-optimized_amd/__init__.py
--- a/cuda-raytracing-optimized_amd/__init__.py
+++ b/cuda-raytracing-optimized_amd/__init__.py
@@ -113,7 +113,7 @@
                     "traceRays", "occludedRays", "rtLastRaysMs",
                     "updateTriangles", "updateMaterials", "updateSpheres", "getMeshBvh", "rtLastUpdateMs",
                     "rebuildBvh", "rtLastRebuildMs",
-                    "rtLastSphereForm"]
+                    "rtLastSphereForm", "rtLastDelivery"]
 RT_API_VERSION = 1002
 ABI_STRUCTS = [render_options, render_stats, camera, sphere, material, triangle, bvh_node, mesh, kernel_scene, stexture, plane, bbox, vec3]
 HOST_SYMBOLS = ["rtMakeCamera", "rtRandomFloat", "rtSceneThreeSpheres", "rtSceneRandomSpheres", "rtStaircaseCamera",
@@ -887,7 +887,7 @@
     return [dict(zip(LAUNCH_FIELDS, buf[k * len(LAUNCH_FIELDS):(k + 1) * len(LAUNCH_FIELDS)])) for k in range(n)]
 
 
-RT_SPHERE_FORM_NONE, RT_SPHERE_FORM_GENERAL, RT_SPHERE_FORM_DEFAULT = -1, 0, 1
+RT_SPHERE_FORM_NONE, RT_SPHERE_FORM_GENERAL, RT_SPHERE_FORM_DEFAULT, RT_SPHERE_FORM_TAIL = -1, 0, 1, 2
 
 
 def last_sphere_form():
@@ -895,6 +895,19 @@
     lib.rtLastSphereForm.argtypes = []
     lib.rtLastSphereForm.restype = C.c_int
     return lib.rtLastSphereForm()
+
+
+DELIVERY_FIELDS = ["early_pixels", "late_pixels", "capacity", "copy_early", "order_passes"]
+
+
+def last_delivery():
+    lib = load_renderer()
+    lib.rtLastDelivery.argtypes = [C.POINTER(C.c_int64), C.c_int]
+    lib.rtLastDelivery.restype = C.c_int
+    buf = (C.c_int64 * len(DELIVERY_FIELDS))()
+    n = lib.rtLastDelivery(buf, len(DELIVERY_FIELDS))
+    assert n == len(DELIVERY_FIELDS), n
+    return dict(zip(DELIVERY_FIELDS, (int(v) for v in buf)))
 
 
 
diff --git a/cuda-raytracing-optimized_amd/csrc/rt_kernels_spheres.hip b/cuda-raytracing-optimized_amd/csrc/rt_kernels_spheres.hip
--- a/cuda-raytracing-optimized_amd/csrc/rt_kernels_spheres.hip
+++ b/cuda-raytracing-optimized_amd/csrc/rt_kernels_spheres.hip
@@ -1199,7 +1199,8 @@
 template <int PHASE, int CLS, bool CHUNKED, bool DBG, int SCENE = 0, int LEAN = 0, int FORM = 0>
 __global__ void __launch_bounds__(kThreads, (LEAN & 4) ? 6 : 4) k_render_spheres_queue(const RtSphereParams P, uint32_t stride, int cfg, int chain_cfg, int caps, FormTag<FORM>) {
     static_assert(FORM == kSphereFormGeneral || (PHASE == 2 && CLS == 2 && !CHUNKED && !DBG && SCENE == 0), "the folded form is the cost-ordered dispatch of whole pixels, LDS scene, no diagnostics");
-    constexpr bool FOLDED = FORM == kSphereFormDefault;
+    constexpr bool TAIL = FORM == kSphereFormTail;
+    constexpr bool FOLDED = FORM == kSphereFormDefault || TAIL;
     constexpr bool MID = CLS == 2 && !FOLDED;
     if (FOLDED) { cfg = kDefaultCfg; chain_cfg = default_chain_cfg((LEAN & 4) != 0); caps = kDefaultCaps; }
     extern __shared__ __align__(16) unsigned char smem[];
@@ -1266,6 +1267,8 @@
     uint32_t pix_rays = 0;
     bool exhausted = false;
     uint32_t pool_next = 0, pool_end = 0;
+    bool drained = false, probing = false;
+    uint32_t cap_waits = 0, ex_probe = 0;
     float* fbf = reinterpret_cast<float*>(P.fb);
     auto sample_params = [&]() {
         typedef const __attribute__((address_space(4))) float* ColdF;
@@ -1304,7 +1307,13 @@
                     P.px_rays[px] = pix_rays;
                 } else if (!CHUNKED) {
                     const f3 out = L.col / (float)P.ns;
-                    *reinterpret_cast<float3*>(fbf + ((size_t)((!FOLDED && P.fb_global_rows) ? L.j : lr) * P.nx + L.i) * 3) = make_float3(out.x, out.y, out.z);
+                    float4* const late = (TAIL && drained) ? rt_cold_arg<float4*>(offsetof(RtSphereParams, late_list)) : nullptr;
+                    if (TAIL && late) {
+                        const uint32_t slot = atomicAdd(P.queue + kTailLateCount, 1u);
+                        if (slot < rt_cold_arg<uint32_t>(offsetof(RtSphereParams, late_cap))) late[slot] = make_float4(__uint_as_float(((uint32_t)lr << 16) | (uint32_t)L.i), out.x, out.y, out.z);
+                    } else {
+                        *reinterpret_cast<float3*>(fbf + ((size_t)((!FOLDED && P.fb_global_rows) ? L.j : lr) * P.nx + L.i) * 3) = make_float3(out.x, out.y, out.z);
+                    }
                     uint32_t* const rays_out = rt_cold_arg<uint32_t*>(offsetof(RtSphereParams, acc_rays));
                     if (rays_out) {
                         const size_t px = (size_t)lr * P.nx + L.i;
@@ -1343,6 +1352,7 @@
                 if (__ballot(have_pixel && ccls == 0) != 0ull) cap = min(cap, caps & caps_list(0).mask);
             }
             const int allowed = cap - (int)__popcll(live_m);
+            if (TAIL && allowed <= 0 && pool_next >= pool_end && (cap_waits++ & 63u) == 0u) { ex_probe = __hip_atomic_load(P.queue + kTailExhausted, __ATOMIC_RELAXED, __HIP_MEMORY_SCOPE_AGENT); probing = true; }
             if (allowed <= 0) break;
             const unsigned long long idle_m = ~live_m;
             const uint32_t idle_rank = __builtin_amdgcn_mbcnt_hi((uint32_t)(idle_m >> 32), __builtin_amdgcn_mbcnt_lo((uint32_t)idle_m, 0u));
@@ -1363,6 +1373,7 @@
                     if (role < 2) { role = 2; continue; }
                     if (xq > 1u && stolen + 1u < 2u * xq) { stolen++; continue; }
                     exhausted = true;
+                    if (TAIL && (threadIdx.x & 63) == 0) __hip_atomic_store(P.queue + kTailExhausted, 1u, __ATOMIC_RELAXED, __HIP_MEMORY_SCOPE_AGENT);
                     break;
                 }
                 pool_next = b;
@@ -1472,6 +1483,18 @@
         if (need_sample) { start_sample<PHASE == 0>(sample_params(), L); need_sample = false; }
         const unsigned long long live_now = __ballot(have_pixel);
         if (dbg_timers) dbg_tm[7] += __builtin_amdgcn_s_memtime() - t_refill;
+        if (TAIL && !drained && exhausted && __popcll(live_now) <= kLateLive) {
+            drained = true;
+            if (rt_cold_arg<float4*>(offsetof(RtSphereParams, late_list))) {
+                __builtin_amdgcn_fence(__ATOMIC_RELEASE, "agent");
+                asm volatile("s_waitcnt vmcnt(0)" ::: "memory");
+                uint32_t before = 0;
+                if ((threadIdx.x & 63) == 0) before = atomicAdd(P.queue + kTailDrained, 1u);
+                before = __builtin_amdgcn_readfirstlane(before);
+                if (before + 1u == gridDim.x * (blockDim.x >> 6) && (threadIdx.x & 63) == 0)
+                    __hip_atomic_store(rt_cold_arg<uint32_t*>(offsetof(RtSphereParams, late_ready)), 1u, __ATOMIC_RELEASE, __HIP_MEMORY_SCOPE_SYSTEM);
+            }
+        }
         if (live_now == 0ull) break;
         if (wdbg) {
             if (exhausted && dbg_tex == 0ull) dbg_tex = __builtin_amdgcn_s_memrealtime();
@@ -1501,6 +1524,7 @@
             if (dbg_timers) { dbg_tm[x > 0 ? 9 : 8] += 1ull; }
             finish(done && sel, steps > 1, sample);
         }
+        if (TAIL && probing) { probing = false; if (__builtin_amdgcn_readfirstlane(ex_probe) != 0u && pool_next >= pool_end) exhausted = true; }
     }
 
     if (PHASE == 1 && poison_at != ~0u && iter_no <= poison_at) poison_rows(P, (size_t)blockIdx.x * blockDim.x + threadIdx.x, (size_t)gridDim.x * blockDim.x);
@@ -1567,6 +1591,14 @@
     }
     hipLaunchKernelGGL(kern, grid, block, lds, stream, args...);
     return hipGetLastError();
+}
+
+namespace {
+__global__ void k_reset_grab(uint32_t* queue) {
+    const uint32_t t = threadIdx.x;
+    if (t < 3u * kXcdQueues) queue[(t / 3u) * kXcdQueueWords + t % 3u] = 0u;
+    if (t >= 32u && t < 35u) queue[kTailExhausted + (int)(t - 32u)] = 0u;
+}
 }
 
 static hipError_t order_pixels_by_cost(const RtSphereParams& q, hipStream_t stream) {
@@ -1745,6 +1777,8 @@
     return pl;
 }
 
+static size_t late_records(const SpherePlan& pl) { return (size_t)pl.blocks * (size_t)(pl.threads / 64) * (size_t)kLateLive; }
+
 template <int PHASE, int CLS, bool CHUNKED, bool DBG, int SCENE, int LEAN = 0> struct SphereQueueForm {};
 
 template <int PHASE, int CLS, bool CHUNKED, bool DBG, int SCENE, int LEAN>
@@ -1757,7 +1791,7 @@
     };
     hipError_t e;
     if constexpr (folded_built(PHASE, CLS, CHUNKED, DBG, SCENE, LEAN)) {
-        e = form == kSphereFormDefault ? launch_form(FormTag<kSphereFormDefault>{}) : launch_form(FormTag<kSphereFormGeneral>{});
+        e = form == kSphereFormTail ? launch_form(FormTag<kSphereFormTail>{}) : (form == kSphereFormDefault ? launch_form(FormTag<kSphereFormDefault>{}) : launch_form(FormTag<kSphereFormGeneral>{}));
     } else {
         if (form != kSphereFormGeneral) return hipErrorInvalidValue;
         e = launch_form(FormTag<kSphereFormGeneral>{});
@@ -1808,13 +1842,15 @@
         return e;
     }
     if (!p.queue) return hipErrorInvalidValue;
-    if ((e = hipMemsetAsync(p.queue, 0, 256, stream)) != hipSuccess) return e;
+    const bool keep_order = pl.frame == SphereFrame::OrderedSingle && p.order_kept != 0 && pl.error == SpherePlanError::None;
+    if (!keep_order && (e = hipMemsetAsync(p.queue, 0, 256, stream)) != hipSuccess) return e;
     if (pl.error == SpherePlanError::Tune)
         fprintf(stderr, "rt error: RT_TUNE=%s out of range (chain_every 1..255, chain_waves 0..%d, heavy_thr 1..255, n_chain 0..15, boost 0..255, "
                         "chain_pixels 1..15, chain_pixels of list 0 / 1 / 2 1..15)\n", sw.tune->text.c_str(), kWavesPerWg);
     if (pl.error != SpherePlanError::None) return hipErrorInvalidValue;
     if (pl.frame == SphereFrame::TwoDispatch || pl.frame == SphereFrame::TwoDispatchResume || pl.frame == SphereFrame::OrderedSingle) {
         RtSphereParams q = p;
+        if (pl.form != kSphereFormTail || !q.late_list || !q.late_ready || (size_t)q.late_cap < late_records(pl)) { q.late_list = nullptr; q.late_ready = nullptr; q.late_cap = 0; }
         if (pl.frame == SphereFrame::TwoDispatchResume) {
             q.px_state = p.acc_state; q.px_rays = p.acc_rays; q.s_split = p.acc_first;
             e = wait_fb();
@@ -1826,8 +1862,15 @@
             e = launch_queue_form<1, 0, false>(pl, q, stream, pl.stride1, pl.cfg1);
         }
         if (e != hipSuccess) return e;
-        if ((e = hipMemsetAsync(p.queue, 0, sizeof(uint32_t) * kXcdQueues * kXcdQueueWords, stream)) != hipSuccess) return e;
-        if ((e = order_pixels_by_cost(q, stream)) != hipSuccess) return e;
+        if (keep_order) {
+            hipLaunchKernelGGL(k_reset_grab, dim3(1), dim3(64), 0, stream, p.queue);
+            if ((e = hipGetLastError()) != hipSuccess) return e;
+            rt_note_order(kOrderKept);
+        } else {
+            if ((e = hipMemsetAsync(p.queue, 0, sizeof(uint32_t) * kXcdQueues * kXcdQueueWords, stream)) != hipSuccess) return e;
+            if ((e = order_pixels_by_cost(q, stream)) != hipSuccess) return e;
+            rt_note_order(pl.frame == SphereFrame::OrderedSingle ? kOrderBuilt + q.cost_samples : kOrderParked);
+        }
         q.phase = 2;
         if (sw.wave_debug_phase) q.wave_dbg = nullptr;
         return launch_queue_form<2, 2, false>(pl, q, stream, pl.stride, pl.cfg, pl.caps);
@@ -1847,3 +1890,13 @@
     }
     return hipGetLastError();
 }
+
+#if defined(RT_MODE_PARITY)
+size_t rt_sphere_late_records(const RtSphereParams& p, int variant, const RtSwitches& sw) {
+    int dev = 0, cus = 256;
+    if (hipGetDevice(&dev) == hipSuccess) (void)hipDeviceGetAttribute(&cus, hipDeviceAttributeMultiprocessorCount, dev);
+    const SpherePlan pl = plan_spheres(p, variant, sw, cus);
+    const bool cost_ordered = pl.frame == SphereFrame::TwoDispatch || pl.frame == SphereFrame::TwoDispatchResume || pl.frame == SphereFrame::OrderedSingle;
+    return (p.queue && pl.error == SpherePlanError::None && cost_ordered && pl.form == kSphereFormTail) ? late_records(pl) : 0;
+}
+#endif
diff --git a/cuda-raytracing-optimized_amd/csrc/rt_late_scatter.h b/cuda-raytracing-optimized_amd/csrc/rt_late_scatter.h
--- /dev/null
+++ b/cuda-raytracing-optimized_amd/csrc/rt_late_scatter.h
@@ -0,0 +1,27 @@
+#pragma once
+
+#include <stddef.h>
+#include <stdint.h>
+
+struct RtLateRec {
+    uint32_t pixel;
+    float r, g, b;
+};
+constexpr uint32_t kLateFreeSlot = 0xFFFFFFFFu;
+
+inline long rt_scatter_late(RtLateRec* list, size_t capacity, int stripe_rows, int rank, int world, int local_rows, int nx, int ny, float* fb) {
+    long n = 0;
+    for (size_t k = 0; k < capacity; k++) {
+        const RtLateRec rec = list[k];
+        if (rec.pixel == kLateFreeSlot) break;
+        const long lr = (long)(rec.pixel >> 16), col = (long)(rec.pixel & 0xFFFFu);
+        if (stripe_rows <= 0 || world <= 0 || rank < 0 || rank >= world || lr >= (long)local_rows || col >= (long)nx) return -1;
+        const long row = ((lr / stripe_rows) * world + rank) * stripe_rows + lr % stripe_rows;
+        if (row >= (long)ny) return -1;
+        float* const px = fb + ((size_t)row * (size_t)nx + (size_t)col) * 3;
+        px[0] = rec.r; px[1] = rec.g; px[2] = rec.b;
+        list[k].pixel = kLateFreeSlot;
+        n++;
+    }
+    return n;
+}
diff --git a/cuda-raytracing-optimized_amd/csrc/rt_params.h b/cuda-raytracing-optimized_amd/csrc/rt_params.h
--- a/cuda-raytracing-optimized_amd/csrc/rt_params.h
+++ b/cuda-raytracing-optimized_amd/csrc/rt_params.h
@@ -89,7 +89,21 @@
     int32_t acc_first;
     uint32_t* cost_rays;
     int32_t cost_samples;
-};
+    float4* late_list;
+    uint32_t* late_ready;
+    uint32_t late_cap;
+    int32_t order_kept;
+};
+struct RtLateRecord {
+    uint32_t pixel;
+    float r, g, b;
+};
+constexpr uint32_t kLateFree = 0xFFFFFFFFu;
+#ifndef RT_LATE_LIVE
+#define RT_LATE_LIVE 4
+#endif
+constexpr int kLateLive = RT_LATE_LIVE;
+constexpr int kTailExhausted = 60, kTailDrained = 61, kTailLateCount = 62;
 constexpr int kXcdQueueWords = 64;
 constexpr int kXcdQueues = 8;
 __host__ __device__ inline uint32_t rt_xcd_of_pixel(uint32_t local_row, uint32_t nx, uint32_t column) {
@@ -178,6 +192,7 @@
     bool ext_fb_no_register = false;
     bool cleanup_device_reset = false;
     int cost_reuse = 1;
+    bool tail_delivery = false;
     int top_thr = 384;
     bool basic = true;
     bool onepass = true;
@@ -213,10 +228,13 @@
 
 hipError_t rt_launch_spheres_parity(const RtSphereParams& p, int variant, const RtSwitches& sw, hipStream_t stream);
 hipError_t rt_launch_spheres_fast(const RtSphereParams& p, int variant, const RtSwitches& sw, hipStream_t stream);
+size_t rt_sphere_late_records(const RtSphereParams& p, int variant, const RtSwitches& sw);
 hipError_t rt_launch_mesh_parity(const RtMeshParams& p, int variant, const RtSwitches& sw, hipStream_t stream);
 hipError_t rt_launch_mesh_fast(const RtMeshParams& p, int variant, const RtSwitches& sw, hipStream_t stream);
 void rt_note_launch(int family, int phase, int cls, int chunked, int dbg, int scene, int lean, int threads, unsigned blocks);
 void rt_note_sphere_form(int form);
+constexpr int kOrderNone = -1, kOrderParked = -2, kOrderKept = 0, kOrderBuilt = 0;
+void rt_note_order(int word);
 
 struct RtGuidePlanes {
     float* albedo;
diff --git a/cuda-raytracing-optimized_amd/csrc/rt_renderer.hip b/cuda-raytracing-optimized_amd/csrc/rt_renderer.hip
--- a/cuda-raytracing-optimized_amd/csrc/rt_renderer.hip
+++ b/cuda-raytracing-optimized_amd/csrc/rt_renderer.hip
@@ -15,6 +15,7 @@
 #include "../../include/rt_api.h"
 #include "rt_params.h"
 #include "rt_scene_layout.h"
+#include "rt_late_scatter.h"
 #include "rt_denoise.h"
 #include "rt_accumulate.h"
 #include "rt_preview.h"
@@ -113,8 +114,15 @@
     uint32_t* d_cost_rays = nullptr;
     int cost_samples = 0;
     std::array<int, 11> cost_key = {};
+    int order_samples = 0;
+    std::array<long long, 20> order_key = {};
     float4* d_acc_state = nullptr;
     uint32_t* d_acc_rays = nullptr;
+    hipStream_t copy_stream = nullptr;
+    RtLateRecord* h_late = nullptr;
+    size_t late_cap = 0;
+    uint32_t* h_late_ready = nullptr;
+    bool tail_armed = false;
     void* d_guide[5] = { nullptr, nullptr, nullptr, nullptr, nullptr };
 };
 
@@ -215,6 +223,11 @@
 std::vector<int32_t> g_launches;
 int g_launch_device = 0, g_launch_fp = 0;
 int g_sphere_form = RT_SPHERE_FORM_NONE;
+struct DeliveryStats {
+    int64_t early_pixels = 0, late_pixels = 0, capacity = 0, copy_early = 0, order_passes = 0;
+};
+DeliveryStats g_delivery;
+int g_order_note = kOrderNone;
 
 void default_options(rt_render_options* o, int spheres) {
     memset(o, 0, sizeof *o);
@@ -240,6 +253,10 @@
     if (d.stream) HIP_CHECK(hipStreamSynchronize(d.stream));
     dev_release_all(d.owned);
     if (d.h_params) HIP_CHECK(hipHostFree(d.h_params));
+    if (d.copy_stream) HIP_CHECK(hipStreamSynchronize(d.copy_stream));
+    if (d.h_late) HIP_CHECK(hipHostFree(d.h_late));
+    if (d.h_late_ready) HIP_CHECK(hipHostFree(d.h_late_ready));
+    if (d.copy_stream) HIP_CHECK(hipStreamDestroy(d.copy_stream));
     if (d.ev_start) HIP_CHECK(hipEventDestroy(d.ev_start));
     if (d.ev_stop) HIP_CHECK(hipEventDestroy(d.ev_stop));
     if (d.ev_upd_start) HIP_CHECK(hipEventDestroy(d.ev_upd_start));
@@ -330,6 +347,9 @@
         if (c.is_spheres) {
             d.d_params = dev_alloc<RtSphereParams>(d.owned, 1);
             HIP_CHECK(hipHostMalloc((void**)&d.h_params, sizeof(RtSphereParams), hipHostMallocDefault));
+            HIP_CHECK(hipStreamCreateWithFlags(&d.copy_stream, hipStreamNonBlocking));
+            HIP_CHECK(hipHostMalloc((void**)&d.h_late_ready, 64, hipHostMallocDefault));
+            *d.h_late_ready = 0;
             upload_sphere_arrays(d);
         } else {
             d.d_tris = upload(d.owned, c.mesh.tris);
@@ -422,6 +442,7 @@
     const int32_t rec[RT_LAUNCH_WORDS] = { family, phase, cls, chunked, dbg, scene, lean, threads, (int32_t)blocks, g_launch_device, g_launch_fp };
     g_launches.insert(g_launches.end(), rec, rec + RT_LAUNCH_WORDS);
 }
+void rt_note_order(int word) { g_order_note = word; }
 void rt_note_sphere_form(int form) { g_sphere_form = g_sphere_form == RT_SPHERE_FORM_NONE ? form : std::min(g_sphere_form, form); }
 
 extern "C" {
@@ -438,6 +459,12 @@
 }
 
 int rtLastSphereForm(void) { return g_sphere_form; }
+
+int rtLastDelivery(int64_t* out, int cap) {
+    const int64_t words[RT_DELIVERY_WORDS] = { g_delivery.early_pixels, g_delivery.late_pixels, g_delivery.capacity, g_delivery.copy_early, g_delivery.order_passes };
+    for (int k = 0; k < cap && k < RT_DELIVERY_WORDS; k++) out[k] = words[k];
+    return RT_DELIVERY_WORDS;
+}
 
 int rtLastLaunches(int32_t* out, int cap) {
     const int count = (int)(g_launches.size() / RT_LAUNCH_WORDS);
@@ -564,20 +591,21 @@
     return d.d_wave_dbg;
 }
 
-void deliver_stripes(const DeviceState& d, const RtPartition& part, char* host, const char* dev, size_t px_bytes) {
+void deliver_stripes(const DeviceState& d, const RtPartition& part, char* host, const char* dev, size_t px_bytes, hipStream_t stream = nullptr) {
     const RenderContext& c = g_ctx;
+    if (!stream) stream = d.stream;
     const size_t row_bytes = (size_t)c.nx * px_bytes;
     const size_t stripe_bytes = (size_t)part.stripe_rows * row_bytes;
     const size_t full = d.fb_rows / part.stripe_rows, rem = d.fb_rows % part.stripe_rows;
     char* dst0 = host + (size_t)part.rank * stripe_bytes;
     if (part.world == 1) {
-        HIP_CHECK(hipMemcpyAsync(dst0, dev, d.fb_rows * row_bytes, hipMemcpyDeviceToHost, d.stream));
+        HIP_CHECK(hipMemcpyAsync(dst0, dev, d.fb_rows * row_bytes, hipMemcpyDeviceToHost, stream));
         return;
     }
     if (full > 0)
-        HIP_CHECK(hipMemcpy2DAsync(dst0, (size_t)part.world * stripe_bytes, dev, stripe_bytes, stripe_bytes, full, hipMemcpyDeviceToHost, d.stream));
+        HIP_CHECK(hipMemcpy2DAsync(dst0, (size_t)part.world * stripe_bytes, dev, stripe_bytes, stripe_bytes, full, hipMemcpyDeviceToHost, stream));
     if (rem > 0)
-        HIP_CHECK(hipMemcpyAsync(dst0 + full * (size_t)part.world * stripe_bytes, dev + full * stripe_bytes, rem * row_bytes, hipMemcpyDeviceToHost, d.stream));
+        HIP_CHECK(hipMemcpyAsync(dst0 + full * (size_t)part.world * stripe_bytes, dev + full * stripe_bytes, rem * row_bytes, hipMemcpyDeviceToHost, stream));
 }
 
 
@@ -672,6 +700,15 @@
              c.scene_edits };
 }
 
+constexpr int kKeptOrderSamples = 8;
+std::array<long long, 20> order_key_of(const DeviceState& d, const std::array<int, 11>& cost_key, const RtSwitches& sw) {
+    std::array<long long, 20> k = {};
+    for (size_t i = 0; i < cost_key.size(); i++) k[i] = cost_key[i];
+    k[11] = sw.xcd_queues; k[12] = sw.ord_packed; k[13] = sw.top_thr; k[14] = g_ctx.opt.variant; k[15] = g_ctx.opt.fp;
+    k[16] = (long long)(intptr_t)d.d_ord_rec; k[17] = (long long)(intptr_t)d.d_ord_state; k[18] = (long long)(intptr_t)d.d_order; k[19] = (long long)(intptr_t)d.d_queue;
+    return k;
+}
+
 double finish_devices(hipEvent_t DeviceState::*start, hipEvent_t DeviceState::*stop, bool with_rows) {
     double ms_max = 0.0;
     for (DeviceState& d : g_ctx.devs) {
@@ -698,6 +735,7 @@
     g_sphere_form = RT_SPHERE_FORM_NONE;
     g_launch_fp = c.opt.fp;
     const RtSwitches sw = rt_read_switches();
+    g_delivery = DeliveryStats();
 
     for (int k = 0; k < nd; k++) {
         DeviceState& d = c.devs[k];
@@ -726,6 +764,7 @@
             HIP_CHECK(hipMemsetAsync(d.d_fb, 0, d.fb_rows * row_bytes, d.stream));
         } else if (c.is_spheres) {
             RtSphereParams p = sphere_params(d, part);
+            std::array<long long, 20> order_key = {};
             p.ns = ns; p.max_depth = c.max_depth;
             p.fb = d.d_fb;
             p.rr = c.opt.rr; p.rng_mode = c.opt.rng;
@@ -748,6 +787,8 @@
                 p.cost_samples = key == d.cost_key ? d.cost_samples : 0;
                 d.cost_key = key;
                 d.cost_samples = ns;
+                order_key = order_key_of(d, key, sw);
+                p.order_kept = (p.cost_samples > 0 && !sw.tune && d.order_samples >= kKeptOrderSamples && order_key == d.order_key) ? 1 : 0;
             }
             p.chain_top_thr = sw.top_thr;
             p.ord_rec = sw.ord_packed ? d.d_ord_rec : nullptr;
@@ -772,13 +813,38 @@
                 p.fb_global_rows = 1;
                 p.poison_fb = sw.fb_poison ? 1 : 0;
             }
+            d.tail_armed = false;
+            const size_t late_n = fb_direct ? 0 : rt_sphere_late_records(p, c.opt.variant, sw);
+            if (late_n > 0) {
+                if (late_n > d.late_cap) {
+                    if (d.h_late) HIP_CHECK(hipHostFree(d.h_late));
+                    d.h_late = nullptr;
+                    HIP_CHECK(hipHostMalloc((void**)&d.h_late, late_n * sizeof(RtLateRecord), hipHostMallocDefault));
+                    memset(d.h_late, 0xFF, late_n * sizeof(RtLateRecord));
+                    d.late_cap = late_n;
+                }
+                void* dp_list = nullptr;
+                void* dp_ready = nullptr;
+                HIP_CHECK(hipHostGetDevicePointer(&dp_list, d.h_late, 0));
+                HIP_CHECK(hipHostGetDevicePointer(&dp_ready, d.h_late_ready, 0));
+                p.late_list = static_cast<float4*>(dp_list);
+                p.late_ready = static_cast<uint32_t*>(dp_ready);
+                p.late_cap = (uint32_t)d.late_cap;
+                __atomic_store_n(d.h_late_ready, 0u, __ATOMIC_RELEASE);
+                d.tail_armed = true;
+            }
             p.self = d.d_params;
             *d.h_params = p;
             HIP_CHECK(hipMemcpyAsync(d.d_params, d.h_params, sizeof(RtSphereParams), hipMemcpyHostToDevice, d.stream));
+            g_order_note = kOrderNone;
             HIP_CHECK(c.opt.fp == RT_FP_FAST ? rt_launch_spheres_fast(p, c.opt.variant, sw, d.stream)
                                              : rt_launch_spheres_parity(p, c.opt.variant, sw, d.stream));
+            if (g_order_note != kOrderKept) d.order_samples = g_order_note > kOrderBuilt ? g_order_note - kOrderBuilt : 0;
+            d.order_key = order_key;
+            if (g_order_note > kOrderBuilt || g_order_note == kOrderParked) g_delivery.order_passes++;
             launches++;
         } else {
+            d.tail_armed = false;
             RtMeshParams p = mesh_params(d, part);
             p.ns = ns; p.max_depth = c.max_depth;
             p.leaf_tri = sw.compact_leaves ? d.d_leaf_tri : nullptr; p.leaf_ofs = sw.compact_leaves ? d.d_leaf_ofs : nullptr;
@@ -801,11 +867,57 @@
         }
         HIP_CHECK(hipEventRecord(d.ev_stop, d.stream));
 
-        if (!fb_direct) deliver_stripes(d, part, reinterpret_cast<char*>(h_target), reinterpret_cast<const char*>(d.d_fb), sizeof(rt_vec3));
+        if (c.max_depth <= 0) d.tail_armed = false;
+        if (!fb_direct && !d.tail_armed) deliver_stripes(d, part, reinterpret_cast<char*>(h_target), reinterpret_cast<const char*>(d.d_fb), sizeof(rt_vec3));
         samples += (int64_t)d.fb_rows * c.nx * (ns - first);
     }
 
+    std::vector<int> waiting;
+    for (int k = 0; k < nd; k++) if (c.devs[k].fb_rows > 0 && c.devs[k].tail_armed) waiting.push_back(k);
+    rt_vec3* const h_frame = c.h_ext ? c.h_ext : c.h_fb;
+    for (unsigned spin = 0; !waiting.empty(); spin++) {
+        for (size_t w = 0; w < waiting.size();) {
+            DeviceState& d = c.devs[waiting[w]];
+            hipStream_t on = nullptr;
+            if (__atomic_load_n(d.h_late_ready, __ATOMIC_ACQUIRE) != 0u) on = d.copy_stream;
+            else if ((spin & 1023u) == 1023u) {
+                HIP_CHECK(hipSetDevice(d.device));
+                const hipError_t e = hipStreamQuery(d.stream);
+                if (e != hipErrorNotReady) { HIP_CHECK(e); on = d.stream; }
+            }
+            if (!on) {
+#if defined(__x86_64__)
+                __builtin_ia32_pause();
+#endif
+                w++;
+                continue;
+            }
+            HIP_CHECK(hipSetDevice(d.device));
+            deliver_stripes(d, partition_of(waiting[w]), reinterpret_cast<char*>(h_frame), reinterpret_cast<const char*>(d.d_fb), sizeof(rt_vec3), on);
+            if (on == d.copy_stream) g_delivery.copy_early = 1;
+            waiting.erase(waiting.begin() + (long)w);
+        }
+    }
+    for (int k = 0; k < nd; k++) {
+        DeviceState& d = c.devs[k];
+        if (d.fb_rows == 0 || !d.tail_armed) continue;
+        HIP_CHECK(hipSetDevice(d.device));
+        HIP_CHECK(hipStreamSynchronize(d.copy_stream));
+    }
     const double kernel_ms = finish_devices(&DeviceState::ev_start, &DeviceState::ev_stop, true);
+    for (int k = 0; k < nd; k++) {
+        DeviceState& d = c.devs[k];
+        if (d.fb_rows == 0 || !d.tail_armed) continue;
+        const RtPartition part = partition_of(k);
+        static_assert(sizeof(RtLateRec) == sizeof(RtLateRecord) && kLateFreeSlot == kLateFree, "the kernel's record is the scatter's");
+        const long late = rt_scatter_late(reinterpret_cast<RtLateRec*>(d.h_late), d.late_cap, part.stripe_rows, part.rank, part.world, part.local_rows, c.nx, c.ny,
+                                          reinterpret_cast<float*>(h_frame));
+        if (late < 0) rt_fail("runRenderer: a late record names a pixel outside the partition");
+        g_delivery.late_pixels += late;
+        g_delivery.early_pixels += (int64_t)d.fb_rows * c.nx - late;
+        g_delivery.capacity += (int64_t)d.late_cap;
+        d.tail_armed = false;
+    }
     rt_render_stats st;
     memset(&st, 0, sizeof st);
     for (int k = 0; k < nd; k++) {
@@ -883,6 +995,7 @@
     s.cleanup_device_reset = env_one("RT_CLEANUP_DEVICE_RESET");
     const int cost_reuse = env_int("RT_COST_REUSE", s.cost_reuse);
     s.cost_reuse = (cost_reuse >= 0 && cost_reuse <= 2) ? cost_reuse : 1;
+    s.tail_delivery = env_flag("RT_TAIL_DELIVERY", s.tail_delivery);
 
     const int top_thr = env_int("RT_TOP_THR", s.top_thr);
     if (top_thr >= 320) s.top_thr = top_thr;
diff --git a/cuda-raytracing-optimized_amd/csrc/rt_sphere_form.h b/cuda-raytracing-optimized_amd/csrc/rt_sphere_form.h
--- a/cuda-raytracing-optimized_amd/csrc/rt_sphere_form.h
+++ b/cuda-raytracing-optimized_amd/csrc/rt_sphere_form.h
@@ -12,12 +12,13 @@
     PlainSingle,
 };
 
-constexpr int kSphereFormGeneral = RT_SPHERE_FORM_GENERAL, kSphereFormDefault = RT_SPHERE_FORM_DEFAULT;
+constexpr int kSphereFormGeneral = RT_SPHERE_FORM_GENERAL, kSphereFormDefault = RT_SPHERE_FORM_DEFAULT, kSphereFormTail = RT_SPHERE_FORM_TAIL;
 
 inline int sphere_frame_form(SphereFrame frame, const RtSphereParams& p, const RtSwitches& sw, bool kind_folded, bool default_constants) {
     const bool cost_ordered = frame == SphereFrame::TwoDispatch || frame == SphereFrame::OrderedSingle || frame == SphereFrame::TwoDispatchResume;
     const bool direct = p.fb_global_rows != 0 || p.poison_fb != 0;
     const bool diagnostics = p.counters != nullptr || p.wave_dbg != nullptr;
-    return (cost_ordered && kind_folded && default_constants && p.xcd_queues == kXcdQueues && p.ord_rec != nullptr && sw.mid_waves == 0 && !sw.tune && !direct && !diagnostics) ? kSphereFormDefault
-                                                                                                                                              : kSphereFormGeneral;
+    return (cost_ordered && kind_folded && default_constants && p.xcd_queues == kXcdQueues && p.ord_rec != nullptr && sw.mid_waves == 0 && !sw.tune && !direct && !diagnostics)
+               ? (sw.tail_delivery ? kSphereFormTail : kSphereFormDefault)
+               : kSphereFormGeneral;
 }
diff --git a/include/rt_api.h b/include/rt_api.h
--- a/include/rt_api.h
+++ b/include/rt_api.h
@@ -105,8 +105,10 @@
 enum { RT_LAUNCH_FAMILY = 0, RT_LAUNCH_PHASE, RT_LAUNCH_CLS, RT_LAUNCH_CHUNKED, RT_LAUNCH_DBG, RT_LAUNCH_SCENE, RT_LAUNCH_LEAN,
        RT_LAUNCH_THREADS, RT_LAUNCH_BLOCKS, RT_LAUNCH_DEVICE, RT_LAUNCH_FP, RT_LAUNCH_WORDS };
 int rtLastLaunches(int32_t* out, int cap);
-enum { RT_SPHERE_FORM_NONE = -1, RT_SPHERE_FORM_GENERAL = 0, RT_SPHERE_FORM_DEFAULT = 1 };
+enum { RT_SPHERE_FORM_NONE = -1, RT_SPHERE_FORM_GENERAL = 0, RT_SPHERE_FORM_DEFAULT = 1, RT_SPHERE_FORM_TAIL = 2 };
 int rtLastSphereForm(void);
+enum { RT_DELIVERY_EARLY_PIXELS = 0, RT_DELIVERY_LATE_PIXELS, RT_DELIVERY_CAPACITY, RT_DELIVERY_COPY_EARLY, RT_DELIVERY_ORDER_PASSES, RT_DELIVERY_WORDS };
+int rtLastDelivery(int64_t* out, int cap);
 
 #ifdef __cplusplus
 }
```

Result: no change. 9419 Msamples/s, median of 6 (+0.8%).
